# qinzheng93/GeoTransformer

Hardware: NVIDIA H100
Metric: point-cloud pairs/sec (3DMatch-shape synth) (higher is better)
Workload: dtype f32

## Files before the change

### geotransformer_b200/_lib.py

```python
import ctypes
import os
import threading

import torch

_HERE = os.path.dirname(os.path.abspath(__file__))
LIB_PATH = os.path.join(_HERE, 'libgeob200.so')
_lib = None

c_void_p, c_int64, c_int32, c_float, c_size_t, c_int = (
    ctypes.c_void_p, ctypes.c_int64, ctypes.c_int32, ctypes.c_float, ctypes.c_size_t, ctypes.c_int)

SIGNATURES = {}


def _sig(name, restype, *argtypes):
    SIGNATURES[name] = (restype, list(argtypes))


P, I64, I32, F, SZ = c_void_p, c_int64, c_int32, c_float, c_size_t
_sig('geob200_last_error', ctypes.c_char_p)
_sig('geob200_launch_count', ctypes.c_uint64)
_sig('geob200_grid_subsample_workspace_bytes', SZ, I64, I64)
_sig('geob200_grid_subsample', c_int, P, I64, P, I64, F, P, P, P, SZ, P)
_sig('geob200_radius_search_workspace_bytes', SZ, I64, I64, I64)
_sig('geob200_radius_search', c_int, P, I64, P, I64, P, P, I64, F, I64, P, P, P, P, SZ, P)

_sig('geob200_neighbor_histogram', c_int, P, I64, I64, I64, I64, P, P)
_sig('geob200_kpconv_workspace_bytes', SZ, I64)
_sig('geob200_kpconv', c_int, P, P, P, P, I64, I64, I64, P, I64, P, P, I64, I64, F, P, P, SZ, P)
_sig('geob200_kpconv_tc_workspace_bytes', SZ, I64, I64, I64)
_sig('geob200_kpconv_tc', c_int, P, P, P, P, I64, I64, I64, P, I64, P, P, I64, I64, F, P, P, SZ, P)
_sig('geob200_set_linear_mode', None, c_int)
_sig('geob200_linear', c_int, P, I64, P, P, P, I64, I64, I64, I64, c_int, P)
_sig('geob200_linear_batched', c_int, P, I64, I64, P, I64, I64, P, I64, P, I64, I64, I64, I64, I64, I64, c_int, P)
_sig('geob200_group_norm_workspace_bytes', SZ, I64)
_sig('geob200_group_norm', c_int, P, I64, I64, I64, P, P, F, P, c_int, F, P, P, SZ, P)
_sig('geob200_fused_group_norm_workspace_bytes', SZ, I64, I64, I64)
_sig('geob200_linear_group_norm', c_int, P, I64, P, P, I64, I64, I64, I64, P, P, F, P, c_int, F, P, P, P, SZ, P)
_sig('geob200_kpconv_group_norm_workspace_bytes', SZ, I64, I64, I64, I64, I64)
_sig('geob200_kpconv_group_norm', c_int, P, P, P, P, I64, I64, I64, P, I64, P, P, I64, I64, F, I64, P, P, F, c_int, F, P, P, P, SZ,
     P, SZ, P)
_sig('geob200_group_norm_batched_workspace_bytes', SZ, I64, I64, I64, I64)
_sig('geob200_group_norm_batched', c_int, P, I64, I64, I64, P, P, F, P, c_int, F, P, P, SZ, P, I64, P)
_sig('geob200_linear_group_norm_batched', c_int, P, I64, P, P, I64, I64, I64, I64, P, P, F, P, c_int, F, P, P, P, SZ, P, I64, P)
_sig('geob200_maxpool', c_int, P, P, I64, I64, I64, I64, P, P)
_sig('geob200_upsample_concat', c_int, P, P, I64, I64, P, I64, I64, I64, P, P)
_sig('geob200_point_to_node_partition', c_int, P, I64, P, I64, I64, P, P, P, P, P, P, P)
_sig('geob200_point_to_node_partition_batched', c_int, P, P, I64, P, P, I64, P, P, P, P, P, P)
_sig('geob200_gather_rows', c_int, P, I64, I64, P, I64, P, P)
_sig('geob200_knn_partition', c_int, P, I64, P, I64, I64, P, P, P)
_sig('geob200_pairwise_distance', c_int, P, I64, P, I64, I64, c_int, P, P)
_sig('geob200_point_to_node_indices', c_int, P, I64, P, I64, P, P, P)
_sig('geob200_apply_transform', c_int, P, I64, P, P, P)
_sig('geob200_gse_indices', c_int, P, I64, F, F, I64, P, P, P)
_sig('geob200_gse_indices_batched', c_int, P, I64, P, F, F, I64, P, P, P)
_sig('geob200_gse_embed_workspace_bytes', SZ, I64, I64)
_sig('geob200_gse_table_bytes', SZ, I64, I64, F, F)
_sig('geob200_gse_table_build', c_int, P, P, P, P, P, I64, I64, F, F, P, SZ, P)
_sig('geob200_gse_embed_table', c_int, P, P, I64, I64, P, SZ, I64, F, F, P, P, P, P, P, P, P)
_sig('geob200_gse_embed', c_int, P, P, I64, I64, P, P, P, P, P, P, P, P, c_int, P, SZ, P)
_sig('geob200_gse_embed_pairs', c_int, P, P, I64, I64, P, P, P, P, P, P, P, P, c_int, P, SZ, P)
_sig('geob200_attention_workspace_bytes', SZ, I64, I64, I64)
_sig('geob200_attention', c_int, P, I64, P, I64, P, I64, P, P, P, I64, I64, I64, I64, P, I64, P, SZ, P)
_sig('geob200_set_attention_tma', c_int, c_int)
_sig('geob200_head_bias', c_int, P, I64, P, I64, I64, I64, P, P)
_sig('geob200_add_layernorm', c_int, P, P, P, P, I64, I64, F, P, P)
_sig('geob200_l2_normalize', c_int, P, I64, I64, P, P)
_sig('geob200_superpoint_matching_workspace_bytes', SZ, I64, I64)
_sig('geob200_superpoint_matching', c_int, P, P, I64, I64, I64, P, P, I64, c_int, P, P, P, P, P, SZ, P)
_sig('geob200_gather_patches', c_int, P, I64, P, P, I64, P, I64, P, P, P, P)
_sig('geob200_patch_scores', c_int, P, I64, P, I64, I64, P, P, I64, I64, P, P)
_sig('geob200_sinkhorn', c_int, P, P, P, P, I64, I64, I64, F, P, P)
_sig('geob200_lgr_workspace_bytes', SZ, I64, I64, I64)
_sig('geob200_local_global_registration', c_int, P, P, P, P, P, I64, I64, I64, I64, F, c_int, F, I64, I64, P, P, P, P, P,
     P, P, P, P, P, SZ, P)
_sig('geob200_superpoint_matching_batched_workspace_bytes', SZ, I64, I64, I64)
_sig('geob200_superpoint_matching_batched', c_int, P, I64, P, I64, P, I64, c_int, P, P, P, P, SZ, P)
_sig('geob200_gather_patches_batched', c_int, P, I64, I64, P, P, P, P, I64, P, P, P, P, P)
_sig('geob200_patch_scores_batched', c_int, P, I64, I64, P, P, P, I64, I64, P, P)
_sig('geob200_lgr_batched_workspace_bytes', SZ, I64, I64, I64, I64)
_sig('geob200_local_global_registration_batched', c_int, P, P, P, P, P, I64, I64, I64, I64, I64, F, c_int, F, I64, I64, P, P, P, P,
     P, P, I64, P, P, P, P, SZ, P)
_sig('geob200_weighted_procrustes', c_int, P, P, P, I64, I64, F, F, P, P)

_sig('geob200_node_correspondences_workspace_bytes', SZ, I64, I64, I64)
_sig('geob200_node_correspondences', c_int, P, P, P, P, P, P, P, P, I64, I64, I64, P, F, P, P, P, P, SZ, P)
_sig('geob200_node_correspondences_batched_workspace_bytes', SZ, I64, I64, I64)
_sig('geob200_node_correspondences_batched', c_int, P, P, P, P, I64, P, I64, P, F, P, P, P, P, SZ, P)
_sig('geob200_evaluate', c_int, P, P, I64, F, P, P, I64, P, P, I64, F, P, P, P, I64, c_int, F, F, F, P, P)
_sig('geob200_evaluate_counts', c_int, P, P, I64, P, F, P, P, I64, P, P, P, I64, P, F, P, P, P, I64, c_int, F, F, F, P, P)
_sig('geob200_evaluate_batched', c_int, P, P, P, F, P, P, I64, P, P, P, I64, P, F, P, P, I64, P, I64, P, P, c_int, F, F, F, P, I64,
     P)

_sig('geob200_linear_profile_enable', c_int, c_int)
_sig('geob200_set_split_k', c_int, c_int)
_sig('geob200_set_linear_persistent', c_int, c_int)
_sig('geob200_linear_profile_read', I64, I64, P, P)
_sig('geob200_backbone_workspace_bytes', SZ, P, P)
_sig('geob200_backbone_forward', c_int, P, P, P, P, P, P, P, P, P, P, P, P, SZ, P, SZ, P)
_sig('geob200_transformer_workspace_bytes', SZ, I64, I64, I64, I64, I64)
_sig('geob200_transformer_forward', c_int, P, I64, I64, I64, P, I64, I64, P, P, P, P, SZ, P)
_sig('geob200_backbone_gn_workspace_bytes', SZ, P, P, I64)
_sig('geob200_backbone_forward_batched', c_int, P, P, P, P, P, P, P, P, P, P, P, P, SZ, P, SZ, P, I64, P, P)
_sig('geob200_cloud_max_count', c_int, P, I64, I64, I64, I64, P, P, P)
_sig('geob200_maxpool_batched', c_int, P, P, I64, I64, I64, I64, P, I64, P, P, P)
_sig('geob200_transformer_batched_workspace_bytes', SZ, I64, P, I64, I64, I64)
_sig('geob200_transformer_forward_batched', c_int, P, I64, I64, I64, P, I64, P, P, P, P, SZ, P)
_sig('geob200_attention_batched_workspace_bytes', SZ, P, I64, I64)
_sig('geob200_attention_batched', c_int, P, I64, I64, I64, I64, I64, I64, I64, P, SZ, P)


def lib():
    global _lib
    if _lib is None:
        if not os.path.exists(LIB_PATH):
            raise RuntimeError(
                f'{LIB_PATH} not found: build it with `python -c "import __graft_entry__ as g; g.build()"` '
                '(there is no CPU fallback for the geotransformer_b200 ops)')
        handle = ctypes.CDLL(LIB_PATH)
        for name, (restype, argtypes) in SIGNATURES.items():
            fn = getattr(handle, name)
            fn.restype = restype
            fn.argtypes = argtypes
        _lib = handle
    return _lib


def check(rc, what):
    if rc != 0:
        msg = lib().geob200_last_error().decode(errors='replace')
        raise RuntimeError(f'{what} failed ({rc}): {msg}')


_tls = threading.local()


def stream_ptr():
    p = getattr(_tls, 'stream', None)
    if p is not None:
        return p
    return torch.cuda.current_stream().cuda_stream


class stream_scope:

    def __init__(self, ptr):
        self.ptr = ptr

    def __enter__(self):
        self.prev = getattr(_tls, 'stream', None)
        _tls.stream = self.ptr
        return self

    def __exit__(self, *a):
        _tls.stream = self.prev
        return False


def require_cuda(t, name, dtype=None):
    if not t.is_cuda:
        raise RuntimeError(f'{name} must be a CUDA tensor (geotransformer_b200 has no CPU path)')
    if dtype is not None and t.dtype != dtype:
        raise RuntimeError(f'{name} must be {dtype}, got {t.dtype}')
    if not t.is_contiguous():
        raise RuntimeError(f'{name} must be contiguous')


_WS = {}


def workspace(nbytes, device, tag='default'):
    key = (device.index if device.index is not None else torch.cuda.current_device(), stream_ptr(), tag)
    buf = _WS.get(key)
    if buf is None or buf.numel() < nbytes:
        buf = torch.empty(max(int(nbytes * 1.3), 1 << 20), dtype=torch.uint8, device=device)
        _WS[key] = buf
    return buf


def ptr(t):
    return None if t is None else t.data_ptr()
```

### geotransformer_b200/csrc/common.cuh

```cuda
#pragma once
#include <cuda_runtime.h>
#include <stdint.h>
#include <stdio.h>

namespace geob200 {

void set_error(const char* fmt, ...);
void count_launches(int n);
int ensure_max_smem(const void* kernel);

#define GEOB_CHECK_CUDA(expr)                                                                   \
    do {                                                                                        \
        cudaError_t _e = (expr);                                                                \
        if (_e != cudaSuccess) {                                                                \
            geob200::set_error("%s:%d CUDA error %s: %s", __FILE__, __LINE__, #expr,            \
                               cudaGetErrorString(_e));                                         \
            return -1;                                                                          \
        }                                                                                       \
    } while (0)

#define GEOB_CHECK_LAUNCH()                                                                     \
    do {                                                                                        \
        cudaError_t _e = cudaGetLastError();                                                    \
        if (_e != cudaSuccess) {                                                                \
            geob200::set_error("%s:%d kernel launch failed: %s", __FILE__, __LINE__,            \
                               cudaGetErrorString(_e));                                         \
            return -1;                                                                          \
        }                                                                                       \
    } while (0)

#define GEOB_REQUIRE(cond, ...)                                                                 \
    do {                                                                                        \
        if (!(cond)) {                                                                          \
            geob200::set_error(__VA_ARGS__);                                                    \
            return -2;                                                                          \
        }                                                                                       \
    } while (0)

static inline size_t align_up(size_t x, size_t a) { return (x + a - 1) / a * a; }

template <int CNT, int MASK>
struct Butterfly {
    template <int NV>
    static __device__ __forceinline__ void run(float (&v)[NV], int lane) {
        if constexpr (CNT > 1) {
            constexpr int HALF = CNT / 2;
            const bool upper = (lane & MASK) != 0;
#pragma unroll
            for (int i = 0; i < HALF; ++i) {
                const float send = upper ? v[i] : v[i + HALF];
                const float keep = upper ? v[i + HALF] : v[i];
                v[i] = keep + __shfl_xor_sync(0xffffffffu, send, MASK);
            }
            if constexpr (MASK > 1) Butterfly<HALF, MASK / 2>::run(v, lane);
        } else {
            v[0] += __shfl_xor_sync(0xffffffffu, v[0], MASK);
            if constexpr (MASK > 1) Butterfly<1, MASK / 2>::run(v, lane);
        }
    }
};
template <int NV>
__device__ __forceinline__ float warp_butterfly(float (&v)[NV], int lane) {
    Butterfly<NV, 16>::run(v, lane);
    return v[0];
}

struct GnFuse {
    int groups;
    int slot_width;
    double* partial;
};

constexpr int GEOB_MAX_CLOUDS = 64;
struct GnSeg {
    int n_clouds;
    int n_pairs;
    int start[GEOB_MAX_CLOUDS + 1];
};
size_t fused_group_norm_workspace_bytes_batched(int64_t n_rows, int64_t channels, int64_t groups, int64_t n_pairs);
int group_norm_impl(const float* x, int64_t n_rows, int64_t channels, int64_t groups, const float* gamma, const float* beta, float eps,
                    const float* residual, int leaky, float slope, float* y, void* workspace, size_t workspace_bytes, void* stream,
                    const GnSeg* seg);
int linear_group_norm_impl(const float* x, int64_t ldx, const float* weight, const float* bias, int64_t m, int64_t n, int64_t k,
                           int64_t groups, const float* gamma, const float* beta, float eps, const float* residual, int leaky,
                           float slope, float* pre_norm, float* y, void* workspace, size_t workspace_bytes, void* stream,
                           const GnSeg* seg);
int kpconv_group_norm_impl(const float* s_feats, const float* q_points, const float* s_points, const int64_t* neighbors,
                           int64_t n_query, int64_t n_support, int64_t n_neighbors, const float* kernel_points, int64_t n_kernel,
                           const float* weights_t, const float* bias, int64_t c_in, int64_t c_out, float sigma, int64_t groups,
                           const float* gamma, const float* beta, float eps, int leaky, float slope, float* pre_norm, float* y,
                           void* gn_workspace, size_t gn_workspace_bytes, void* workspace, size_t workspace_bytes, void* stream,
                           const GnSeg* seg);

int maxpool_seg(const float* x, const int64_t* neighbors, int64_t n_query, int64_t n_support, int64_t n_neighbors, int64_t channels,
                float* y, const GnSeg* seg, const int* cloud_max, void* stream);

struct Segs {
    int n;
    int max;
    int start[GEOB_MAX_CLOUDS];
    int count[GEOB_MAX_CLOUDS];
};
int segs_from_counts(Segs* s, int64_t n, const int64_t* counts);
Segs segs_one(int64_t count);
Segs segs_range(const Segs& s, int first, int n);
int segs_products(Segs* s, const Segs& ref, const Segs& src);

struct Arena {
    char* base;
    size_t off;
    size_t cap;
    __host__ Arena(void* p, size_t bytes) : base(static_cast<char*>(p)), off(0), cap(bytes) {}
    template <typename T>
    __host__ T* take(size_t n) {
        off = align_up(off, 256);
        T* r = reinterpret_cast<T*>(base + off);
        off += n * sizeof(T);
        return r;
    }
    __host__ bool ok() const { return off <= cap; }
};

__device__ __forceinline__ float warp_sum(float v) {
#pragma unroll
    for (int o = 16; o > 0; o >>= 1) v += __shfl_xor_sync(0xffffffffu, v, o);
    return v;
}
__device__ __forceinline__ float warp_max(float v) {
#pragma unroll
    for (int o = 16; o > 0; o >>= 1) v = fmaxf(v, __shfl_xor_sync(0xffffffffu, v, o));
    return v;
}
__device__ __forceinline__ double warp_sum_d(double v) {
#pragma unroll
    for (int o = 16; o > 0; o >>= 1) v += __shfl_xor_sync(0xffffffffu, v, o);
    return v;
}

__device__ __forceinline__ float tf32_rn(float x) {
    uint32_t r;
    asm("cvt.rna.tf32.f32 %0, %1;" : "=r"(r) : "f"(x));
    return __uint_as_float(r);
}

static inline int num_sms() {
    static int n = 0;
    if (n == 0) {
        int dev = 0;
        cudaGetDevice(&dev);
        cudaDeviceGetAttribute(&n, cudaDevAttrMultiProcessorCount, dev);
        if (n <= 0) n = 132;
    }
    return n;
}

}
```

### geotransformer_b200/csrc/hopper.cuh

```cuda
#pragma once
#include <cuda.h>
#include <stdint.h>

namespace geob200 {
namespace hop {

__device__ __forceinline__ uint32_t smem_u32(const void* p) { return (uint32_t)__cvta_generic_to_shared(p); }
__device__ __forceinline__ void mbar_init(uint64_t* bar, uint32_t count) {
    asm volatile("mbarrier.init.shared::cta.b64 [%0], %1;" ::"r"(smem_u32(bar)), "r"(count));
}
__device__ __forceinline__ void mbar_arrive(uint64_t* bar) {
    asm volatile("{\n\t.reg .b64 st;\n\tmbarrier.arrive.shared::cta.b64 st, [%0];\n\t}" ::"r"(smem_u32(bar)) : "memory");
}
__device__ __forceinline__ void mbar_arrive_expect_tx(uint64_t* bar, uint32_t bytes) {
    asm volatile("{\n\t.reg .b64 st;\n\tmbarrier.arrive.expect_tx.shared::cta.b64 st, [%0], %1;\n\t}" ::"r"(smem_u32(bar)), "r"(bytes)
                 : "memory");
}
__device__ __forceinline__ void mbar_wait(uint64_t* bar, uint32_t parity) {
    const uint32_t addr = smem_u32(bar);
    uint32_t done;
    do {
        asm volatile("{\n\t.reg .pred p;\n\tmbarrier.try_wait.parity.shared::cta.b64 p, [%1], %2;\n\tselp.u32 %0, 1, 0, p;\n\t}"
                     : "=r"(done)
                     : "r"(addr), "r"(parity)
                     : "memory");
    } while (!done);
}
__device__ __forceinline__ void mbar_wait_cluster(uint64_t* bar, uint32_t parity) {
    const uint32_t addr = smem_u32(bar);
    uint32_t done;
    do {
        asm volatile("{\n\t.reg .pred p;\n\tmbarrier.try_wait.parity.acquire.cluster.shared::cta.b64 p, [%1], %2;\n\tselp.u32 %0, 1, 0, p;\n\t}"
                     : "=r"(done)
                     : "r"(addr), "r"(parity)
                     : "memory");
    } while (!done);
}
__device__ __forceinline__ void fence_proxy_async() { asm volatile("fence.proxy.async.shared::cta;" ::: "memory"); }

__device__ __forceinline__ void tma_load_2d(void* dst, const CUtensorMap* map, int c0, int c1, uint64_t* bar) {
    asm volatile("cp.async.bulk.tensor.2d.shared::cluster.global.mbarrier::complete_tx::bytes [%0], [%1, {%2, %3}], [%4];" ::"r"(
                     smem_u32(dst)),
                 "l"(map), "r"(c0), "r"(c1), "r"(smem_u32(bar))
                 : "memory");
}
__device__ __forceinline__ void bulk_g2s(void* dst, const void* src, uint32_t bytes, uint64_t* bar) {
    asm volatile("cp.async.bulk.shared::cluster.global.mbarrier::complete_tx::bytes [%0], [%1], %2, [%3];" ::"r"(smem_u32(dst)),
                 "l"(src), "r"(bytes), "r"(smem_u32(bar))
                 : "memory");
}

__device__ __forceinline__ uint64_t make_desc(uint32_t smem_addr) {
    uint64_t d = 0;
    d |= (uint64_t)((smem_addr & 0x3FFFFu) >> 4);
    d |= (uint64_t)1 << 16;
    d |= (uint64_t)(1024 >> 4) << 32;
    d |= (uint64_t)1 << 62;
    return d;
}

__device__ __forceinline__ void wgmma_fence() { asm volatile("wgmma.fence.sync.aligned;" ::: "memory"); }
__device__ __forceinline__ void wgmma_commit() { asm volatile("wgmma.commit_group.sync.aligned;" ::: "memory"); }
template <int N>
__device__ __forceinline__ void wgmma_wait() { asm volatile("wgmma.wait_group.sync.aligned %0;" ::"n"(N) : "memory"); }
template <int R>
__device__ __forceinline__ void reg_fence(float (&d)[R]) {
#pragma unroll
    for (int i = 0; i < R; ++i) asm volatile("" : "+f"(d[i])::"memory");
}

template <int N> __device__ void wgmma_tf32(float (&d)[N / 2], uint64_t da, uint64_t db, uint32_t acc);

template <> __device__ __forceinline__ void wgmma_tf32<32>(float (&d)[16], uint64_t da, uint64_t db, uint32_t acc) {
    asm volatile(
        "{\n\t.reg .pred p;\n\tsetp.ne.b32 p, %18, 0;\n\t"
        "wgmma.mma_async.sync.aligned.m64n32k8.f32.tf32.tf32 {%0, %1, %2, %3, %4, %5, %6, %7, %8, %9, %10, %11, %12, %13, %14, %15}, %16, %17, p, 1, 1;\n\t}"
        : "+f"(d[0]), "+f"(d[1]), "+f"(d[2]), "+f"(d[3]), "+f"(d[4]), "+f"(d[5]), "+f"(d[6]), "+f"(d[7]), "+f"(d[8]), "+f"(d[9]), "+f"(d[10]), "+f"(d[11]), "+f"(d[12]), "+f"(d[13]), "+f"(d[14]), "+f"(d[15])
        : "l"(da), "l"(db), "r"(acc));
}

template <> __device__ __forceinline__ void wgmma_tf32<64>(float (&d)[32], uint64_t da, uint64_t db, uint32_t acc) {
    asm volatile(
        "{\n\t.reg .pred p;\n\tsetp.ne.b32 p, %34, 0;\n\t"
        "wgmma.mma_async.sync.aligned.m64n64k8.f32.tf32.tf32 {%0, %1, %2, %3, %4, %5, %6, %7, %8, %9, %10, %11, %12, %13, %14, %15, %16, %17, %18, %19, %20, %21, %22, %23, %24, %25, %26, %27, %28, %29, %30, %31}, %32, %33, p, 1, 1;\n\t}"
        : "+f"(d[0]), "+f"(d[1]), "+f"(d[2]), "+f"(d[3]), "+f"(d[4]), "+f"(d[5]), "+f"(d[6]), "+f"(d[7]), "+f"(d[8]), "+f"(d[9]), "+f"(d[10]), "+f"(d[11]), "+f"(d[12]), "+f"(d[13]), "+f"(d[14]), "+f"(d[15]), "+f"(d[16]), "+f"(d[17]), "+f"(d[18]), "+f"(d[19]), "+f"(d[20]), "+f"(d[21]), "+f"(d[22]), "+f"(d[23]), "+f"(d[24]), "+f"(d[25]), "+f"(d[26]), "+f"(d[27]), "+f"(d[28]), "+f"(d[29]), "+f"(d[30]), "+f"(d[31])
        : "l"(da), "l"(db), "r"(acc));
}

template <> __device__ __forceinline__ void wgmma_tf32<128>(float (&d)[64], uint64_t da, uint64_t db, uint32_t acc) {
    asm volatile(
        "{\n\t.reg .pred p;\n\tsetp.ne.b32 p, %66, 0;\n\t"
        "wgmma.mma_async.sync.aligned.m64n128k8.f32.tf32.tf32 {%0, %1, %2, %3, %4, %5, %6, %7, %8, %9, %10, %11, %12, %13, %14, %15, %16, %17, %18, %19, %20, %21, %22, %23, %24, %25, %26, %27, %28, %29, %30, %31, %32, %33, %34, %35, %36, %37, %38, %39, %40, %41, %42, %43, %44, %45, %46, %47, %48, %49, %50, %51, %52, %53, %54, %55, %56, %57, %58, %59, %60, %61, %62, %63}, %64, %65, p, 1, 1;\n\t}"
        : "+f"(d[0]), "+f"(d[1]), "+f"(d[2]), "+f"(d[3]), "+f"(d[4]), "+f"(d[5]), "+f"(d[6]), "+f"(d[7]), "+f"(d[8]), "+f"(d[9]), "+f"(d[10]), "+f"(d[11]), "+f"(d[12]), "+f"(d[13]), "+f"(d[14]), "+f"(d[15]), "+f"(d[16]), "+f"(d[17]), "+f"(d[18]), "+f"(d[19]), "+f"(d[20]), "+f"(d[21]), "+f"(d[22]), "+f"(d[23]), "+f"(d[24]), "+f"(d[25]), "+f"(d[26]), "+f"(d[27]), "+f"(d[28]), "+f"(d[29]), "+f"(d[30]), "+f"(d[31]), "+f"(d[32]), "+f"(d[33]), "+f"(d[34]), "+f"(d[35]), "+f"(d[36]), "+f"(d[37]), "+f"(d[38]), "+f"(d[39]), "+f"(d[40]), "+f"(d[41]), "+f"(d[42]), "+f"(d[43]), "+f"(d[44]), "+f"(d[45]), "+f"(d[46]), "+f"(d[47]), "+f"(d[48]), "+f"(d[49]), "+f"(d[50]), "+f"(d[51]), "+f"(d[52]), "+f"(d[53]), "+f"(d[54]), "+f"(d[55]), "+f"(d[56]), "+f"(d[57]), "+f"(d[58]), "+f"(d[59]), "+f"(d[60]), "+f"(d[61]), "+f"(d[62]), "+f"(d[63])
        : "l"(da), "l"(db), "r"(acc));
}

template <> __device__ __forceinline__ void wgmma_tf32<256>(float (&d)[128], uint64_t da, uint64_t db, uint32_t acc) {
    asm volatile(
        "{\n\t.reg .pred p;\n\tsetp.ne.b32 p, %130, 0;\n\t"
        "wgmma.mma_async.sync.aligned.m64n256k8.f32.tf32.tf32 {%0, %1, %2, %3, %4, %5, %6, %7, %8, %9, %10, %11, %12, %13, %14, %15, %16, %17, %18, %19, %20, %21, %22, %23, %24, %25, %26, %27, %28, %29, %30, %31, %32, %33, %34, %35, %36, %37, %38, %39, %40, %41, %42, %43, %44, %45, %46, %47, %48, %49, %50, %51, %52, %53, %54, %55, %56, %57, %58, %59, %60, %61, %62, %63, %64, %65, %66, %67, %68, %69, %70, %71, %72, %73, %74, %75, %76, %77, %78, %79, %80, %81, %82, %83, %84, %85, %86, %87, %88, %89, %90, %91, %92, %93, %94, %95, %96, %97, %98, %99, %100, %101, %102, %103, %104, %105, %106, %107, %108, %109, %110, %111, %112, %113, %114, %115, %116, %117, %118, %119, %120, %121, %122, %123, %124, %125, %126, %127}, %128, %129, p, 1, 1;\n\t}"
        : "+f"(d[0]), "+f"(d[1]), "+f"(d[2]), "+f"(d[3]), "+f"(d[4]), "+f"(d[5]), "+f"(d[6]), "+f"(d[7]), "+f"(d[8]), "+f"(d[9]), "+f"(d[10]), "+f"(d[11]), "+f"(d[12]), "+f"(d[13]), "+f"(d[14]), "+f"(d[15]), "+f"(d[16]), "+f"(d[17]), "+f"(d[18]), "+f"(d[19]), "+f"(d[20]), "+f"(d[21]), "+f"(d[22]), "+f"(d[23]), "+f"(d[24]), "+f"(d[25]), "+f"(d[26]), "+f"(d[27]), "+f"(d[28]), "+f"(d[29]), "+f"(d[30]), "+f"(d[31]), "+f"(d[32]), "+f"(d[33]), "+f"(d[34]), "+f"(d[35]), "+f"(d[36]), "+f"(d[37]), "+f"(d[38]), "+f"(d[39]), "+f"(d[40]), "+f"(d[41]), "+f"(d[42]), "+f"(d[43]), "+f"(d[44]), "+f"(d[45]), "+f"(d[46]), "+f"(d[47]), "+f"(d[48]), "+f"(d[49]), "+f"(d[50]), "+f"(d[51]), "+f"(d[52]), "+f"(d[53]), "+f"(d[54]), "+f"(d[55]), "+f"(d[56]), "+f"(d[57]), "+f"(d[58]), "+f"(d[59]), "+f"(d[60]), "+f"(d[61]), "+f"(d[62]), "+f"(d[63]), "+f"(d[64]), "+f"(d[65]), "+f"(d[66]), "+f"(d[67]), "+f"(d[68]), "+f"(d[69]), "+f"(d[70]), "+f"(d[71]), "+f"(d[72]), "+f"(d[73]), "+f"(d[74]), "+f"(d[75]), "+f"(d[76]), "+f"(d[77]), "+f"(d[78]), "+f"(d[79]), "+f"(d[80]), "+f"(d[81]), "+f"(d[82]), "+f"(d[83]), "+f"(d[84]), "+f"(d[85]), "+f"(d[86]), "+f"(d[87]), "+f"(d[88]), "+f"(d[89]), "+f"(d[90]), "+f"(d[91]), "+f"(d[92]), "+f"(d[93]), "+f"(d[94]), "+f"(d[95]), "+f"(d[96]), "+f"(d[97]), "+f"(d[98]), "+f"(d[99]), "+f"(d[100]), "+f"(d[101]), "+f"(d[102]), "+f"(d[103]), "+f"(d[104]), "+f"(d[105]), "+f"(d[106]), "+f"(d[107]), "+f"(d[108]), "+f"(d[109]), "+f"(d[110]), "+f"(d[111]), "+f"(d[112]), "+f"(d[113]), "+f"(d[114]), "+f"(d[115]), "+f"(d[116]), "+f"(d[117]), "+f"(d[118]), "+f"(d[119]), "+f"(d[120]), "+f"(d[121]), "+f"(d[122]), "+f"(d[123]), "+f"(d[124]), "+f"(d[125]), "+f"(d[126]), "+f"(d[127])
        : "l"(da), "l"(db), "r"(acc));
}

template <int N> __device__ void wgmma_f16(float (&d)[N / 2], uint64_t da, uint64_t db, uint32_t acc);

template <> __device__ __forceinline__ void wgmma_f16<128>(float (&d)[64], uint64_t da, uint64_t db, uint32_t acc) {
    asm volatile(
        "{\n\t.reg .pred p;\n\tsetp.ne.b32 p, %66, 0;\n\t"
        "wgmma.mma_async.sync.aligned.m64n128k16.f32.f16.f16 {%0, %1, %2, %3, %4, %5, %6, %7, %8, %9, %10, %11, %12, %13, %14, %15, %16, %17, %18, %19, %20, %21, %22, %23, %24, %25, %26, %27, %28, %29, %30, %31, %32, %33, %34, %35, %36, %37, %38, %39, %40, %41, %42, %43, %44, %45, %46, %47, %48, %49, %50, %51, %52, %53, %54, %55, %56, %57, %58, %59, %60, %61, %62, %63}, %64, %65, p, 1, 1, 0, 0;\n\t}"
        : "+f"(d[0]), "+f"(d[1]), "+f"(d[2]), "+f"(d[3]), "+f"(d[4]), "+f"(d[5]), "+f"(d[6]), "+f"(d[7]), "+f"(d[8]), "+f"(d[9]), "+f"(d[10]), "+f"(d[11]), "+f"(d[12]), "+f"(d[13]), "+f"(d[14]), "+f"(d[15]), "+f"(d[16]), "+f"(d[17]), "+f"(d[18]), "+f"(d[19]), "+f"(d[20]), "+f"(d[21]), "+f"(d[22]), "+f"(d[23]), "+f"(d[24]), "+f"(d[25]), "+f"(d[26]), "+f"(d[27]), "+f"(d[28]), "+f"(d[29]), "+f"(d[30]), "+f"(d[31]), "+f"(d[32]), "+f"(d[33]), "+f"(d[34]), "+f"(d[35]), "+f"(d[36]), "+f"(d[37]), "+f"(d[38]), "+f"(d[39]), "+f"(d[40]), "+f"(d[41]), "+f"(d[42]), "+f"(d[43]), "+f"(d[44]), "+f"(d[45]), "+f"(d[46]), "+f"(d[47]), "+f"(d[48]), "+f"(d[49]), "+f"(d[50]), "+f"(d[51]), "+f"(d[52]), "+f"(d[53]), "+f"(d[54]), "+f"(d[55]), "+f"(d[56]), "+f"(d[57]), "+f"(d[58]), "+f"(d[59]), "+f"(d[60]), "+f"(d[61]), "+f"(d[62]), "+f"(d[63])
        : "l"(da), "l"(db), "r"(acc));
}

template <> __device__ __forceinline__ void wgmma_f16<256>(float (&d)[128], uint64_t da, uint64_t db, uint32_t acc) {
    asm volatile(
        "{\n\t.reg .pred p;\n\tsetp.ne.b32 p, %130, 0;\n\t"
        "wgmma.mma_async.sync.aligned.m64n256k16.f32.f16.f16 {%0, %1, %2, %3, %4, %5, %6, %7, %8, %9, %10, %11, %12, %13, %14, %15, %16, %17, %18, %19, %20, %21, %22, %23, %24, %25, %26, %27, %28, %29, %30, %31, %32, %33, %34, %35, %36, %37, %38, %39, %40, %41, %42, %43, %44, %45, %46, %47, %48, %49, %50, %51, %52, %53, %54, %55, %56, %57, %58, %59, %60, %61, %62, %63, %64, %65, %66, %67, %68, %69, %70, %71, %72, %73, %74, %75, %76, %77, %78, %79, %80, %81, %82, %83, %84, %85, %86, %87, %88, %89, %90, %91, %92, %93, %94, %95, %96, %97, %98, %99, %100, %101, %102, %103, %104, %105, %106, %107, %108, %109, %110, %111, %112, %113, %114, %115, %116, %117, %118, %119, %120, %121, %122, %123, %124, %125, %126, %127}, %128, %129, p, 1, 1, 0, 0;\n\t}"
        : "+f"(d[0]), "+f"(d[1]), "+f"(d[2]), "+f"(d[3]), "+f"(d[4]), "+f"(d[5]), "+f"(d[6]), "+f"(d[7]), "+f"(d[8]), "+f"(d[9]), "+f"(d[10]), "+f"(d[11]), "+f"(d[12]), "+f"(d[13]), "+f"(d[14]), "+f"(d[15]), "+f"(d[16]), "+f"(d[17]), "+f"(d[18]), "+f"(d[19]), "+f"(d[20]), "+f"(d[21]), "+f"(d[22]), "+f"(d[23]), "+f"(d[24]), "+f"(d[25]), "+f"(d[26]), "+f"(d[27]), "+f"(d[28]), "+f"(d[29]), "+f"(d[30]), "+f"(d[31]), "+f"(d[32]), "+f"(d[33]), "+f"(d[34]), "+f"(d[35]), "+f"(d[36]), "+f"(d[37]), "+f"(d[38]), "+f"(d[39]), "+f"(d[40]), "+f"(d[41]), "+f"(d[42]), "+f"(d[43]), "+f"(d[44]), "+f"(d[45]), "+f"(d[46]), "+f"(d[47]), "+f"(d[48]), "+f"(d[49]), "+f"(d[50]), "+f"(d[51]), "+f"(d[52]), "+f"(d[53]), "+f"(d[54]), "+f"(d[55]), "+f"(d[56]), "+f"(d[57]), "+f"(d[58]), "+f"(d[59]), "+f"(d[60]), "+f"(d[61]), "+f"(d[62]), "+f"(d[63]), "+f"(d[64]), "+f"(d[65]), "+f"(d[66]), "+f"(d[67]), "+f"(d[68]), "+f"(d[69]), "+f"(d[70]), "+f"(d[71]), "+f"(d[72]), "+f"(d[73]), "+f"(d[74]), "+f"(d[75]), "+f"(d[76]), "+f"(d[77]), "+f"(d[78]), "+f"(d[79]), "+f"(d[80]), "+f"(d[81]), "+f"(d[82]), "+f"(d[83]), "+f"(d[84]), "+f"(d[85]), "+f"(d[86]), "+f"(d[87]), "+f"(d[88]), "+f"(d[89]), "+f"(d[90]), "+f"(d[91]), "+f"(d[92]), "+f"(d[93]), "+f"(d[94]), "+f"(d[95]), "+f"(d[96]), "+f"(d[97]), "+f"(d[98]), "+f"(d[99]), "+f"(d[100]), "+f"(d[101]), "+f"(d[102]), "+f"(d[103]), "+f"(d[104]), "+f"(d[105]), "+f"(d[106]), "+f"(d[107]), "+f"(d[108]), "+f"(d[109]), "+f"(d[110]), "+f"(d[111]), "+f"(d[112]), "+f"(d[113]), "+f"(d[114]), "+f"(d[115]), "+f"(d[116]), "+f"(d[117]), "+f"(d[118]), "+f"(d[119]), "+f"(d[120]), "+f"(d[121]), "+f"(d[122]), "+f"(d[123]), "+f"(d[124]), "+f"(d[125]), "+f"(d[126]), "+f"(d[127])
        : "l"(da), "l"(db), "r"(acc));
}

}
}
```

### geotransformer_b200/csrc/kpconv.cu

```cuda
#include "common.cuh"
#include "geob200.h"

namespace geob200 {

constexpr int KP = 15;
constexpr int KP_PAD = 16;
constexpr int TQ = 32;
constexpr int CC = 32;

__device__ __forceinline__ void influence15(const float* __restrict__ kp_s, float rx, float ry, float rz, float inv_dummy,
                                            float sigma, float* w) {
#pragma unroll
    for (int k = 0; k < KP; ++k) {
        const float dx = rx - kp_s[3 * k], dy = ry - kp_s[3 * k + 1], dz = rz - kp_s[3 * k + 2];
        const float sq = __fadd_rn(__fadd_rn(__fmul_rn(dx, dx), __fmul_rn(dy, dy)), __fmul_rn(dz, dz));
        w[k] = fmaxf(1.0f - sqrtf(sq) / sigma, 0.0f);
    }
    (void)inv_dummy;
}

__global__ void __launch_bounds__(256) kpconv_c1_kernel(const float* __restrict__ feats, const float* __restrict__ q_pts,
                                                        const float* __restrict__ s_pts, const long long* __restrict__ nbr,
                                                        int H, const float* __restrict__ kp, const float* __restrict__ W,
                                                        const float* __restrict__ bias, float sigma, int Ns, int M, int Cout,
// ... 496 lines not shown
            if (var < 0.0) var = 0.0;
            mean_rstd[2 * g] = (float)mean;
            mean_rstd[2 * g + 1] = (float)(1.0 / sqrt(var + eps));
        }
    }
}

__global__ void __launch_bounds__(256) gn_tile_stats_kernel(const float* __restrict__ x, int N, int C, int slot_width,
                                                            double* __restrict__ partial) {
    extern __shared__ double sh[];
    const int slots = C / slot_width;
    for (int i = threadIdx.x; i < 2 * slots; i += blockDim.x) sh[i] = 0.0;
    __syncthreads();
    const int r0 = blockIdx.x * 128, r1 = min(N, r0 + 128);
    const int cw = C < 256 ? C : 256;
    const int rpb = 256 / cw;
    const int rr = threadIdx.x / cw;
    if (rr < rpb)
        for (int c = threadIdx.x % cw; c < C; c += cw) {
            double s = 0.0, s2 = 0.0;
            for (int r = r0 + rr; r < r1; r += rpb) {
                const double v = (double)x[(long long)r * C + c];
                s += v;
                s2 += v * v;
            }
            atomicAdd(&sh[2 * (c / slot_width)], s);
            atomicAdd(&sh[2 * (c / slot_width) + 1], s2);
        }
    __syncthreads();
    for (int i = threadIdx.x; i < 2 * slots; i += blockDim.x) partial[(long long)blockIdx.x * 2 * slots + i] = sh[i];
}

__global__ void __launch_bounds__(128) gn_seg_finalize_kernel(const double* __restrict__ partial, const float* __restrict__ x, int C,
                                                              int slots_total, int spg, int G, double eps, GnSeg seg,
                                                              float* __restrict__ mean_rstd) {
    __shared__ double red[8];
    const int lane = threadIdx.x & 31, warp = threadIdx.x >> 5;
    const int g = blockIdx.x, p = blockIdx.y;
    const int cpg = C / G;
    const double2* part = reinterpret_cast<const double2*>(partial);
    double sa = 0.0, sb = 0.0;
    long long rows = 0;
    for (int c = p; c < seg.n_clouds; c += seg.n_pairs) {
        const int r0 = seg.start[c], r1 = seg.start[c + 1];
        rows += r1 - r0;
        int t0 = (r0 + 127) / 128, t1 = r1 / 128;
        if (t1 < t0) t1 = t0;
        const int n_full = (t1 - t0) * spg;
        for (int i = threadIdx.x; i < n_full; i += 128) {
            const int t = t0 + i / spg, sl = i % spg;
            const double2 v = part[(long long)t * slots_total + (long long)g * spg + sl];
            sa += v.x;
            sb += v.y;
        }
        const int e0 = min(r1, t0 * 128);
        const int b1 = min(r1, max(e0, t1 * 128));
        const int n_edge = (e0 - r0) + (r1 - b1);
        for (int i = threadIdx.x; i < n_edge * cpg; i += 128) {
            const int ri = i / cpg, j = i % cpg;
            const int r = ri < e0 - r0 ? r0 + ri : b1 + (ri - (e0 - r0));
            const double v = (double)x[(long long)r * C + g * cpg + j];
            sa += v;
            sb += v * v;
        }
    }
#pragma unroll
    for (int o = 16; o > 0; o >>= 1) {
        sa += __shfl_xor_sync(0xffffffffu, sa, o);
        sb += __shfl_xor_sync(0xffffffffu, sb, o);
    }
    if (lane == 0) { red[2 * warp] = sa; red[2 * warp + 1] = sb; }
    __syncthreads();
    if (threadIdx.x == 0) {
        sa = (red[0] + red[2]) + (red[4] + red[6]);
        sb = (red[1] + red[3]) + (red[5] + red[7]);
        const double count = (double)cpg * (double)rows;
        const double mean = sa / count;
        double var = sb / count - mean * mean;
        if (var < 0.0) var = 0.0;
        mean_rstd[((long long)p * G + g) * 2] = (float)mean;
        mean_rstd[((long long)p * G + g) * 2 + 1] = (float)(1.0 / sqrt(var + eps));
    }
}

constexpr int GN_RPB = 32;
__global__ void __launch_bounds__(256) gn_seg_apply_kernel(const float* __restrict__ x, const float* __restrict__ mean_rstd,
                                                           const float* __restrict__ gamma, const float* __restrict__ beta,
                                                           const float* __restrict__ residual, float* __restrict__ y, int n_rows,
                                                           int C, int cpg, int G, int leaky, float slope, GnSeg seg) {
    extern __shared__ float gn_tab[];
    __shared__ int starts[GEOB_MAX_CLOUDS + 1];
    for (int i = threadIdx.x; i <= seg.n_clouds; i += blockDim.x) starts[i] = seg.start[i];
    __syncthreads();
    const int r0 = blockIdx.x * GN_RPB, r1 = min(n_rows, r0 + GN_RPB);
    int c0 = 0, hi = seg.n_clouds;
    while (hi - c0 > 1) {
        const int mid = (c0 + hi) >> 1;
        if (starts[mid] <= r0) c0 = mid; else hi = mid;
    }
    for (int i = threadIdx.x; i < 2 * C; i += blockDim.x) {
        const int t = i / C, c = i % C;
        const int cl = min(c0 + t, seg.n_clouds - 1);
        const float* mr = mean_rstd + (long long)(cl % seg.n_pairs) * 2 * G + 2 * (c / cpg);
        gn_tab[(2 * t) * C + c] = mr[0];
        gn_tab[(2 * t + 1) * C + c] = mr[1];
    }
    __syncthreads();
    const int b0 = starts[c0 + 1];
    const int b1 = (c0 + 2 <= seg.n_clouds) ? starts[c0 + 2] : n_rows;
    const int C4 = C >> 2;
    const long long base4 = (long long)r0 * C4;
    const int total4 = (r1 - r0) * C4;
    for (int i = threadIdx.x; i < total4; i += blockDim.x) {
        const int row = r0 + i / C4, c = (i % C4) * 4;
        const float4 v = reinterpret_cast<const float4*>(x)[base4 + i];
        float4 rv = make_float4(0.f, 0.f, 0.f, 0.f);
        if (residual != nullptr) rv = reinterpret_cast<const float4*>(residual)[base4 + i];
        float in[4] = {v.x, v.y, v.z, v.w}, o[4];
        const float rs[4] = {rv.x, rv.y, rv.z, rv.w};
        if (row < b1) {
            const float* ta = gn_tab + (row < b0 ? 0 : 2 * C) + c;
            const float4 gm = __ldg(reinterpret_cast<const float4*>(gamma + c)), bt = __ldg(reinterpret_cast<const float4*>(beta + c));
            const float ga[4] = {gm.x, gm.y, gm.z, gm.w}, ba[4] = {bt.x, bt.y, bt.z, bt.w};
#pragma unroll
            for (int u = 0; u < 4; ++u) o[u] = (in[u] - ta[u]) * ta[C + u] * ga[u] + ba[u] + rs[u];
        } else {
            int lo = c0, hh = seg.n_clouds;
            while (hh - lo > 1) {
                const int mid = (lo + hh) >> 1;
                if (starts[mid] <= row) lo = mid; else hh = mid;
            }
            const float* mr = mean_rstd + (long long)(lo % seg.n_pairs) * 2 * G;
#pragma unroll
            for (int u = 0; u < 4; ++u) {
                const int g = (c + u) / cpg;
                o[u] = (in[u] - mr[2 * g]) * mr[2 * g + 1] * gamma[c + u] + beta[c + u] + rs[u];
            }
        }
        if (leaky) {
#pragma unroll
            for (int u = 0; u < 4; ++u) o[u] = o[u] > 0.f ? o[u] : o[u] * slope;
        }
        reinterpret_cast<float4*>(y)[base4 + i] = make_float4(o[0], o[1], o[2], o[3]);
    }
}

__global__ void __launch_bounds__(256) gn_apply_kernel(const float* __restrict__ x, const float* __restrict__ mean_rstd,
                                                       const float* __restrict__ gamma, const float* __restrict__ beta,
                                                       const float* __restrict__ residual, float* __restrict__ y,
                                                       long long total4, int C, int cpg, int leaky, float slope) {
    const long long i = (long long)blockIdx.x * blockDim.x + threadIdx.x;
    if (i >= total4) return;
    const float4 v = reinterpret_cast<const float4*>(x)[i];
    const int c = (int)((i * 4) % C);
    float in[4] = {v.x, v.y, v.z, v.w}, o[4];
    float4 rv = make_float4(0.f, 0.f, 0.f, 0.f);
    if (residual != nullptr) rv = reinterpret_cast<const float4*>(residual)[i];
    const float rs[4] = {rv.x, rv.y, rv.z, rv.w};
#pragma unroll
    for (int u = 0; u < 4; ++u) {
        const int g = (c + u) / cpg;
        float t = (in[u] - mean_rstd[2 * g]) * mean_rstd[2 * g + 1] * gamma[c + u] + beta[c + u];
        t += rs[u];
        if (leaky) t = t > 0.f ? t : t * slope;
        o[u] = t;
    }
    reinterpret_cast<float4*>(y)[i] = make_float4(o[0], o[1], o[2], o[3]);
}

__device__ __forceinline__ void maxpool_row(const float* __restrict__ x, const long long* __restrict__ nb, int W, int Ns, int C,
                                            float* __restrict__ yrow, int lane) {
    constexpr int NI = 5;
    if ((C & 3) == 0 && W <= 32 * NI) {
        int idx_l[NI];
#pragma unroll
        for (int i = 0; i < NI; ++i) idx_l[i] = (lane + 32 * i < W) ? (int)min(nb[lane + 32 * i], (long long)Ns) : Ns;
        const int C4 = C >> 2;
        for (int c0 = 0; c0 < C4; c0 += 32) {
            const int c4 = c0 + lane;
            const bool active = c4 < C4;
            float4 best = make_float4(-INFINITY, -INFINITY, -INFINITY, -INFINITY);
            for (int h0 = 0; h0 < W; h0 += 4) {
                float4 v[4];
#pragma unroll
                for (int u = 0; u < 4; ++u) {
                    const int h = h0 + u;
                    int id = Ns;
#pragma unroll
                    for (int i = 0; i < NI; ++i) {
                        const int t = __shfl_sync(0xffffffffu, idx_l[i], h & 31);
                        if ((h >> 5) == i) id = t;
                    }
                    v[u] = (active && h < W && id < Ns) ? __ldg(reinterpret_cast<const float4*>(x + (long long)id * C) + c4)
                                                        : make_float4(0.f, 0.f, 0.f, 0.f);
                    if (h >= W) v[u] = best;
                }
#pragma unroll
                for (int u = 0; u < 4; ++u) {
                    best.x = fmaxf(best.x, v[u].x); best.y = fmaxf(best.y, v[u].y);
                    best.z = fmaxf(best.z, v[u].z); best.w = fmaxf(best.w, v[u].w);
                }
            }
            if (active) reinterpret_cast<float4*>(yrow)[c4] = best;
        }
        return;
    }
    for (int c = lane; c < C; c += 32) {
        float best = -INFINITY;
        for (int h = 0; h < W; ++h) {
            const long long idx = nb[h];
            const float v = (idx < Ns) ? x[idx * C + c] : 0.f;
            best = fmaxf(best, v);
        }
        yrow[c] = best;
    }
}

__global__ void __launch_bounds__(256) maxpool_seg_kernel(const float* __restrict__ x, const long long* __restrict__ nbr, int H,
                                                          int Ns, int M, int C, float* __restrict__ y, GnSeg seg,
                                                          const int* __restrict__ cloud_max) {
    __shared__ int starts[GEOB_MAX_CLOUDS + 1];
    __shared__ int width[GEOB_MAX_CLOUDS];
    for (int i = threadIdx.x; i <= seg.n_clouds; i += blockDim.x) starts[i] = seg.start[i];
    for (int i = threadIdx.x; i < seg.n_clouds; i += blockDim.x) {
        const int p = i % seg.n_pairs;
        int w = 0;
        for (int c = p; c < seg.n_clouds; c += seg.n_pairs) w = max(w, cloud_max[c]);
        width[i] = min(H, w);
    }
    __syncthreads();
    const int lane = threadIdx.x & 31;
    const int m = blockIdx.x * 8 + (threadIdx.x >> 5);
    if (m >= M) return;
    int lo = 0, hi = seg.n_clouds;
    while (hi - lo > 1) {
        const int mid = (lo + hi) >> 1;
        if (starts[mid] <= m) lo = mid; else hi = mid;
    }
    const int W = width[lo];
    maxpool_row(x, nbr + (long long)m * H, W, Ns, C, y + (long long)m * C, lane);
}

__global__ void __launch_bounds__(256) cloud_max_count_kernel(const long long* __restrict__ nbr, int H, int Ns, GnSeg seg,
                                                              int* __restrict__ cloud_max) {
    __shared__ int red[8];
    const int c = blockIdx.x;
    const int r0 = seg.start[c], r1 = seg.start[c + 1];
    int best = 0;
    for (int m = r0 + (int)threadIdx.x; m < r1; m += blockDim.x) {
        int lo = 0, hi = H;
        while (lo < hi) {
            const int mid = (lo + hi) >> 1;
            if (nbr[(long long)m * H + mid] < Ns) lo = mid + 1; else hi = mid;
        }
        best = max(best, lo);
    }
    for (int o = 16; o > 0; o >>= 1) best = max(best, __shfl_xor_sync(0xffffffffu, best, o));
    if ((threadIdx.x & 31) == 0) red[threadIdx.x >> 5] = best;
    __syncthreads();
    if (threadIdx.x == 0) {
        for (int w = 1; w < 8; ++w) best = max(best, red[w]);
        cloud_max[c] = best;
    }
}

__global__ void __launch_bounds__(256) maxpool_kernel(const float* __restrict__ x, const long long* __restrict__ nbr, int H,
                                                      int Ns, int M, int C, float* __restrict__ y) {
    const int lane = threadIdx.x & 31;
    const int m = blockIdx.x * 8 + (threadIdx.x >> 5);
    if (m >= M) return;
    if ((C & 3) == 0 && H <= 160) {
        maxpool_row(x, nbr + (long long)m * H, H, Ns, C, y + (long long)m * C, lane);
        return;
    }
    for (int c = lane; c < C; c += 32) {
        float best = -INFINITY;
        for (int h = 0; h < H; ++h) {
            const long long idx = nbr[(long long)m * H + h];
            const float v = (idx < Ns) ? x[idx * C + c] : 0.f;
            best = fmaxf(best, v);
        }
        y[(long long)m * C + c] = best;
    }
}

__global__ void __launch_bounds__(256) upsample_concat_kernel(const float* __restrict__ x, const long long* __restrict__ up,
                                                              int up_stride, int Ns, const float* __restrict__ skip, int M,
                                                              int C1, int C2, float* __restrict__ y) {
    const int lane = threadIdx.x & 31;
    const int m = blockIdx.x * 8 + (threadIdx.x >> 5);
    if (m >= M) return;
    const long long idx = up[(long long)m * up_stride];
    float* yr = y + (long long)m * (C1 + C2);
    for (int c = lane; c < C1; c += 32) yr[c] = (idx < Ns) ? x[idx * C1 + c] : 0.f;
    if (skip != nullptr)
        for (int c = lane; c < C2; c += 32) yr[C1 + c] = skip[(long long)m * C2 + c];
}

}

using namespace geob200;

namespace geob200 {
int linear_tc(const float* x, int64_t ldx, const float* w, int64_t ldw, const float* bias, const float* row_scale, float* y, int64_t ldy,
              int64_t m, int64_t n, int64_t k, int relu, cudaStream_t st, const GnFuse* gn = nullptr);
static int g_linear_mode = 1;
}

extern "C" {

void geob200_set_linear_mode(int mode) { g_linear_mode = mode; }

size_t geob200_kpconv_workspace_bytes(int64_t n_support) { return (size_t)n_support + 256; }

size_t geob200_kpconv_tc_workspace_bytes(int64_t n_query, int64_t n_support, int64_t c_in) {
    return align_up((size_t)n_support, 256) + align_up((size_t)n_query * 4, 256) + (size_t)n_query * KP * (size_t)c_in * 4 + 1024;
}

int geob200_kpconv_tc(const float* s_feats, const float* q_points, const float* s_points, const int64_t* neighbors, int64_t n_query,
                      int64_t n_support, int64_t n_neighbors, const float* kernel_points, int64_t n_kernel, const float* weights_t,
                      const float* bias, int64_t c_in, int64_t c_out, float sigma, float* out, void* workspace, size_t workspace_bytes,
                      void* stream) {
    cudaStream_t st = (cudaStream_t)stream;
    GEOB_REQUIRE(n_kernel == KP, "kpconv_tc: kernel_size %lld unsupported", (long long)n_kernel);
    GEOB_REQUIRE(n_query > 0 && n_support > 0 && n_neighbors > 0, "kpconv_tc: empty input");
    GEOB_REQUIRE(c_in % 32 == 0 && c_out % 16 == 0 && c_out >= 32 && (c_out <= 128 || c_out % 128 == 0) && n_query >= 64,
                 "kpconv_tc: unsupported shape (%lld -> %lld, %lld queries)", (long long)c_in, (long long)c_out, (long long)n_query);
    GEOB_REQUIRE(workspace_bytes >= geob200_kpconv_tc_workspace_bytes(n_query, n_support, c_in), "kpconv_tc: workspace too small");
    Arena ar(workspace, workspace_bytes);
    unsigned char* pos = ar.take<unsigned char>(n_support);
    float* inv_count = ar.take<float>(n_query);
    float* wf = ar.take<float>((size_t)n_query * KP * c_in);
    row_positive_kernel<<<(unsigned)((n_support + 7) / 8), 256, 0, st>>>(s_feats, (int)n_support, (int)c_in, pos);
    launch_kpconv_gather(s_feats, pos, q_points, s_points, (const long long*)neighbors, (int)n_neighbors, kernel_points, sigma,
                         (int)n_support, (int)n_query, (int)c_in, wf, inv_count, st);
    GEOB_CHECK_LAUNCH();
    count_launches(2);
    const int rc = linear_tc(wf, KP * c_in, weights_t, KP * c_in, bias, inv_count, out, c_out, n_query, c_out, KP * c_in, 0, st);
    GEOB_REQUIRE(rc == 0, "kpconv_tc: tensor-core GEMM rejected the shape");
    return 0;
}

int geob200_kpconv(const float* s_feats, const float* q_points, const float* s_points, const int64_t* neighbors,
                   int64_t n_query, int64_t n_support, int64_t n_neighbors, const float* kernel_points, int64_t n_kernel,
                   const float* weights, const float* bias, int64_t c_in, int64_t c_out, float sigma, float* out,
                   void* workspace, size_t workspace_bytes, void* stream) {
    cudaStream_t st = (cudaStream_t)stream;
    GEOB_REQUIRE(n_kernel == KP, "kpconv: kernel_size %lld unsupported (all shipped models use 15)", (long long)n_kernel);
    GEOB_REQUIRE(n_query > 0 && n_support > 0 && n_neighbors > 0, "kpconv: empty input");
    if (c_in == 1) {
        kpconv_c1_kernel<<<(unsigned)((n_query + 15) / 16), 256, 0, st>>>(s_feats, q_points, s_points, (const long long*)neighbors,
                                                                       (int)n_neighbors, kernel_points, weights, bias, sigma,
                                                                       (int)n_support, (int)n_query, (int)c_out, out);
        GEOB_CHECK_LAUNCH();
        count_launches(1);
        return 0;
    }
    GEOB_REQUIRE(c_in % 32 == 0 && c_out % 32 == 0 && c_out <= 512,
                 "kpconv: channel counts (%lld -> %lld) must be multiples of 32, c_out <= 512", (long long)c_in, (long long)c_out);
    GEOB_REQUIRE(workspace != nullptr && workspace_bytes >= geob200_kpconv_workspace_bytes(n_support), "kpconv: workspace too small");
    unsigned char* pos = (unsigned char*)workspace;
    row_positive_kernel<<<(unsigned)((n_support + 7) / 8), 256, 0, st>>>(s_feats, (int)n_support, (int)c_in, pos);
    const size_t smem = sizeof(float) * (TQ * KP * CC + 8 * 32 * KP_PAD + TQ + KP * 3 + 3) + sizeof(int) * 8 * 32;
    const unsigned qtiles = (unsigned)((n_query + TQ - 1) / TQ);
    int rc = (int)(c_out / 32);
    int split = 1;
    while (rc > 1 && split < 4 && (long long)qtiles * split < 2ll * num_sms()) { rc >>= 1; split <<= 1; }
    const dim3 grid(qtiles, (unsigned)split);
#define LAUNCH_KP(RCV)                                                                                              \
    {                                                                                                               \
        if (ensure_max_smem((const void*)kpconv_kernel<RCV>)) return -1;                                            \
        kpconv_kernel<RCV><<<grid, 256, smem, st>>>(s_feats, pos, q_points, s_points, (const long long*)neighbors,  \
                                                    (int)n_neighbors, kernel_points, weights, bias, sigma,         \
                                                    (int)n_support, (int)n_query, (int)c_in, (int)c_out, out);     \
    }
    switch (rc) {
        case 1: LAUNCH_KP(1) break;
        case 2: LAUNCH_KP(2) break;
        case 4: LAUNCH_KP(4) break;
        case 8: LAUNCH_KP(8) break;
        case 16: LAUNCH_KP(16) break;
        default: GEOB_REQUIRE(false, "kpconv: c_out %lld unsupported (32,64,128,256,512)", (long long)c_out);
    }
#undef LAUNCH_KP
    GEOB_CHECK_LAUNCH();
    count_launches(2);
    return 0;
}

int geob200_linear_batched(const float* x, int64_t ldx, int64_t stride_x, const float* weight, int64_t ldw, int64_t stride_w,
                           const float* bias, int64_t stride_b, float* y, int64_t ldy, int64_t stride_y, int64_t m, int64_t n,
                           int64_t k, int64_t batch, int relu, void* stream) {
    cudaStream_t st = (cudaStream_t)stream;
    GEOB_REQUIRE(m > 0 && n > 0 && k > 0 && batch > 0, "linear: empty problem");
    if (batch == 1 && g_linear_mode == 1) {
        const int rc = linear_tc(x, ldx, weight, ldw, bias, nullptr, y, ldy, m, n, k, relu, st);
        if (rc <= 0) return rc;
    }
    const unsigned z = (unsigned)batch;
    const long long c64 = ((n + 63) / 64) * ((m + 63) / 64) * batch, c6432 = ((n + 31) / 32) * ((m + 63) / 64) * batch;
    if (c64 >= num_sms()) {
        dim3 grid((unsigned)((n + 63) / 64), (unsigned)((m + 63) / 64), z);
        linear_kernel<64, 64><<<grid, 256, 0, st>>>(x, (int)ldx, weight, (int)ldw, bias, y, (int)ldy, (int)m, (int)n, (int)k, relu,
                                                    stride_x, stride_w, stride_b, stride_y);
    } else if (c6432 >= num_sms()) {
        dim3 grid((unsigned)((n + 31) / 32), (unsigned)((m + 63) / 64), z);
        linear_kernel<64, 32><<<grid, 256, 0, st>>>(x, (int)ldx, weight, (int)ldw, bias, y, (int)ldy, (int)m, (int)n, (int)k, relu,
                                                    stride_x, stride_w, stride_b, stride_y);
    } else {
        dim3 grid((unsigned)((n + 31) / 32), (unsigned)((m + 31) / 32), z);
        linear_kernel<32, 32><<<grid, 256, 0, st>>>(x, (int)ldx, weight, (int)ldw, bias, y, (int)ldy, (int)m, (int)n, (int)k, relu,
                                                    stride_x, stride_w, stride_b, stride_y);
    }
    GEOB_CHECK_LAUNCH();
    count_launches(1);
    return 0;
}

int geob200_linear(const float* x, int64_t ldx, const float* weight, const float* bias, float* y, int64_t ldy, int64_t m,
                   int64_t n, int64_t k, int relu, void* stream) {
    return geob200_linear_batched(x, ldx, 0, weight, k, 0, bias, 0, y, ldy, 0, m, n, k, 1, relu, stream);
}

size_t geob200_group_norm_workspace_bytes(int64_t groups) { return (size_t)(592 * 2 * groups * 8 + 2 * groups * 4 + 256 + 1024); }

size_t geob200_fused_group_norm_workspace_bytes(int64_t n_rows, int64_t channels, int64_t groups) {
    const size_t tiles = (size_t)((n_rows + 127) / 128);
    const size_t slots = (size_t)(channels / groups >= 32 ? channels / 32 : groups);
    const size_t fused = tiles * slots * 2 * 8;
    const size_t plain = (size_t)(592 * 2 * groups * 8);
    return (fused > plain ? fused : plain) + (size_t)(2 * groups * 4) + 256 + 1024;
}

}

namespace geob200 {
size_t fused_group_norm_workspace_bytes_batched(int64_t n_rows, int64_t channels, int64_t groups, int64_t n_pairs) {
    return geob200_fused_group_norm_workspace_bytes(n_rows, channels, groups) + (size_t)(2 * groups * 4) * (size_t)(n_pairs > 1 ? n_pairs : 1) + 512;
}
struct GnWs { unsigned* ticket; float* mean_rstd; double* partial; };
static GnWs gn_carve(void* workspace, size_t bytes, int64_t groups, int64_t n_pairs = 1) {
    Arena ar(workspace, bytes);
    GnWs w;
    w.ticket = ar.take<unsigned>(64);
    w.mean_rstd = ar.take<float>(2 * groups * n_pairs);
    w.partial = ar.take<double>(1);
    return w;
}
static void launch_gn_seg_apply(const float* x, const GnWs& w, const float* gamma, const float* beta, const float* residual, float* y,
                                int64_t n_rows, int64_t channels, int64_t groups, float eps, int leaky, float slope, const GnSeg& seg,
                                cudaStream_t st) {
    const int cpg = (int)(channels / groups);
    const int slot_width = cpg < 32 ? cpg : 32;
    gn_seg_finalize_kernel<<<dim3((unsigned)groups, (unsigned)seg.n_pairs), 128, 0, st>>>(
        w.partial, x, (int)channels, (int)(channels / slot_width), cpg / slot_width, (int)groups, (double)eps, seg, w.mean_rstd);
    gn_seg_apply_kernel<<<(unsigned)((n_rows + GN_RPB - 1) / GN_RPB), 256, sizeof(float) * 4 * channels, st>>>(
        x, w.mean_rstd, gamma, beta, residual, y, (int)n_rows, (int)channels, cpg, (int)groups, leaky, slope, seg);
    count_launches(2);
}
static void launch_gn_tile_stats(const float* x, const GnWs& w, int64_t n_rows, int64_t channels, int64_t groups, cudaStream_t st) {
    const int cpg = (int)(channels / groups);
    const int slot_width = cpg < 32 ? cpg : 32;
    gn_tile_stats_kernel<<<(unsigned)((n_rows + 127) / 128), 256, sizeof(double) * 2 * (channels / slot_width), st>>>(
        x, (int)n_rows, (int)channels, slot_width, w.partial);
    count_launches(1);
}
static void launch_gn_apply(const float* x, const GnWs& w, const float* gamma, const float* beta, const float* residual, float* y,
                            int64_t n_rows, int64_t channels, int64_t groups, float eps, int leaky, float slope, cudaStream_t st) {
    const int cpg = (int)(channels / groups);
    const int slot_width = cpg < 32 ? cpg : 32;
    gn_finalize_kernel<<<1, 1024, 0, st>>>(w.partial, (int)((n_rows + 127) / 128), (int)(channels / slot_width), cpg / slot_width,
                                           (int)groups, (double)cpg * (double)n_rows, (double)eps, w.mean_rstd);
    const long long total4 = n_rows * channels / 4;
    gn_apply_kernel<<<(unsigned)((total4 + 255) / 256), 256, 0, st>>>(x, w.mean_rstd, gamma, beta, residual, y, total4, (int)channels,
                                                                     (int)(channels / groups), leaky, slope);
}
}

extern "C" {

int geob200_group_norm(const float* x, int64_t n_rows, int64_t channels, int64_t groups, const float* gamma,
                       const float* beta, float eps, const float* residual, int leaky, float slope, float* y,
                       void* workspace, size_t workspace_bytes, void* stream) {
    return geob200::group_norm_impl(x, n_rows, channels, groups, gamma, beta, eps, residual, leaky, slope, y, workspace, workspace_bytes,
                                    stream, nullptr);
}
}

namespace geob200 {
int group_norm_impl(const float* x, int64_t n_rows, int64_t channels, int64_t groups, const float* gamma, const float* beta, float eps,
                    const float* residual, int leaky, float slope, float* y, void* workspace, size_t workspace_bytes, void* stream,
                    const GnSeg* seg) {
    cudaStream_t st = (cudaStream_t)stream;
    GEOB_REQUIRE(n_rows > 0 && channels > 0 && groups > 0 && channels % groups == 0, "group_norm: bad shape");
    GEOB_REQUIRE(channels % 4 == 0, "group_norm: channels must be a multiple of 4");
    if (seg != nullptr && seg->n_pairs > 1) {
        GEOB_REQUIRE(workspace_bytes >= fused_group_norm_workspace_bytes_batched(n_rows, channels, groups, seg->n_pairs),
                     "group_norm: workspace too small (batched)");
        const GnWs w = gn_carve(workspace, workspace_bytes, groups, seg->n_pairs);
        launch_gn_tile_stats(x, w, n_rows, channels, groups, st);
        launch_gn_seg_apply(x, w, gamma, beta, residual, y, n_rows, channels, groups, eps, leaky, slope, *seg, st);
        GEOB_CHECK_LAUNCH();
        return 0;
    }
    GEOB_REQUIRE(workspace_bytes >= geob200_group_norm_workspace_bytes(groups), "group_norm: workspace too small");
    Arena ar(workspace, workspace_bytes);
    unsigned* ticket = ar.take<unsigned>(64);
    float* mean_rstd = ar.take<float>(2 * groups);
    double* partial = ar.take<double>(592 * 2 * groups);
    int nblk = (int)((n_rows + 127) / 128);
    if (nblk > 296) nblk = 296;
    if (nblk < 1) nblk = 1;
    gn_stats_kernel<<<nblk, 256, sizeof(double) * 2 * groups, st>>>(x, (int)n_rows, (int)channels, (int)groups, (double)eps,
                                                                    partial, ticket, mean_rstd);
    const long long total4 = n_rows * channels / 4;
    gn_apply_kernel<<<(unsigned)((total4 + 255) / 256), 256, 0, st>>>(x, mean_rstd, gamma, beta, residual, y, total4,
                                                                     (int)channels, (int)(channels / groups), leaky, slope);
    GEOB_CHECK_LAUNCH();
    count_launches(2);
    return 0;
}
}

extern "C" {

int geob200_maxpool(const float* x, const int64_t* neighbors, int64_t n_query, int64_t n_support, int64_t n_neighbors,
                    int64_t channels, float* y, void* stream) {
    maxpool_kernel<<<(unsigned)((n_query + 7) / 8), 256, 0, (cudaStream_t)stream>>>(x, (const long long*)neighbors, (int)n_neighbors,
                                                                                  (int)n_support, (int)n_query, (int)channels, y);
    GEOB_CHECK_LAUNCH();
    count_launches(1);
    return 0;
}

int geob200_upsample_concat(const float* x, const int64_t* up_indices, int64_t up_stride, int64_t n_support,
                            const float* skip, int64_t n_query, int64_t c1, int64_t c2, float* y, void* stream) {
    upsample_concat_kernel<<<(unsigned)((n_query + 7) / 8), 256, 0, (cudaStream_t)stream>>>(
        x, (const long long*)up_indices, (int)up_stride, (int)n_support, skip, (int)n_query, (int)c1, (int)c2, y);
    GEOB_CHECK_LAUNCH();
    count_launches(1);
    return 0;
}

int geob200_linear_group_norm(const float* x, int64_t ldx, const float* weight, const float* bias, int64_t m, int64_t n, int64_t k,
                              int64_t groups, const float* gamma, const float* beta, float eps, const float* residual, int leaky,
                              float slope, float* pre_norm, float* y, void* workspace, size_t workspace_bytes, void* stream) {
    return geob200::linear_group_norm_impl(x, ldx, weight, bias, m, n, k, groups, gamma, beta, eps, residual, leaky, slope, pre_norm, y,
                                           workspace, workspace_bytes, stream, nullptr);
}
}

namespace geob200 {
int linear_group_norm_impl(const float* x, int64_t ldx, const float* weight, const float* bias, int64_t m, int64_t n, int64_t k,
                           int64_t groups, const float* gamma, const float* beta, float eps, const float* residual, int leaky,
                           float slope, float* pre_norm, float* y, void* workspace, size_t workspace_bytes, void* stream,
                           const GnSeg* seg) {
    cudaStream_t st = (cudaStream_t)stream;
    const int64_t np = (seg != nullptr && seg->n_pairs > 1) ? seg->n_pairs : 1;
    GEOB_REQUIRE(m > 0 && n > 0 && k > 0 && groups > 0 && n % groups == 0 && n % 4 == 0, "linear_group_norm: bad shape");
    GEOB_REQUIRE(workspace_bytes >= (np > 1 ? fused_group_norm_workspace_bytes_batched(m, n, groups, np)
                                            : geob200_fused_group_norm_workspace_bytes(m, n, groups)), "linear_group_norm: workspace too small");
    if (g_linear_mode == 1) {
        const GnWs w = gn_carve(workspace, workspace_bytes, groups, np);
        GnFuse gn{(int)groups, 0, w.partial};
        const int rc = linear_tc(x, ldx, weight, k, bias, nullptr, pre_norm, n, m, n, k, 0, st, &gn);
        if (rc < 0) return rc;
        if (rc == 0) {
            if (np > 1) {
                launch_gn_seg_apply(pre_norm, w, gamma, beta, residual, y, m, n, groups, eps, leaky, slope, *seg, st);
            } else {
                launch_gn_apply(pre_norm, w, gamma, beta, residual, y, m, n, groups, eps, leaky, slope, st);
                count_launches(2);
            }
            GEOB_CHECK_LAUNCH();
            return 0;
        }
    }
    int rc = geob200_linear(x, ldx, weight, bias, pre_norm, n, m, n, k, 0, stream);
    if (rc != 0) return rc;
    return group_norm_impl(pre_norm, m, n, groups, gamma, beta, eps, residual, leaky, slope, y, workspace, workspace_bytes, stream, seg);
}
}

extern "C" {

size_t geob200_kpconv_group_norm_workspace_bytes(int64_t n_query, int64_t n_support, int64_t c_in, int64_t c_out, int64_t groups) {
    return align_up(geob200_fused_group_norm_workspace_bytes(n_query, c_out, groups), 256) +
           geob200_kpconv_tc_workspace_bytes(n_query, n_support, c_in);
}

int geob200_kpconv_group_norm(const float* s_feats, const float* q_points, const float* s_points, const int64_t* neighbors,
                              int64_t n_query, int64_t n_support, int64_t n_neighbors, const float* kernel_points, int64_t n_kernel,
                              const float* weights_t, const float* bias, int64_t c_in, int64_t c_out, float sigma, int64_t groups,
                              const float* gamma, const float* beta, float eps, int leaky, float slope, float* pre_norm, float* y,
                              void* gn_workspace, size_t gn_workspace_bytes, void* workspace, size_t workspace_bytes, void* stream) {
    return geob200::kpconv_group_norm_impl(s_feats, q_points, s_points, neighbors, n_query, n_support, n_neighbors, kernel_points, n_kernel,
                                           weights_t, bias, c_in, c_out, sigma, groups, gamma, beta, eps, leaky, slope, pre_norm, y,
                                           gn_workspace, gn_workspace_bytes, workspace, workspace_bytes, stream, nullptr);
}
}

namespace geob200 {
int kpconv_group_norm_impl(const float* s_feats, const float* q_points, const float* s_points, const int64_t* neighbors,
                           int64_t n_query, int64_t n_support, int64_t n_neighbors, const float* kernel_points, int64_t n_kernel,
                           const float* weights_t, const float* bias, int64_t c_in, int64_t c_out, float sigma, int64_t groups,
                           const float* gamma, const float* beta, float eps, int leaky, float slope, float* pre_norm, float* y,
                           void* gn_workspace, size_t gn_workspace_bytes, void* workspace, size_t workspace_bytes, void* stream,
                           const GnSeg* seg) {
    cudaStream_t st = (cudaStream_t)stream;
    const int64_t np = (seg != nullptr && seg->n_pairs > 1) ? seg->n_pairs : 1;
    GEOB_REQUIRE(n_kernel == KP, "kpconv_group_norm: kernel_size %lld unsupported", (long long)n_kernel);
    GEOB_REQUIRE(n_query > 0 && n_support > 0 && n_neighbors > 0, "kpconv_group_norm: empty input");
    GEOB_REQUIRE(c_in % 32 == 0 && c_out % 16 == 0 && c_out >= 32 && (c_out <= 128 || c_out % 128 == 0) && n_query >= 64,
                 "kpconv_group_norm: unsupported shape (%lld -> %lld, %lld queries)", (long long)c_in, (long long)c_out,
                 (long long)n_query);
    GEOB_REQUIRE(groups > 0 && c_out % groups == 0, "kpconv_group_norm: bad group count");
    GEOB_REQUIRE(gn_workspace_bytes >= (np > 1 ? fused_group_norm_workspace_bytes_batched(n_query, c_out, groups, np)
                                               : geob200_fused_group_norm_workspace_bytes(n_query, c_out, groups)),
                 "kpconv_group_norm: GroupNorm workspace too small");
    GEOB_REQUIRE(workspace_bytes >= geob200_kpconv_tc_workspace_bytes(n_query, n_support, c_in), "kpconv_group_norm: workspace too small");
    Arena ar(workspace, workspace_bytes);
    unsigned char* pos = ar.take<unsigned char>(n_support);
    float* inv_count = ar.take<float>(n_query);
    float* wf = ar.take<float>((size_t)n_query * KP * c_in);
    row_positive_kernel<<<(unsigned)((n_support + 7) / 8), 256, 0, st>>>(s_feats, (int)n_support, (int)c_in, pos);
    launch_kpconv_gather(s_feats, pos, q_points, s_points, (const long long*)neighbors, (int)n_neighbors, kernel_points, sigma,
                         (int)n_support, (int)n_query, (int)c_in, wf, inv_count, st);
    GEOB_CHECK_LAUNCH();
    count_launches(2);
    const GnWs w = gn_carve(gn_workspace, gn_workspace_bytes, groups, np);
    GnFuse gn{(int)groups, 0, w.partial};
    int rc = linear_tc(wf, KP * c_in, weights_t, KP * c_in, bias, inv_count, pre_norm, c_out, n_query, c_out, KP * c_in, 0, st, &gn);
    if (rc < 0) return rc;
    if (rc == 0) {
        if (np > 1) {
            launch_gn_seg_apply(pre_norm, w, gamma, beta, nullptr, y, n_query, c_out, groups, eps, leaky, slope, *seg, st);
        } else {
            launch_gn_apply(pre_norm, w, gamma, beta, nullptr, y, n_query, c_out, groups, eps, leaky, slope, st);
            count_launches(2);
        }
        GEOB_CHECK_LAUNCH();
        return 0;
    }
    rc = linear_tc(wf, KP * c_in, weights_t, KP * c_in, bias, inv_count, pre_norm, c_out, n_query, c_out, KP * c_in, 0, st);
    GEOB_REQUIRE(rc == 0, "kpconv_group_norm: tensor-core GEMM rejected the shape");
    return group_norm_impl(pre_norm, n_query, c_out, groups, gamma, beta, eps, nullptr, leaky, slope, y, gn_workspace, gn_workspace_bytes,
                           stream, seg);
}
}

namespace geob200 {
static int make_seg(GnSeg* g, int64_t n_pairs, const int64_t* cloud_rows_h, int64_t n_rows) {
    GEOB_REQUIRE(n_pairs >= 1 && 2 * n_pairs <= GEOB_MAX_CLOUDS && cloud_rows_h != nullptr, "group_norm: 1 <= pairs per batch <= %d", GEOB_MAX_CLOUDS / 2);
    g->n_pairs = (int)n_pairs; g->n_clouds = (int)(2 * n_pairs); g->start[0] = 0;
    for (int c = 0; c < g->n_clouds; ++c) g->start[c + 1] = g->start[c] + (int)cloud_rows_h[c];
    GEOB_REQUIRE(g->start[g->n_clouds] == n_rows, "group_norm: cloud rows do not add up to n_rows");
    return 0;
}
}

extern "C" {

size_t geob200_group_norm_batched_workspace_bytes(int64_t n_rows, int64_t channels, int64_t groups, int64_t n_pairs) {
    return geob200::fused_group_norm_workspace_bytes_batched(n_rows, channels, groups, n_pairs);
}

int geob200_group_norm_batched(const float* x, int64_t n_rows, int64_t channels, int64_t groups, const float* gamma, const float* beta,
                               float eps, const float* residual, int leaky, float slope, float* y, void* workspace, size_t workspace_bytes,
                               void* stream, int64_t n_pairs, const int64_t* cloud_rows_h) {
    geob200::GnSeg seg;
    if (geob200::make_seg(&seg, n_pairs, cloud_rows_h, n_rows)) return -2;
    return geob200::group_norm_impl(x, n_rows, channels, groups, gamma, beta, eps, residual, leaky, slope, y, workspace, workspace_bytes,
                                    stream, &seg);
}

int geob200_linear_group_norm_batched(const float* x, int64_t ldx, const float* weight, const float* bias, int64_t m, int64_t n, int64_t k,
                                      int64_t groups, const float* gamma, const float* beta, float eps, const float* residual, int leaky,
                                      float slope, float* pre_norm, float* y, void* workspace, size_t workspace_bytes, void* stream,
                                      int64_t n_pairs, const int64_t* cloud_rows_h) {
    geob200::GnSeg seg;
    if (geob200::make_seg(&seg, n_pairs, cloud_rows_h, m)) return -2;
    return geob200::linear_group_norm_impl(x, ldx, weight, bias, m, n, k, groups, gamma, beta, eps, residual, leaky, slope, pre_norm, y,
                                           workspace, workspace_bytes, stream, &seg);
}

int geob200_cloud_max_count(const int64_t* neighbors, int64_t n_query, int64_t n_support, int64_t n_neighbors, int64_t n_pairs,
                            const int64_t* cloud_rows_h, int32_t* cloud_max, void* stream) {
    geob200::GnSeg seg;
    if (geob200::make_seg(&seg, n_pairs, cloud_rows_h, n_query)) return -2;
    geob200::cloud_max_count_kernel<<<seg.n_clouds, 256, 0, (cudaStream_t)stream>>>((const long long*)neighbors, (int)n_neighbors,
                                                                                   (int)n_support, seg, cloud_max);
    GEOB_CHECK_LAUNCH();
    geob200::count_launches(1);
    return 0;
}

int geob200_maxpool_batched(const float* x, const int64_t* neighbors, int64_t n_query, int64_t n_support, int64_t n_neighbors,
                            int64_t channels, float* y, int64_t n_pairs, const int64_t* cloud_rows_h, const int32_t* cloud_max,
                            void* stream) {
    geob200::GnSeg seg;
    if (geob200::make_seg(&seg, n_pairs, cloud_rows_h, n_query)) return -2;
    return geob200::maxpool_seg(x, neighbors, n_query, n_support, n_neighbors, channels, y, &seg, cloud_max, stream);
}

}

namespace geob200 {
int maxpool_seg(const float* x, const int64_t* neighbors, int64_t n_query, int64_t n_support, int64_t n_neighbors, int64_t channels,
                float* y, const GnSeg* seg, const int* cloud_max, void* stream) {
    maxpool_seg_kernel<<<(unsigned)((n_query + 7) / 8), 256, 0, (cudaStream_t)stream>>>(x, (const long long*)neighbors, (int)n_neighbors,
                                                                                      (int)n_support, (int)n_query, (int)channels, y, *seg,
                                                                                      cloud_max);
    GEOB_CHECK_LAUNCH();
    count_launches(1);
    return 0;
}
}
```

### geotransformer_b200/csrc/linear_tc.cu

```cuda
#include <cuda.h>

#include <cstdlib>
#include <mutex>
#include <vector>

#include "common.cuh"
#include "geob200.h"
#include "hopper.cuh"

namespace geob200 {
namespace ltc {

using namespace hop;

constexpr int BM = 128;
constexpr int KC = 32;
constexpr int TILE_A = BM * 128;
constexpr int TILE_B = 128 * 128;
constexpr int STAGE = 2 * TILE_A + 2 * TILE_B;
constexpr int NSTAGE = 3;
constexpr int PRODUCER_WARP = 8;
constexpr int NSPLIT_WARPS = 3;
constexpr int NTHREADS = (PRODUCER_WARP + 1 + NSPLIT_WARPS) * 32;
constexpr int SMEM = NSTAGE * STAGE + 1024 + 256 + 8 * 128 * 8 + 512;

__device__ __forceinline__ void split_stage(unsigned char* st, int BN, int t) {
    constexpr int NT = NSPLIT_WARPS * 32;
    const int nvec_a = TILE_A / 16, nvec_b = BN * 128 / 16;
    const int nvec = nvec_a + nvec_b;
    for (int v0 = t; v0 < nvec; v0 += 2 * NT) {
        const int v1 = v0 + NT;
        unsigned char* p0 = (v0 < nvec_a) ? (st + v0 * 16) : (st + 2 * TILE_A + (v0 - nvec_a) * 16);
        unsigned char* l0 = p0 + ((v0 < nvec_a) ? TILE_A : TILE_B);
        const bool two = v1 < nvec;
        unsigned char* p1 = !two ? p0 : (v1 < nvec_a) ? (st + v1 * 16) : (st + 2 * TILE_A + (v1 - nvec_a) * 16);
        unsigned char* l1 = p1 + ((v1 < nvec_a) ? TILE_A : TILE_B);
        const float4 x0 = *reinterpret_cast<float4*>(p0);
        const float4 x1 = *reinterpret_cast<float4*>(p1);
        float4 h0, q0, h1, q1;
        h0.x = tf32_rn(x0.x); q0.x = x0.x - h0.x;
        h0.y = tf32_rn(x0.y); q0.y = x0.y - h0.y;
        h0.z = tf32_rn(x0.z); q0.z = x0.z - h0.z;
        h0.w = tf32_rn(x0.w); q0.w = x0.w - h0.w;
        h1.x = tf32_rn(x1.x); q1.x = x1.x - h1.x;
        h1.y = tf32_rn(x1.y); q1.y = x1.y - h1.y;
        h1.z = tf32_rn(x1.z); q1.z = x1.z - h1.z;
        h1.w = tf32_rn(x1.w); q1.w = x1.w - h1.w;
        *reinterpret_cast<float4*>(p0) = h0;
        *reinterpret_cast<float4*>(l0) = q0;
        if (two) {
            *reinterpret_cast<float4*>(p1) = h1;
            *reinterpret_cast<float4*>(l1) = q1;
        }
    }
    fence_proxy_async();
}

template <int BNI>
__global__ void __launch_bounds__(NTHREADS, 1) linear_tc_kernel(const __grid_constant__ CUtensorMap map_x,
                                                                const __grid_constant__ CUtensorMap map_w,
                                                                const float* __restrict__ bias, const float* __restrict__ row_scale,
                                                                float* __restrict__ Y, int ldy, int M, int N, int K, int BN, int relu,
                                                                GnFuse gn, float* __restrict__ splitk_out, int chunks_per_split,
                                                                int col_tiles, int row_tiles, int num_tiles) {
    constexpr int R = BNI / 2;
    extern __shared__ unsigned char smem_raw[];
    unsigned char* smem = (unsigned char*)(((uintptr_t)smem_raw + 1023) & ~(uintptr_t)1023);
    uint64_t* bars = (uint64_t*)(smem + NSTAGE * STAGE);
    uint64_t* raw_full = bars;
    uint64_t* split_full = bars + NSTAGE;
    uint64_t* empty = bars + 2 * NSTAGE;
    float2* gn_sm = (float2*)(smem + NSTAGE * STAGE + 256);
    float* bias_s = (float*)(gn_sm + 8 * 128);
    const int warp = threadIdx.x >> 5, lane = threadIdx.x & 31;
    const int nk = (K + KC - 1) / KC;
    const int tiles_per_split = col_tiles * row_tiles;

    if (threadIdx.x == 0) {
        for (int s = 0; s < NSTAGE; ++s) { mbar_init(&raw_full[s], 1); mbar_init(&split_full[s], NSPLIT_WARPS); mbar_init(&empty[s], 8); }
        asm volatile("fence.mbarrier_init.release.cluster;" ::: "memory");
        asm volatile("prefetch.tensormap [%0];" ::"l"(&map_x) : "memory");
        asm volatile("prefetch.tensormap [%0];" ::"l"(&map_w) : "memory");
    }
    __syncthreads();

    if (warp == PRODUCER_WARP) {
        if (lane == 0) {
            int s = 0;
            uint32_t ph = 0;
            for (int t = blockIdx.x; t < num_tiles; t += gridDim.x) {
                const int z = t / tiles_per_split, rem = t % tiles_per_split;
                const int m0 = (rem / col_tiles) * BM, n0 = (rem % col_tiles) * BN;
                const int kc0 = z * chunks_per_split, kc1 = min(nk, kc0 + chunks_per_split);
                for (int kc = kc0; kc < kc1; ++kc) {
                    mbar_wait(&empty[s], ph ^ 1u);
                    unsigned char* st = smem + s * STAGE;
                    mbar_arrive_expect_tx(&raw_full[s], (uint32_t)(TILE_A + BN * 128));
                    tma_load_2d(st, &map_x, kc * KC, m0, &raw_full[s]);
                    tma_load_2d(st + 2 * TILE_A, &map_w, kc * KC, n0, &raw_full[s]);
                    if (++s == NSTAGE) { s = 0; ph ^= 1u; }
                }
            }
        }
        return;
    }
    if (warp > PRODUCER_WARP) {
        const int ts = threadIdx.x - (PRODUCER_WARP + 1) * 32;
        int s = 0;
        uint32_t ph = 0;
        for (int t = blockIdx.x; t < num_tiles; t += gridDim.x) {
            const int z = t / tiles_per_split;
            const int kc0 = z * chunks_per_split, kc1 = min(nk, kc0 + chunks_per_split);
            for (int kc = kc0; kc < kc1; ++kc) {
                mbar_wait(&raw_full[s], ph);
                split_stage(smem + s * STAGE, BN, ts);
                __syncwarp();
                if (lane == 0) mbar_arrive(&split_full[s]);
                if (++s == NSTAGE) { s = 0; ph ^= 1u; }
            }
        }
        return;
    }

    const int wg = warp >> 2, wq = warp & 3;
    int s = 0;
    uint32_t ph = 0;
    for (int t = blockIdx.x; t < num_tiles; t += gridDim.x) {
        const int z = t / tiles_per_split, rem = t % tiles_per_split;
        const int ty = rem / col_tiles;
        const int m0 = ty * BM, n0 = (rem % col_tiles) * BN;
        const int kc0 = z * chunks_per_split, kc1 = min(nk, kc0 + chunks_per_split);
        asm volatile("bar.sync 1, 256;" ::: "memory");
        if (threadIdx.x < 128) bias_s[threadIdx.x] = (bias != nullptr && (int)threadIdx.x < BN) ? __ldg(bias + n0 + threadIdx.x) : 0.f;
        asm volatile("bar.sync 1, 256;" ::: "memory");

        float acc[R], cor[R];
#pragma unroll
        for (int i = 0; i < R; ++i) { acc[i] = 0.f; cor[i] = 0.f; }
        int prev_s = -1;
        for (int kc = kc0; kc < kc1; ++kc) {
            mbar_wait(&split_full[s], ph);
            const uint32_t st = smem_u32(smem + s * STAGE);
            const uint64_t a_hi = make_desc(st + wg * (TILE_A / 2)), a_lo = make_desc(st + TILE_A + wg * (TILE_A / 2));
            const uint64_t b_hi = make_desc(st + 2 * TILE_A), b_lo = make_desc(st + 2 * TILE_A + TILE_B);
            wgmma_fence();
#pragma unroll
            for (int kk = 0; kk < KC / 8; ++kk) {
                const uint64_t adv = (uint64_t)(kk * 2);
                const uint32_t accum = (kc == kc0 && kk == 0) ? 0u : 1u;
                wgmma_tf32<BNI>(acc, a_hi + adv, b_hi + adv, accum);
                wgmma_tf32<BNI>(cor, a_hi + adv, b_lo + adv, accum);
                wgmma_tf32<BNI>(cor, a_lo + adv, b_hi + adv, 1u);
            }
            wgmma_commit();
            wgmma_wait<1>();
            if (prev_s >= 0) { __syncwarp(); if (lane == 0) mbar_arrive(&empty[prev_s]); }
            prev_s = s;
            if (++s == NSTAGE) { s = 0; ph ^= 1u; }
        }
        wgmma_wait<0>();
        reg_fence(acc);
        reg_fence(cor);
        if (prev_s >= 0) { __syncwarp(); if (lane == 0) mbar_arrive(&empty[prev_s]); }

        const int r0 = m0 + wg * 64 + wq * 16 + (lane >> 2);
        const int c0 = 2 * (lane & 3);
        float rs[2];
#pragma unroll
        for (int h = 0; h < 2; ++h) rs[h] = (row_scale != nullptr && r0 + 8 * h < M) ? row_scale[r0 + 8 * h] : 1.0f;
        if (splitk_out != nullptr) {
#pragma unroll
            for (int j = 0; j < BNI / 8; ++j)
#pragma unroll
                for (int h = 0; h < 2; ++h) {
                    const int m = r0 + 8 * h, col = 8 * j + c0;
                    if (m < M && col < BN)
                        *reinterpret_cast<float2*>(splitk_out + ((long long)z * M + m) * N + n0 + col) =
                            make_float2(acc[4 * j + 2 * h] + cor[4 * j + 2 * h], acc[4 * j + 2 * h + 1] + cor[4 * j + 2 * h + 1]);
                }
            continue;
        }
        const bool vec2 = ((ldy & 1) == 0) && ((reinterpret_cast<uintptr_t>(Y) & 7) == 0);
#pragma unroll
        for (int j = 0; j < BNI / 8; ++j) {
            const int col = 8 * j + c0;
            float o[4];
#pragma unroll
            for (int e = 0; e < 4; ++e) {
                float v = (acc[4 * j + e] + cor[4 * j + e]) * rs[e >> 1] + bias_s[col + (e & 1)];
                if (relu) v = fmaxf(v, 0.f);
                o[e] = v;
            }
#pragma unroll
            for (int h = 0; h < 2; ++h) {
                const int m = r0 + 8 * h;
                if (m < M && col < BN) {
                    float* yp = Y + (long long)m * ldy + n0 + col;
                    if (vec2) *reinterpret_cast<float2*>(yp) = make_float2(o[2 * h], o[2 * h + 1]);
                    else { yp[0] = o[2 * h]; yp[1] = o[2 * h + 1]; }
                }
            }
            if (gn.groups > 0) {
                const bool ok0 = r0 < M && col < BN, ok1 = r0 + 8 < M && col < BN;
                float a0 = (ok0 ? o[0] : 0.f) + (ok1 ? o[2] : 0.f), a1 = (ok0 ? o[1] : 0.f) + (ok1 ? o[3] : 0.f);
                float q0 = (ok0 ? o[0] * o[0] : 0.f) + (ok1 ? o[2] * o[2] : 0.f);
                float q1 = (ok0 ? o[1] * o[1] : 0.f) + (ok1 ? o[3] * o[3] : 0.f);
#pragma unroll
                for (int off = 4; off < 32; off <<= 1) {
                    a0 += __shfl_xor_sync(0xffffffffu, a0, off);
                    a1 += __shfl_xor_sync(0xffffffffu, a1, off);
                    q0 += __shfl_xor_sync(0xffffffffu, q0, off);
                    q1 += __shfl_xor_sync(0xffffffffu, q1, off);
                }
                if (lane < 4) {
                    gn_sm[warp * 128 + col] = make_float2(a0, q0);
                    gn_sm[warp * 128 + col + 1] = make_float2(a1, q1);
                }
            }
        }
        if (gn.groups > 0) {
            asm volatile("bar.sync 1, 256;" ::: "memory");
            const int sw = gn.slot_width, slots_tile = BN / sw, slots_total = N / sw;
            const int et = threadIdx.x;
            if (et < slots_tile) {
                double s1 = 0.0, s2 = 0.0;
                for (int w = 0; w < 8; ++w) {
                    float f1 = 0.f, f2 = 0.f;
                    for (int c = 0; c < sw; ++c) {
                        const float2 p = gn_sm[w * 128 + et * sw + c];
                        f1 += p.x;
                        f2 += p.y;
                    }
                    s1 += (double)f1;
                    s2 += (double)f2;
                }
                double* dst = gn.partial + ((long long)ty * slots_total + n0 / sw + et) * 2;
                dst[0] = s1;
                dst[1] = s2;
            }
        }
    }
}

__global__ void __launch_bounds__(256) splitk_reduce_kernel(const float* __restrict__ P, int splits, long long MN, int N,
                                                            const float* __restrict__ bias, const float* __restrict__ row_scale,
                                                            float* __restrict__ Y, int ldy, int relu) {
    const long long i4 = ((long long)blockIdx.x * blockDim.x + threadIdx.x) * 4;
    if (i4 >= MN) return;
    float4 a = *reinterpret_cast<const float4*>(P + i4);
    for (int z = 1; z < splits; ++z) {
        const float4 b = *reinterpret_cast<const float4*>(P + (long long)z * MN + i4);
        a.x += b.x; a.y += b.y; a.z += b.z; a.w += b.w;
    }
    const long long m = i4 / N;
    const int n = (int)(i4 % N);
    const float rs = row_scale != nullptr ? row_scale[m] : 1.0f;
    float o[4] = {a.x * rs, a.y * rs, a.z * rs, a.w * rs};
#pragma unroll
    for (int u = 0; u < 4; ++u) {
        if (bias != nullptr) o[u] += bias[n + u];
        if (relu) o[u] = fmaxf(o[u], 0.f);
    }
    float* y = Y + m * ldy + n;
    if ((reinterpret_cast<uintptr_t>(y) & 15) == 0) *reinterpret_cast<float4*>(y) = make_float4(o[0], o[1], o[2], o[3]);
    else { y[0] = o[0]; y[1] = o[1]; y[2] = o[2]; y[3] = o[3]; }
}

typedef CUresult (*EncodeTiledFn)(CUtensorMap*, CUtensorMapDataType, cuuint32_t, void*, const cuuint64_t*, const cuuint64_t*,
                                  const cuuint32_t*, const cuuint32_t*, CUtensorMapInterleave, CUtensorMapSwizzle,
                                  CUtensorMapL2promotion, CUtensorMapFloatOOBfill);
static EncodeTiledFn encode_fn() {
    static EncodeTiledFn fn = nullptr;
    if (fn == nullptr) {
        void* p = nullptr;
        cudaDriverEntryPointQueryResult q;
        if (cudaGetDriverEntryPoint("cuTensorMapEncodeTiled", &p, cudaEnableDefault, &q) == cudaSuccess && q == cudaDriverEntryPointSuccess)
            fn = (EncodeTiledFn)p;
    }
    return fn;
}

static int encode_map(CUtensorMap* map, const float* base, int64_t rows, int64_t cols, int64_t ld, int box_rows) {
    EncodeTiledFn fn = encode_fn();
    if (fn == nullptr) { set_error("cuTensorMapEncodeTiled entry point not available"); return -1; }
    cuuint64_t gdim[2] = {(cuuint64_t)cols, (cuuint64_t)rows};
    cuuint64_t gstride[1] = {(cuuint64_t)ld * sizeof(float)};
    cuuint32_t box[2] = {(cuuint32_t)KC, (cuuint32_t)box_rows};
    cuuint32_t estr[2] = {1, 1};
    CUresult r = fn(map, CU_TENSOR_MAP_DATA_TYPE_FLOAT32, 2, (void*)base, gdim, gstride, box, estr, CU_TENSOR_MAP_INTERLEAVE_NONE,
                    CU_TENSOR_MAP_SWIZZLE_128B, CU_TENSOR_MAP_L2_PROMOTION_L2_128B, CU_TENSOR_MAP_FLOAT_OOB_FILL_NONE);
    if (r != CUDA_SUCCESS) { set_error("cuTensorMapEncodeTiled failed with CUresult %d", (int)r); return -1; }
    return 0;
}

}

struct ProfRec { cudaEvent_t a, b; long long m, n, k; };
static std::vector<ProfRec> g_prof;
static std::mutex g_prof_mu;
static bool g_prof_on = false;
static bool g_splitk_on = true;
static bool g_persistent_on = true;

struct SplitWs { void* ptr; size_t bytes; };
static std::vector<std::pair<cudaStream_t, SplitWs>> g_split_ws;
static std::mutex g_split_mu;
static float* splitk_scratch(cudaStream_t st, size_t bytes) {
    std::lock_guard<std::mutex> lk(g_split_mu);
    for (auto& e : g_split_ws)
        if (e.first == st) {
            if (e.second.bytes >= bytes) return (float*)e.second.ptr;
            cudaFreeAsync(e.second.ptr, st);
            e.second = {nullptr, 0};
            if (cudaMallocAsync(&e.second.ptr, bytes * 2, st) != cudaSuccess) return nullptr;
            e.second.bytes = bytes * 2;
            return (float*)e.second.ptr;
        }
    SplitWs w{nullptr, 0};
    const size_t cap = bytes * 2 > (16u << 20) ? bytes * 2 : (16u << 20);
    if (cudaMallocAsync(&w.ptr, cap, st) != cudaSuccess) return nullptr;
    w.bytes = cap;
    g_split_ws.push_back({st, w});
    return (float*)w.ptr;
}

int linear_tc(const float* x, int64_t ldx, const float* w, int64_t ldw, const float* bias, const float* row_scale, float* y, int64_t ldy,
              int64_t m, int64_t n, int64_t k, int relu, cudaStream_t st, const GnFuse* gn) {
    if (m < 64 || n < 32 || (n % 16) != 0 || (k % 4) != 0 || (ldx % 4) != 0 || (ldw % 4) != 0) return 1;
    if ((reinterpret_cast<uintptr_t>(x) & 15) || (reinterpret_cast<uintptr_t>(w) & 15)) return 1;
    if (n > 128 && (n % 128) != 0) return 1;
    const int BN = (int)(n >= 128 ? 128 : n);
    CUtensorMap mx, mw;
    if (ltc::encode_map(&mx, x, m, k, ldx, ltc::BM)) return -1;
    if (ltc::encode_map(&mw, w, n, k, ldw, BN)) return -1;
    const int col_tiles = (int)(n / BN), row_tiles = (int)((m + ltc::BM - 1) / ltc::BM);
    GnFuse g{};
    if (gn != nullptr) {
        g = *gn;
        const int64_t cpg = n / g.groups;
        if (g.groups <= 0 || n % g.groups != 0 || (cpg < 32 ? (32 % cpg) != 0 : (cpg % 32) != 0 || (BN % cpg) != 0) || relu) return 1;
        g.slot_width = (int)(cpg < 32 ? cpg : 32);
    }
    const int nk = (int)((k + ltc::KC - 1) / ltc::KC);
    const int tiles = col_tiles * row_tiles;
    int splits = 1;
    if (g_splitk_on && tiles * 2 <= num_sms() && nk >= 16) {
        splits = nk / 8;
        if (splits > num_sms() / tiles) splits = num_sms() / tiles;
        if (splits > 16) splits = 16;
        if (splits < 2) splits = 1;
    }
    if (gn != nullptr && splits > 1) return 1;
    int cps = nk;
    float* part = nullptr;
    if (splits > 1) {
        cps = (nk + splits - 1) / splits;
        splits = (nk + cps - 1) / cps;
        part = splitk_scratch(st, (size_t)splits * (size_t)m * (size_t)n * sizeof(float));
        if (part == nullptr) { splits = 1; cps = nk; }
    }
    ProfRec rec{};
    const bool prof = g_prof_on;
    if (prof) {
        cudaEventCreate(&rec.a);
        cudaEventCreate(&rec.b);
        rec.m = m; rec.n = n; rec.k = k;
        cudaEventRecord(rec.a, st);
    }
    const int num_tiles = tiles * splits;
    const bool persistent = g_persistent_on && splits == 1 && tiles > num_sms();
    const unsigned grid = (unsigned)(persistent ? num_sms() : num_tiles);
    const void* kern = BN <= 32 ? (const void*)ltc::linear_tc_kernel<32> : BN <= 64 ? (const void*)ltc::linear_tc_kernel<64>
                                                                                      : (const void*)ltc::linear_tc_kernel<128>;
    if (ensure_max_smem(kern)) return -1;
#define GEOB_LTC_LAUNCH(BNI)                                                                                                  \
    ltc::linear_tc_kernel<BNI><<<grid, ltc::NTHREADS, ltc::SMEM, st>>>(mx, mw, bias, row_scale, y, (int)ldy, (int)m, (int)n, (int)k, \
                                                                       BN, relu, g, part, cps, col_tiles, row_tiles, num_tiles)
    if (BN <= 32) GEOB_LTC_LAUNCH(32);
    else if (BN <= 64) GEOB_LTC_LAUNCH(64);
    else GEOB_LTC_LAUNCH(128);
#undef GEOB_LTC_LAUNCH
    if (part != nullptr) {
        const long long mn = (long long)m * n;
        ltc::splitk_reduce_kernel<<<(unsigned)((mn / 4 + 255) / 256), 256, 0, st>>>(part, splits, mn, (int)n, bias, row_scale, y, (int)ldy, relu);
        count_launches(1);
    }
    if (prof) {
        cudaEventRecord(rec.b, st);
        std::lock_guard<std::mutex> lk(g_prof_mu);
        g_prof.push_back(rec);
    }
    GEOB_CHECK_LAUNCH();
    count_launches(1);
    return 0;
}

}

extern "C" {

int geob200_set_linear_persistent(int on) {
    geob200::g_persistent_on = on != 0;
    return 0;
}

int geob200_set_split_k(int on) {
    geob200::g_splitk_on = on != 0;
    return 0;
}

int geob200_linear_profile_enable(int on) {
    std::lock_guard<std::mutex> lk(geob200::g_prof_mu);
    for (auto& r : geob200::g_prof) { cudaEventDestroy(r.a); cudaEventDestroy(r.b); }
    geob200::g_prof.clear();
    geob200::g_prof_on = on != 0;
    return 0;
}

int64_t geob200_linear_profile_read(int64_t capacity, int64_t* shapes, float* ms) {
    std::lock_guard<std::mutex> lk(geob200::g_prof_mu);
    int64_t n = 0;
    for (auto& r : geob200::g_prof) {
        if (n >= capacity) break;
        if (cudaEventSynchronize(r.b) != cudaSuccess) break;
        float t = 0.f;
        cudaEventElapsedTime(&t, r.a, r.b);
        shapes[3 * n] = r.m; shapes[3 * n + 1] = r.n; shapes[3 * n + 2] = r.k;
        ms[n] = t;
        ++n;
    }
    return n;
}

}
```

### geotransformer_b200/csrc/native.cu

```cuda
#include "common.cuh"
#include "geob200.h"

namespace geob200 {

struct Ctx {
    Arena ar;
    void* gn_ws;
    size_t gn_ws_bytes;
    void* stream;
    int groups;
    Ctx(void* p, size_t n) : ar(p, n) {}
    float* fl(int64_t rows, int64_t ch) { return ar.take<float>((size_t)rows * (size_t)ch); }
};

#define TRY(expr)                  \
    do {                           \
        int _rc = (expr);          \
        if (_rc != 0) return _rc;  \
    } while (0)

static int run_kpconv(Ctx& c, const geob200_kpconv_t& k, const float* s_feats, const float* q_pts, const float* s_pts,
                      const int64_t* nbr, int64_t m, int64_t ns, int64_t h, float* out) {
    const bool tc = (k.c_in % 32 == 0) && (k.c_out % 16 == 0) && k.c_out >= 32 && (k.c_out <= 128 || k.c_out % 128 == 0) && m >= 64 &&
                    k.weights_t != nullptr;
    if (tc) {
        const size_t wb = geob200_kpconv_tc_workspace_bytes(m, ns, k.c_in);
        const size_t mark = c.ar.off;
        void* ws = c.ar.take<char>(wb);
        GEOB_REQUIRE(c.ar.ok(), "native: arena too small (kpconv)");
        TRY(geob200_kpconv_tc(s_feats, q_pts, s_pts, nbr, m, ns, h, k.kernel_points, 15, k.weights_t, k.bias, k.c_in, k.c_out, k.sigma,
                              out, ws, wb, c.stream));
        c.ar.off = mark;
        return 0;
    }
    const size_t wb = geob200_kpconv_workspace_bytes(ns);
    const size_t mark = c.ar.off;
    void* ws = c.ar.take<char>(wb);
    GEOB_REQUIRE(c.ar.ok(), "native: arena too small (kpconv)");
    TRY(geob200_kpconv(s_feats, q_pts, s_pts, nbr, m, ns, h, k.kernel_points, 15, k.weights, k.bias, k.c_in, k.c_out, k.sigma, out, ws,
                       wb, c.stream));
    c.ar.off = mark;
    return 0;
}

static int run_kpconv_norm(Ctx& c, const geob200_kpconv_t& k, const geob200_norm_t& n, const float* s_feats, const float* q_pts,
                           const float* s_pts, const int64_t* nbr, int64_t m, int64_t ns, int64_t h, float* out, const GnSeg* seg) {
    float* y = c.fl(m, k.c_out);
    GEOB_REQUIRE(c.ar.ok(), "native: arena too small (kpconv output)");
    const bool tc = (k.c_in % 32 == 0) && (k.c_out % 16 == 0) && k.c_out >= 32 && (k.c_out <= 128 || k.c_out % 128 == 0) && m >= 64 &&
                    k.weights_t != nullptr;
    if (tc) {
        const size_t wb = geob200_kpconv_tc_workspace_bytes(m, ns, k.c_in);
        const size_t mark = c.ar.off;
        void* ws = c.ar.take<char>(wb);
        GEOB_REQUIRE(c.ar.ok(), "native: arena too small (kpconv)");
        TRY(kpconv_group_norm_impl(s_feats, q_pts, s_pts, nbr, m, ns, h, k.kernel_points, 15, k.weights_t, k.bias, k.c_in, k.c_out,
                                   k.sigma, c.groups, n.gamma, n.beta, 1e-5f, 1, 0.1f, y, out, c.gn_ws, c.gn_ws_bytes, ws, wb, c.stream, seg));
        c.ar.off = mark;
        return 0;
    }
    TRY(run_kpconv(c, k, s_feats, q_pts, s_pts, nbr, m, ns, h, y));
    return group_norm_impl(y, m, k.c_out, c.groups, n.gamma, n.beta, 1e-5f, nullptr, 1, 0.1f, out, c.gn_ws, c.gn_ws_bytes, c.stream, seg);
}

static int run_unary(Ctx& c, const geob200_linear_t& l, const geob200_norm_t& n, const float* x, int64_t rows, const float* residual,
                     int leaky, float* out, const GnSeg* seg) {
    float* t = c.fl(rows, l.c_out);
    GEOB_REQUIRE(c.ar.ok(), "native: arena too small (unary)");
    TRY(linear_group_norm_impl(x, l.c_in, l.weight, l.bias, rows, l.c_out, l.c_in, c.groups, n.gamma, n.beta, 1e-5f, residual, leaky,
                               0.1f, t, out, c.gn_ws, c.gn_ws_bytes, c.stream, seg));
    return 0;
}

static int run_resblock(Ctx& c, const geob200_resblock_t& b, const float* feats, int64_t ns, const float* q_pts, const float* s_pts,
                        const int64_t* nbr, int64_t m, int64_t h, float* out, const GnSeg* seg_s, const GnSeg* seg_q,
                        const int* cloud_max = nullptr) {
    const float* x = feats;
    if (b.has_unary1) {
        float* u = c.fl(ns, b.unary1.c_out);
        TRY(run_unary(c, b.unary1, b.norm1, feats, ns, nullptr, 1, u, seg_s));
        x = u;
    }
    float* yn = c.fl(m, b.conv.c_out);
    GEOB_REQUIRE(c.ar.ok(), "native: arena too small (resblock)");
    TRY(run_kpconv_norm(c, b.conv, b.norm_conv, x, q_pts, s_pts, nbr, m, ns, h, yn, seg_q));
    const float* sc = feats;
    if (b.strided) {
        float* mp = c.fl(m, b.c_in);
        GEOB_REQUIRE(c.ar.ok(), "native: arena too small (maxpool)");
        if (seg_q != nullptr && cloud_max != nullptr) {
            TRY(maxpool_seg(feats, nbr, m, ns, h, b.c_in, mp, seg_q, cloud_max, c.stream));
        } else {
            TRY(geob200_maxpool(feats, nbr, m, ns, h, b.c_in, mp, c.stream));
        }
        sc = mp;
    }
    if (b.has_shortcut) {
        float* s2 = c.fl(m, b.shortcut.c_out);
        TRY(run_unary(c, b.shortcut, b.norm_sc, sc, m, nullptr, 0, s2, seg_q));
        sc = s2;
    }
    return run_unary(c, b.unary2, b.norm2, yn, m, sc, 1, out, seg_q);
}

}

using namespace geob200;

extern "C" {

size_t geob200_backbone_workspace_bytes(const geob200_backbone_t* net, const int64_t* level_rows) {
    size_t total = 1 << 20;
    for (int l = 0; l < net->num_stages; ++l) {
        const size_t rows = (size_t)level_rows[l];
        const size_t ch = (size_t)net->init_dim << (l + 1);
        total += rows * ch * 4 * 24;
        total += geob200_kpconv_tc_workspace_bytes(level_rows[l], l > 0 ? level_rows[l - 1] : level_rows[l], (int64_t)(ch / 2)) + 4096;
    }
    return total;
}

int geob200_backbone_forward(const geob200_backbone_t* net, const float* feats, const float* const* points, const int64_t* level_rows,
                             const int64_t* const* neighbors, const int64_t* neighbor_width, const int64_t* const* subsampling,
                             const int64_t* subsampling_width, const int64_t* const* upsampling, const int64_t* upsampling_width,
                             float* const* out_feats , void* gn_workspace,
                             size_t gn_workspace_bytes, void* workspace, size_t workspace_bytes, void* stream) {
    return geob200_backbone_forward_batched(net, feats, points, level_rows, neighbors, neighbor_width, subsampling, subsampling_width,
                                            upsampling, upsampling_width, out_feats, gn_workspace, gn_workspace_bytes, workspace,
                                            workspace_bytes, stream, 1, nullptr, nullptr);
}

size_t geob200_backbone_gn_workspace_bytes(const geob200_backbone_t* net, const int64_t* level_rows, int64_t n_pairs) {
    return fused_group_norm_workspace_bytes_batched(level_rows[0], (int64_t)net->init_dim << net->num_stages, net->groups, n_pairs);
}

int geob200_backbone_forward_batched(const geob200_backbone_t* net, const float* feats, const float* const* points,
                                     const int64_t* level_rows, const int64_t* const* neighbors, const int64_t* neighbor_width,
                                     const int64_t* const* subsampling, const int64_t* subsampling_width,
                                     const int64_t* const* upsampling, const int64_t* upsampling_width, float* const* out_feats,
                                     void* gn_workspace, size_t gn_workspace_bytes, void* workspace, size_t workspace_bytes, void* stream,
                                     int64_t n_pairs, const int64_t* const* cloud_rows_h, const int32_t* const* sub_cloud_max) {
    GEOB_REQUIRE(n_pairs == 1 || sub_cloud_max != nullptr, "backbone: batched execution needs the per-cloud subsampling widths");
    GEOB_REQUIRE(net->num_stages >= 2 && net->num_stages <= GEOB200_MAX_STAGES, "backbone: num_stages out of range");
    GEOB_REQUIRE(n_pairs >= 1 && 2 * n_pairs <= GEOB_MAX_CLOUDS, "backbone: 1 <= pairs per batch <= %d", GEOB_MAX_CLOUDS / 2);
    GEOB_REQUIRE(n_pairs == 1 || cloud_rows_h != nullptr, "backbone: batched execution needs the per-cloud row counts of every level");
    Ctx c(workspace, workspace_bytes);
    c.gn_ws = gn_workspace; c.gn_ws_bytes = gn_workspace_bytes; c.stream = stream; c.groups = net->groups;
    const int S = net->num_stages;
    GnSeg segs[GEOB200_MAX_STAGES];
    const GnSeg* sg[GEOB200_MAX_STAGES];
    for (int l = 0; l < S; ++l) {
        sg[l] = nullptr;
        if (n_pairs > 1) {
            GnSeg& g = segs[l];
            g.n_pairs = (int)n_pairs; g.n_clouds = (int)(2 * n_pairs); g.start[0] = 0;
            for (int cl = 0; cl < g.n_clouds; ++cl) g.start[cl + 1] = g.start[cl] + (int)cloud_rows_h[l][cl];
            GEOB_REQUIRE(g.start[g.n_clouds] == level_rows[l], "backbone: cloud rows of level %d do not add up", l);
            sg[l] = &g;
        }
    }
    const float* enc[GEOB200_MAX_STAGES];
    int64_t enc_ch[GEOB200_MAX_STAGES];
    {
        const int64_t n0 = level_rows[0];
        float* yn = c.fl(n0, net->conv1.c_out);
        GEOB_REQUIRE(c.ar.ok(), "native: arena too small (encoder1_1)");
        TRY(run_kpconv_norm(c, net->conv1, net->norm1, feats, points[0], points[0], neighbors[0], n0, n0, neighbor_width[0], yn, sg[0]));
        const geob200_resblock_t& b = net->blocks[0];
        float* o = c.fl(n0, b.unary2.c_out);
        TRY(run_resblock(c, b, yn, n0, points[0], points[0], neighbors[0], n0, neighbor_width[0], o, sg[0], sg[0]));
        enc[0] = o; enc_ch[0] = b.unary2.c_out;
    }
    int bi = 1;
    for (int lvl = 1; lvl < S; ++lvl) {
        const int64_t m = level_rows[lvl], ns = level_rows[lvl - 1];
        const geob200_resblock_t& b1 = net->blocks[bi++];
        float* o1 = c.fl(m, b1.unary2.c_out);
        TRY(run_resblock(c, b1, enc[lvl - 1], ns, points[lvl], points[lvl - 1], subsampling[lvl - 1], m, subsampling_width[lvl - 1], o1,
                         sg[lvl - 1], sg[lvl], sub_cloud_max != nullptr ? sub_cloud_max[lvl - 1] : nullptr));
        const geob200_resblock_t& b2 = net->blocks[bi++];
        float* o2 = c.fl(m, b2.unary2.c_out);
        TRY(run_resblock(c, b2, o1, m, points[lvl], points[lvl], neighbors[lvl], m, neighbor_width[lvl], o2, sg[lvl], sg[lvl]));
        const geob200_resblock_t& b3 = net->blocks[bi++];
        float* o3 = (lvl == S - 1) ? out_feats[0] : c.fl(m, b3.unary2.c_out);
        TRY(run_resblock(c, b3, o2, m, points[lvl], points[lvl], neighbors[lvl], m, neighbor_width[lvl], o3, sg[lvl], sg[lvl]));
        enc[lvl] = o3; enc_ch[lvl] = b3.unary2.c_out;
    }
    const float* latent = enc[S - 1];
    int64_t latent_ch = enc_ch[S - 1];
    int oi = 1;
    for (int lvl = S - 1; lvl >= net->finest_decoder; --lvl) {
        const int64_t m = level_rows[lvl - 1], ns = level_rows[lvl];
        const int64_t c2 = enc_ch[lvl - 1];
        float* cat = c.fl(m, latent_ch + c2);
        GEOB_REQUIRE(c.ar.ok(), "native: arena too small (decoder)");
        TRY(geob200_upsample_concat(latent, upsampling[lvl - 1], upsampling_width[lvl - 1], ns, enc[lvl - 1], m, latent_ch, c2, cat, stream));
        const geob200_linear_t& l = net->decoders[S - 1 - lvl];
        float* o = out_feats[oi++];
        if (lvl == net->finest_decoder) {
            TRY(geob200_linear(cat, l.c_in, l.weight, l.bias, o, l.c_out, m, l.c_out, l.c_in, 0, stream));
        } else {
            TRY(run_unary(c, l, net->decoder_norms[S - 1 - lvl], cat, m, nullptr, 1, o, sg[lvl - 1]));
        }
        latent = o; latent_ch = l.c_out;
    }
    GEOB_REQUIRE(c.ar.ok(), "native: arena too small");
    return 0;
}


size_t geob200_transformer_workspace_bytes(int64_t n0, int64_t n1, int64_t channels, int64_t heads, int64_t num_layers) {
    const int64_t rows[2] = {n0, n1};
    return geob200_transformer_batched_workspace_bytes(1, rows, channels, heads, num_layers);
}

static int run_tail(Ctx& c, const geob200_tlayer_t& L, const float* hidden, const float* inp, int64_t rows, int64_t ch, float* out) {
    float* h = c.fl(rows, ch);
    float* x = c.fl(rows, ch);
    float* y1 = c.fl(rows, 2 * ch);
    float* y2 = c.fl(rows, ch);
    GEOB_REQUIRE(c.ar.ok(), "native: arena too small (transformer tail)");
    TRY(geob200_linear(hidden, ch, L.att_linear.weight, L.att_linear.bias, h, ch, rows, ch, ch, 0, c.stream));
    TRY(geob200_add_layernorm(h, inp, L.att_norm.gamma, L.att_norm.beta, rows, ch, 1e-5f, x, c.stream));
    TRY(geob200_linear(x, ch, L.expand.weight, L.expand.bias, y1, 2 * ch, rows, 2 * ch, ch, 1, c.stream));
    TRY(geob200_linear(y1, 2 * ch, L.squeeze.weight, L.squeeze.bias, y2, ch, rows, ch, 2 * ch, 0, c.stream));
    TRY(geob200_add_layernorm(x, y2, L.out_norm.gamma, L.out_norm.beta, rows, ch, 1e-5f, out, c.stream));
    return 0;
}

int geob200_transformer_forward(const geob200_tlayer_t* layers, int64_t num_layers, int64_t channels, int64_t heads, const float* x_in,
                                int64_t n0, int64_t n1, const float* emb0, const float* emb1, float* out, void* workspace,
                                size_t workspace_bytes, void* stream) {
    const int64_t rows[2] = {n0, n1};
    const float* embs[2] = {emb0, emb1};
    return geob200_transformer_forward_batched(layers, num_layers, channels, heads, x_in, 1, rows, embs, out, workspace, workspace_bytes, stream);
}

size_t geob200_transformer_batched_workspace_bytes(int64_t n_pairs, const int64_t* cloud_rows_h, int64_t channels, int64_t heads,
                                                   int64_t num_layers) {
    size_t n = 0, att = 0;
    for (int64_t c = 0; c < 2 * n_pairs; ++c) {
        n += (size_t)cloud_rows_h[c];
        const size_t other = (size_t)cloud_rows_h[(c + n_pairs) % (2 * n_pairs)];
        const size_t m = (size_t)cloud_rows_h[c] > other ? (size_t)cloud_rows_h[c] : other;
        att += align_up((size_t)cloud_rows_h[c] * m * (size_t)heads * 4, 256);
    }
    return (n * (size_t)channels * 4 * (3 + 1 + (size_t)heads + 12)) * (size_t)(num_layers + 1) + att + (2 << 20);
}

int geob200_transformer_forward_batched(const geob200_tlayer_t* layers, int64_t num_layers, int64_t channels, int64_t heads,
                                        const float* x_in, int64_t n_pairs, const int64_t* cloud_rows_h, const float* const* embeddings,
                                        float* out, void* workspace, size_t workspace_bytes, void* stream) {
    GEOB_REQUIRE(n_pairs >= 1 && 2 * n_pairs <= GEOB_MAX_CLOUDS, "transformer: 1 <= pairs per batch <= %d", GEOB_MAX_CLOUDS / 2);
    Ctx c(workspace, workspace_bytes);
    c.stream = stream;
    const int64_t C = channels, H = heads, B = n_pairs, NC = 2 * n_pairs;
    int64_t off[GEOB_MAX_CLOUDS + 1];
    off[0] = 0;
    for (int64_t i = 0; i < NC; ++i) off[i + 1] = off[i] + cloud_rows_h[i];
    const int64_t n = off[NC], R = off[B];
    const float* x = x_in;
    geob200_att_item_t items[GEOB_MAX_CLOUDS];
    size_t att_ws_bytes = 0;
    {
        for (int64_t i = 0; i < NC; ++i) { items[i].n_query = cloud_rows_h[i]; items[i].n_key = cloud_rows_h[i]; }
        att_ws_bytes = geob200_attention_batched_workspace_bytes(items, NC, H);
        for (int64_t p = 0; p < B; ++p) { items[p].n_query = cloud_rows_h[p]; items[p].n_key = cloud_rows_h[B + p]; }
        const size_t cross = geob200_attention_batched_workspace_bytes(items, B, H);
        if (cross > att_ws_bytes) att_ws_bytes = cross;
    }
    void* att_ws = c.fl((int64_t)(att_ws_bytes / 4 + 1), 1);
    for (int64_t i = 0; i < num_layers; ++i) {
        const geob200_tlayer_t& L = layers[i];
        float* y = (i == num_layers - 1) ? out : c.fl(n, C);
        if (L.is_self) {
            float* qkv = c.fl(n, 3 * C);
            float* qp = c.fl(n, H * C);
            float* qb = c.fl(n, H);
            float* hidden = c.fl(n, C);
            GEOB_REQUIRE(c.ar.ok(), "native: arena too small (self layer)");
            TRY(geob200_linear(x, C, L.w_qkv, L.b_qkv, qkv, 3 * C, n, 3 * C, C, 0, stream));
            const int64_t d = C / H;
            TRY(geob200_linear_batched(qkv, 3 * C, d, L.wp_t, C, d, nullptr, 0, qp, H * C, C, n, C, d, H, 0, stream));
            TRY(geob200_head_bias(qkv, 3 * C, L.bp, n, C, H, qb, stream));
            for (int64_t cl = 0; cl < NC; ++cl) {
                const int64_t o = off[cl];
                items[cl] = geob200_att_item_t{qkv + o * 3 * C, qkv + o * 3 * C + C, qkv + o * 3 * C + 2 * C, qp + o * H * C, qb + o * H,
                                               embeddings[cl], hidden + o * C, cloud_rows_h[cl], cloud_rows_h[cl]};
            }
            TRY(geob200_attention_batched(items, NC, 3 * C, 3 * C, 3 * C, C, C, H, att_ws, att_ws_bytes, stream));
            TRY(run_tail(c, L, hidden, x, n, C, y));
        } else {
            const int64_t Sn = n - R;
            float* q0 = c.fl(R, C);
            float* kv1 = c.fl(Sn, 2 * C);
            float* hid0 = c.fl(R, C);
            float* q1 = c.fl(Sn, C);
            float* kv0 = c.fl(R, 2 * C);
            float* hid1 = c.fl(Sn, C);
            GEOB_REQUIRE(c.ar.ok(), "native: arena too small (cross layer)");
            TRY(geob200_linear(x, C, L.w_q, L.b_q, q0, C, R, C, C, 0, stream));
            TRY(geob200_linear(x + R * C, C, L.w_kv, L.b_kv, kv1, 2 * C, Sn, 2 * C, C, 0, stream));
            for (int64_t p = 0; p < B; ++p) {
                const int64_t ro = off[p], so = off[B + p] - R;
                items[p] = geob200_att_item_t{q0 + ro * C, kv1 + so * 2 * C, kv1 + so * 2 * C + C, nullptr, nullptr, nullptr, hid0 + ro * C,
                                              cloud_rows_h[p], cloud_rows_h[B + p]};
            }
            TRY(geob200_attention_batched(items, B, C, 2 * C, 2 * C, C, C, H, att_ws, att_ws_bytes, stream));
            TRY(run_tail(c, L, hid0, x, R, C, y));
            TRY(geob200_linear(x + R * C, C, L.w_q, L.b_q, q1, C, Sn, C, C, 0, stream));
            TRY(geob200_linear(y, C, L.w_kv, L.b_kv, kv0, 2 * C, R, 2 * C, C, 0, stream));
            for (int64_t p = 0; p < B; ++p) {
                const int64_t ro = off[p], so = off[B + p] - R;
                items[p] = geob200_att_item_t{q1 + so * C, kv0 + ro * 2 * C, kv0 + ro * 2 * C + C, nullptr, nullptr, nullptr, hid1 + so * C,
                                              cloud_rows_h[B + p], cloud_rows_h[p]};
            }
            TRY(geob200_attention_batched(items, B, C, 2 * C, 2 * C, C, C, H, att_ws, att_ws_bytes, stream));
            TRY(run_tail(c, L, hid1, x + R * C, Sn, C, y + R * C));
        }
        x = y;
    }
    return 0;
}

}
```

### geotransformer_b200/functional.py

```python
import ctypes
import math

import torch

from . import _lib as L

_f32, _i64, _u8, _i32 = torch.float32, torch.int64, torch.uint8, torch.int32

GSE_MODE = int(__import__('os').environ.get('GEOB200_GSE_MODE', '5'))
GSE_TABLE_INV_STEP = int(__import__('os').environ.get('GEOB200_GSE_TABLE_INV_STEP', '256'))
GSE_TABLE_D_MAX = float(__import__('os').environ.get('GEOB200_GSE_TABLE_D_MAX', '96'))

EVENTS = None


class _timed:
    def __init__(self, name):
        self.name = name

    def __enter__(self):
        if EVENTS is not None:
            self.s = torch.cuda.Event(enable_timing=True)
            self.e = torch.cuda.Event(enable_timing=True)
            self.s.record()
        return self

    def __exit__(self, *a):
        if EVENTS is not None:
            self.e.record()
            EVENTS.setdefault(self.name, []).append((self.s, self.e))
        return False


def _f(t, name):
    L.require_cuda(t, name, _f32)
    return t


def _detach(t):
    return t.detach() if t is not None and t.requires_grad else t


_GN_WS = {}


def _gn_workspace(device, groups, rows=0, channels=0, n_pairs=1):
    key = (device.index, L.stream_ptr(), groups)
    lib = L.lib()
    need = lib.geob200_fused_group_norm_workspace_bytes(rows, channels, groups) if rows else lib.geob200_group_norm_workspace_bytes(groups)
    need += 8 * groups * max(int(n_pairs), 1) + 1024
    ws = _GN_WS.get(key)
    if ws is None or ws.numel() < need:
        ws = torch.zeros(max(int(need * 1.5), 1 << 20), dtype=_u8, device=device)
        _GN_WS[key] = ws
    return ws



KPCONV_MODE = 'tc'


def kpconv(s_feats, q_points, s_points, neighbor_indices, kernel_points, weights, bias, sigma, weights_t=None):
    s_feats, weights, bias = _detach(s_feats), _detach(weights), _detach(bias)
    _f(s_feats, 's_feats'); _f(q_points, 'q_points'); _f(s_points, 's_points')
    L.require_cuda(neighbor_indices, 'neighbor_indices', _i64)
    m, h = neighbor_indices.shape
    ns = s_points.shape[0]
    k, cin, cout = weights.shape
    out = torch.empty((m, cout), dtype=_f32, device=s_feats.device)
    lib = L.lib()
    if (KPCONV_MODE == 'tc' and cin % 32 == 0 and cout % 16 == 0 and cout >= 32 and (cout <= 128 or cout % 128 == 0) and m >= 64):
        if weights_t is None:
            weights_t = weights.reshape(k * cin, cout).t().contiguous()
        ws = L.workspace(lib.geob200_kpconv_tc_workspace_bytes(m, ns, cin), s_feats.device, 'kpconv_tc')
        L.check(lib.geob200_kpconv_tc(s_feats.data_ptr(), q_points.data_ptr(), s_points.data_ptr(), neighbor_indices.data_ptr(), m, ns,
                                      h, kernel_points.data_ptr(), k, weights_t.data_ptr(), L.ptr(bias), cin, cout, float(sigma),
                                      out.data_ptr(), ws.data_ptr(), ws.numel(), L.stream_ptr()), 'kpconv_tc')
        return out
    ws = L.workspace(lib.geob200_kpconv_workspace_bytes(ns), s_feats.device, 'kpconv')
    L.check(lib.geob200_kpconv(s_feats.data_ptr(), q_points.data_ptr(), s_points.data_ptr(),
                               neighbor_indices.data_ptr(), m, ns, h, kernel_points.data_ptr(), k,
                               weights.data_ptr(), L.ptr(bias), cin, cout, float(sigma), out.data_ptr(),
                               ws.data_ptr(), ws.numel(), L.stream_ptr()), 'kpconv')
    return out


def linear(x, weight, bias=None, relu=False, out=None):
    x, weight, bias = _detach(x), _detach(weight), _detach(bias)
    if not x.is_cuda or x.dtype != _f32 or x.stride(1) != 1:
        raise RuntimeError('linear: x must be a float32 CUDA tensor with unit inner stride')
    L.require_cuda(weight, 'weight', _f32)
    m, k = x.shape
    n = weight.shape[0]
    if out is None:
        out = torch.empty((m, n), dtype=_f32, device=x.device)
    L.check(L.lib().geob200_linear(x.data_ptr(), x.stride(0), weight.data_ptr(), L.ptr(bias), out.data_ptr(),
                                   out.stride(0), m, n, k, int(relu), L.stream_ptr()), 'linear')
    return out


def group_norm(x, weight, bias, groups, eps=1e-5, negative_slope=None, residual=None):
    x, weight, bias = _detach(x), _detach(weight), _detach(bias)
    _f(x, 'x')
    n, c = x.shape
    ws = _gn_workspace(x.device, groups)
    y = torch.empty_like(x)
    L.check(L.lib().geob200_group_norm(x.data_ptr(), n, c, groups, weight.data_ptr(), bias.data_ptr(), float(eps),
                                       L.ptr(residual), int(negative_slope is not None),
                                       float(negative_slope or 0.0), y.data_ptr(), ws.data_ptr(), ws.numel(),
                                       L.stream_ptr()), 'group_norm')
    return y


def linear_group_norm(x, weight, bias, gn_weight, gn_bias, groups, eps=1e-5, negative_slope=None, residual=None):
    x, weight, bias, gn_weight, gn_bias = _detach(x), _detach(weight), _detach(bias), _detach(gn_weight), _detach(gn_bias)
    if not x.is_cuda or x.dtype != _f32 or x.stride(1) != 1:
        raise RuntimeError('linear_group_norm: x must be a float32 CUDA tensor with unit inner stride')
    L.require_cuda(weight, 'weight', _f32)
    m, k = x.shape
    n = weight.shape[0]
    pre = scratch((m, n), x.device, 'pre_norm')
    y = torch.empty((m, n), dtype=_f32, device=x.device)
    ws = _gn_workspace(x.device, groups, m, n)
    L.check(L.lib().geob200_linear_group_norm(x.data_ptr(), x.stride(0), weight.data_ptr(), L.ptr(bias), m, n, k, groups,
                                              gn_weight.data_ptr(), gn_bias.data_ptr(), float(eps), L.ptr(residual),
                                              int(negative_slope is not None), float(negative_slope or 0.0), pre.data_ptr(),
                                              y.data_ptr(), ws.data_ptr(), ws.numel(), L.stream_ptr()), 'linear_group_norm')
    return y


def kpconv_group_norm(s_feats, q_points, s_points, neighbor_indices, kernel_points, weights, bias, sigma, gn_weight, gn_bias, groups,
                      eps=1e-5, negative_slope=0.1, weights_t=None):
    m, h = neighbor_indices.shape
    k, cin, cout = weights.shape
    if not (KPCONV_MODE == 'tc' and cin % 32 == 0 and cout % 16 == 0 and cout >= 32 and (cout <= 128 or cout % 128 == 0) and m >= 64):
        x = kpconv(s_feats, q_points, s_points, neighbor_indices, kernel_points, weights, bias, sigma, weights_t=weights_t)
        return group_norm(x, gn_weight, gn_bias, groups, eps, negative_slope=negative_slope)
    s_feats, weights, bias, gn_weight, gn_bias = _detach(s_feats), _detach(weights), _detach(bias), _detach(gn_weight), _detach(gn_bias)
    _f(s_feats, 's_feats'); _f(q_points, 'q_points'); _f(s_points, 's_points')
    L.require_cuda(neighbor_indices, 'neighbor_indices', _i64)
    ns = s_points.shape[0]
    dev = s_feats.device
    if weights_t is None:
        weights_t = weights.reshape(k * cin, cout).t().contiguous()
    lib = L.lib()
    pre = scratch((m, cout), dev, 'pre_norm')
    y = torch.empty((m, cout), dtype=_f32, device=dev)
    gws = _gn_workspace(dev, groups, m, cout)
    ws = L.workspace(lib.geob200_kpconv_tc_workspace_bytes(m, ns, cin), dev, 'kpconv_tc')
    L.check(lib.geob200_kpconv_group_norm(s_feats.data_ptr(), q_points.data_ptr(), s_points.data_ptr(), neighbor_indices.data_ptr(),
                                          m, ns, h, kernel_points.data_ptr(), k, weights_t.data_ptr(), L.ptr(bias), cin, cout,
                                          float(sigma), groups, gn_weight.data_ptr(), gn_bias.data_ptr(), float(eps),
                                          int(negative_slope is not None), float(negative_slope or 0.0), pre.data_ptr(),
                                          y.data_ptr(), gws.data_ptr(), gws.numel(), ws.data_ptr(), ws.numel(), L.stream_ptr()),
            'kpconv_group_norm')
    return y


def _cloud_rows(cloud_rows):
    import ctypes
    return (ctypes.c_int64 * len(cloud_rows))(*[int(r) for r in cloud_rows])


def group_norm_batched(x, weight, bias, groups, cloud_rows, eps=1e-5, negative_slope=None, residual=None):
    x, weight, bias = _detach(x), _detach(weight), _detach(bias)
    _f(x, 'x')
    n, c = x.shape
    np_ = len(cloud_rows) // 2
    ws = _gn_workspace(x.device, groups, n, c, n_pairs=np_)
    y = torch.empty_like(x)
    L.check(L.lib().geob200_group_norm_batched(x.data_ptr(), n, c, groups, weight.data_ptr(), bias.data_ptr(), float(eps), L.ptr(residual),
                                               int(negative_slope is not None), float(negative_slope or 0.0), y.data_ptr(), ws.data_ptr(),
                                               ws.numel(), L.stream_ptr(), np_, _cloud_rows(cloud_rows)), 'group_norm_batched')
    return y


def linear_group_norm_batched(x, weight, bias, gn_weight, gn_bias, groups, cloud_rows, eps=1e-5, negative_slope=None, residual=None):
    x, weight, bias, gn_weight, gn_bias = _detach(x), _detach(weight), _detach(bias), _detach(gn_weight), _detach(gn_bias)
    m, k = x.shape
    n = weight.shape[0]
    np_ = len(cloud_rows) // 2
    pre = scratch((m, n), x.device, 'pre_norm')
    y = torch.empty((m, n), dtype=_f32, device=x.device)
    ws = _gn_workspace(x.device, groups, m, n, n_pairs=np_)
    L.check(L.lib().geob200_linear_group_norm_batched(x.data_ptr(), x.stride(0), weight.data_ptr(), L.ptr(bias), m, n, k, groups,
                                                      gn_weight.data_ptr(), gn_bias.data_ptr(), float(eps), L.ptr(residual),
                                                      int(negative_slope is not None), float(negative_slope or 0.0), pre.data_ptr(),
                                                      y.data_ptr(), ws.data_ptr(), ws.numel(), L.stream_ptr(), np_, _cloud_rows(cloud_rows)),
            'linear_group_norm_batched')
    return y


def maxpool(x, neighbor_indices):
    x = _detach(x)
    _f(x, 'x'); L.require_cuda(neighbor_indices, 'neighbor_indices', _i64)
    m, h = neighbor_indices.shape
    y = torch.empty((m, x.shape[1]), dtype=_f32, device=x.device)
    L.check(L.lib().geob200_maxpool(x.data_ptr(), neighbor_indices.data_ptr(), m, x.shape[0], h, x.shape[1],
                                    y.data_ptr(), L.stream_ptr()), 'maxpool')
    return y


def upsample_concat(x, upsample_indices, skip=None):
    x = _detach(x)
    _f(x, 'x')
    if not upsample_indices.is_cuda or upsample_indices.dtype != _i64:
        raise RuntimeError('upsample_indices must be an int64 CUDA tensor')
    m = upsample_indices.shape[0]
    stride = upsample_indices.stride(0) if upsample_indices.ndim == 2 else 1
    c1 = x.shape[1]
    c2 = 0 if skip is None else skip.shape[1]
    y = torch.empty((m, c1 + c2), dtype=_f32, device=x.device)
    L.check(L.lib().geob200_upsample_concat(x.data_ptr(), upsample_indices.data_ptr(), stride, x.shape[0],
                                            L.ptr(skip), m, c1, c2, y.data_ptr(), L.stream_ptr()), 'upsample_concat')
    return y


def nearest_upsample(x, upsample_indices):
    return upsample_concat(x, upsample_indices, None)



def point_to_node_partition(points, nodes, point_limit, return_count=False):
    _f(points, 'points'); _f(nodes, 'nodes')
    n, m = points.shape[0], nodes.shape[0]
    dev = points.device
    p2n = torch.empty((n,), dtype=_i64, device=dev)
    node_masks = torch.empty((m,), dtype=torch.bool, device=dev)
    node_sizes = torch.empty((m,), dtype=_i32, device=dev)
    knn = torch.empty((m, point_limit), dtype=_i64, device=dev)
    knn_masks = torch.empty((m, point_limit), dtype=torch.bool, device=dev)
    L.check(L.lib().geob200_point_to_node_partition(points.data_ptr(), n, nodes.data_ptr(), m, point_limit,
                                                    p2n.data_ptr(), node_masks.data_ptr(), node_sizes.data_ptr(),
                                                    knn.data_ptr(), knn_masks.data_ptr(), None,
                                                    L.stream_ptr()), 'point_to_node_partition')
    if return_count:
        return p2n, node_sizes.long(), node_masks, knn, knn_masks
    return p2n, node_masks, knn, knn_masks


def knn_partition(points, nodes, k, return_distance=False):
    _f(points, 'points'); _f(nodes, 'nodes')
    n, m = points.shape[0], nodes.shape[0]
    k = min(int(k), n)
    idx = torch.empty((m, k), dtype=_i64, device=points.device)
    d2 = torch.empty((m, k), dtype=_f32, device=points.device) if return_distance else None
    L.check(L.lib().geob200_knn_partition(points.data_ptr(), n, nodes.data_ptr(), m, k, idx.data_ptr(), L.ptr(d2), L.stream_ptr()),
            'knn_partition')
    if return_distance:
        return d2.sqrt_(), idx
    return idx


def pairwise_distance(x, y, normalized=False, channel_first=False):
    if channel_first:
        x, y = x.transpose(-1, -2), y.transpose(-1, -2)
    if x.ndim == 3:
        return torch.stack([pairwise_distance(a, b, normalized) for a, b in zip(x, y)])
    x, y = x.contiguous(), y.contiguous()
    _f(x, 'x'); _f(y, 'y')
    if x.ndim != 2 or y.ndim != 2 or x.shape[1] != y.shape[1]:
        raise RuntimeError('pairwise_distance: x (N, C) and y (M, C) expected')
    out = torch.empty((x.shape[0], y.shape[0]), dtype=_f32, device=x.device)
    L.check(L.lib().geob200_pairwise_distance(x.data_ptr(), x.shape[0], y.data_ptr(), y.shape[0], x.shape[1], int(normalized),
                                              out.data_ptr(), L.stream_ptr()), 'pairwise_distance')
    return out


def point_to_node_indices(points, nodes, return_counts=False):
    _f(points, 'points'); _f(nodes, 'nodes')
    idx = torch.empty((points.shape[0],), dtype=_i64, device=points.device)
    sizes = torch.empty((nodes.shape[0],), dtype=_i32, device=points.device) if return_counts else None
    L.check(L.lib().geob200_point_to_node_indices(points.data_ptr(), points.shape[0], nodes.data_ptr(), nodes.shape[0], idx.data_ptr(),
                                                  L.ptr(sizes), L.stream_ptr()), 'get_point_to_node_indices')
    return (idx, sizes.long()) if return_counts else idx


def apply_transform(points, transform):
    _f(transform, 'transform')
    p = points.reshape(-1, 3).contiguous()
    _f(p, 'points')
    out = torch.empty_like(p)
    L.check(L.lib().geob200_apply_transform(p.data_ptr(), p.shape[0], transform.data_ptr(), out.data_ptr(), L.stream_ptr()),
            'apply_transform')
    return out.reshape(points.shape)


def gather_rows(table, indices):
    table = _detach(table)
    _f(table, 'table'); L.require_cuda(indices, 'indices', _i64)
    c = table.shape[1]
    out = torch.empty((*indices.shape, c), dtype=_f32, device=table.device)
    L.check(L.lib().geob200_gather_rows(table.data_ptr(), table.shape[0], c, indices.data_ptr(), indices.numel(),
                                        out.data_ptr(), L.stream_ptr()), 'gather_rows')
    return out



def gse_indices(points, sigma_d, sigma_a, angle_k, out=None):
    _f(points, 'points')
    n = points.shape[0]
    if out is not None:
        d, a = out[0].view(n, n), out[1].view(n, n, angle_k)
    else:
        d = torch.empty((n, n), dtype=_f32, device=points.device)
        a = torch.empty((n, n, angle_k), dtype=_f32, device=points.device)
    factor_a = 180.0 / (sigma_a * math.pi)
    L.check(L.lib().geob200_gse_indices(points.data_ptr(), n, float(sigma_d), float(factor_a), angle_k, d.data_ptr(),
                                        a.data_ptr(), L.stream_ptr()), 'gse_indices')
    return d, a


def gse_indices_batched(points, cloud_rows, sigma_d, sigma_a, angle_k, d_out, a_out):
    _f(points, 'points')
    factor_a = 180.0 / (sigma_a * math.pi)
    L.check(L.lib().geob200_gse_indices_batched(points.data_ptr(), len(cloud_rows), _cloud_rows(cloud_rows), float(sigma_d), float(factor_a),
                                                angle_k, d_out.data_ptr(), a_out.data_ptr(), L.stream_ptr()), 'gse_indices_batched')
    return d_out, a_out


def scratch(shape, device, tag):
    numel = 1
    for s in shape:
        numel *= int(s)
    key = (device.index if device.index is not None else torch.cuda.current_device(), L.stream_ptr(), tag)
    buf = _SCRATCH.get(key)
    if buf is None or buf.numel() < numel:
        buf = torch.empty(int(numel * 1.3) + 1024, dtype=_f32, device=device)
        _SCRATCH[key] = buf
    return buf[:numel].view(*shape)


_SCRATCH = {}
_ARANGE = {}


def scratch_arange(n, device, tag='arange'):
    key = device.index if device.index is not None else torch.cuda.current_device()
    buf = _ARANGE.get(key)
    if buf is None or buf.numel() < n:
        buf = torch.arange(max(int(n) * 2, 4096), dtype=_i64, device=device)
        torch.cuda.current_stream(device).synchronize()
        _ARANGE[key] = buf
    return buf[:n]


class GseTable:
    __slots__ = ('blob', 'channels', 'inv_step', 'd_max', 'a_max')

    def __init__(self, blob, channels, inv_step, d_max, a_max):
        self.blob, self.channels, self.inv_step, self.d_max, self.a_max = blob, channels, inv_step, d_max, a_max


def gse_table(div_term, wd_t, wa_t, bd, ba, sigma_a, inv_step=None, d_max=None):
    for t, name in ((div_term, 'div_term'), (wd_t, 'wd_t'), (wa_t, 'wa_t'), (bd, 'bd'), (ba, 'ba')):
        L.require_cuda(t, name, _f32)
    c = int(wd_t.shape[0])
    inv_step = GSE_TABLE_INV_STEP if inv_step is None else int(inv_step)
    d_max = GSE_TABLE_D_MAX if d_max is None else float(d_max)
    a_max = 180.0 / float(sigma_a) + 0.25
    lib = L.lib()
    nbytes = lib.geob200_gse_table_bytes(c, inv_step, d_max, a_max)
    if nbytes == 0:
        raise RuntimeError(f'gse_table: bad grid (channels {c}, inv_step {inv_step}, d_max {d_max}, a_max {a_max})')
    blob = torch.empty(nbytes, dtype=_u8, device=wd_t.device)
    L.check(lib.geob200_gse_table_build(div_term.data_ptr(), wd_t.data_ptr(), wa_t.data_ptr(), bd.data_ptr(), ba.data_ptr(), c,
                                        inv_step, d_max, a_max, blob.data_ptr(), nbytes, L.stream_ptr()), 'gse_table_build')
    torch.cuda.current_stream(wd_t.device).synchronize()
    return GseTable(blob, c, inv_step, d_max, a_max)


def _gse_embed_table(d_indices, a_indices, n_rows, div_term, wd, wa, bd, ba, table, out):
    c = wd.shape[0]
    if table is None or table.channels != c:
        raise RuntimeError('gse_embed mode 5 (tabulated projections) needs the GseTable of these weights (functional.gse_table)')
    with _timed('gse_embed'):
        L.check(L.lib().geob200_gse_embed_table(d_indices.data_ptr(), a_indices.data_ptr(), int(n_rows), c, table.blob.data_ptr(),
                                                table.blob.numel(), table.inv_step, table.d_max, table.a_max, div_term.data_ptr(),
                                                wd.data_ptr(), wa.data_ptr(), bd.data_ptr(), ba.data_ptr(), out.data_ptr(),
                                                L.stream_ptr()), 'gse_embed_table')
    return out


def _gse_mode(mode, table):
    if mode is not None:
        return mode
    return 3 if (GSE_MODE == 5 and table is None) else GSE_MODE


def gse_embed_flat(d_indices, a_indices, n_rows, div_term, wd, wa, bd, ba, wd_t, wa_t, out, mode=None, table=None):
    c = wd.shape[0]
    mode = _gse_mode(mode, table)
    if mode == 5 and c in (128, 256):
        return _gse_embed_table(d_indices, a_indices, n_rows, div_term, wd, wa, bd, ba, table, out)
    if c == 128 and mode != 0:
        mode = 3
    elif c != 256:
        mode = 0
    lib = L.lib()
    ws = L.workspace(lib.geob200_gse_embed_workspace_bytes(1, c), d_indices.device, 'gse')
# ... 369 lines not shown
```

### geotransformer_b200/native.py

```python
import ctypes

import torch

from . import _lib as L
from . import functional as GF

MAX_STAGES = 6
P, I64, I32, F32 = ctypes.c_void_p, ctypes.c_int64, ctypes.c_int32, ctypes.c_float


class LinearT(ctypes.Structure):
    _fields_ = [('weight', P), ('bias', P), ('c_in', I64), ('c_out', I64)]


class NormT(ctypes.Structure):
    _fields_ = [('gamma', P), ('beta', P)]


class KPConvT(ctypes.Structure):
    _fields_ = [('weights', P), ('weights_t', P), ('bias', P), ('kernel_points', P), ('c_in', I64), ('c_out', I64), ('sigma', F32)]


class ResBlockT(ctypes.Structure):
    _fields_ = [('has_unary1', I32), ('has_shortcut', I32), ('strided', I32), ('reserved', I32), ('c_in', I64),
                ('unary1', LinearT), ('norm1', NormT), ('conv', KPConvT), ('norm_conv', NormT), ('unary2', LinearT), ('norm2', NormT),
                ('shortcut', LinearT), ('norm_sc', NormT)]


class BackboneT(ctypes.Structure):
    _fields_ = [('num_stages', I32), ('finest_decoder', I32), ('groups', I32), ('init_dim', I32), ('conv1', KPConvT), ('norm1', NormT),
                ('blocks', ResBlockT * (1 + 3 * (MAX_STAGES - 1))), ('decoders', LinearT * MAX_STAGES), ('decoder_norms', NormT * MAX_STAGES)]


class TLayerT(ctypes.Structure):
    _fields_ = [('is_self', I32), ('reserved', I32), ('w_qkv', P), ('b_qkv', P), ('w_q', P), ('b_q', P), ('w_kv', P), ('b_kv', P),
                ('wp_t', P), ('bp', P), ('att_linear', LinearT), ('att_norm', NormT), ('expand', LinearT), ('squeeze', LinearT),
                ('out_norm', NormT)]


def _ptr(t):
    return None if t is None else t.data_ptr()


class NativeModel:

    def __init__(self, model):
        self.model = model
        self._keep = []
        self.device = next(model.parameters()).device
        self.backbone = self._build_backbone(model.backbone)
        self.layers, self.num_layers = self._build_transformer(model.transformer.transformer)
        self.hidden = model.transformer.in_proj.out_features
        self.heads = model.transformer.transformer.layers[0].attention.attention.num_heads

    def _lin(self, mlp):
        return LinearT(_ptr(mlp.weight), _ptr(mlp.bias), mlp.in_features, mlp.out_features)

    def _norm(self, gn):
        return NormT(_ptr(gn.norm.weight), _ptr(gn.norm.bias))

    def _kp(self, kp):
        w = kp.weights.detach()
        wt = w.reshape(-1, w.shape[2]).t().contiguous() if w.shape[1] % 32 == 0 else None
        if wt is not None:
            self._keep.append(wt)
        return KPConvT(_ptr(w), _ptr(wt), _ptr(kp.bias), _ptr(kp.kernel_points), w.shape[1], w.shape[2], float(kp.sigma))

    def _res(self, blk):
        r = ResBlockT()
        r.c_in, r.strided = blk.in_channels, int(blk.strided)
        r.has_unary1 = int(not isinstance(blk.unary1, torch.nn.Identity))
        if r.has_unary1:
            r.unary1, r.norm1 = self._lin(blk.unary1.mlp), self._norm(blk.unary1.norm)
        r.conv, r.norm_conv = self._kp(blk.KPConv), self._norm(blk.norm_conv)
        r.unary2, r.norm2 = self._lin(blk.unary2.mlp), self._norm(blk.unary2.norm)
        r.has_shortcut = int(not isinstance(blk.unary_shortcut, torch.nn.Identity))
        if r.has_shortcut:
            r.shortcut, r.norm_sc = self._lin(blk.unary_shortcut.mlp), self._norm(blk.unary_shortcut.norm)
        return r

    def _build_backbone(self, bb):
        b = BackboneT()
        b.num_stages, b.finest_decoder = bb.num_stages, bb.finest_decoder
        b.groups = bb.encoder1_1.norm.num_groups
        b.init_dim = bb.encoder1_1.out_channels
        b.conv1, b.norm1 = self._kp(bb.encoder1_1.KPConv), self._norm(bb.encoder1_1.norm)
        b.blocks[0] = self._res(bb.encoder1_2)
        i = 1
        for lvl in range(2, bb.num_stages + 1):
            for j in (1, 2, 3):
                b.blocks[i] = self._res(getattr(bb, f'encoder{lvl}_{j}'))
                i += 1
        for d, lvl in enumerate(range(bb.num_stages - 1, bb.finest_decoder - 1, -1)):
            dec = getattr(bb, f'decoder{lvl}')
            b.decoders[d] = self._lin(dec.mlp)
            if lvl != bb.finest_decoder:
                b.decoder_norms[d] = self._norm(dec.norm)
        self._dec_channels = [getattr(bb, f'decoder{lvl}').mlp.out_features
                              for lvl in range(bb.num_stages - 1, bb.finest_decoder - 1, -1)]
        self._coarse_channels = getattr(bb, f'encoder{bb.num_stages}_3').out_channels
        return b

    def _build_transformer(self, tr):
        arr = (TLayerT * len(tr.layers))()
        for i, (blk, layer) in enumerate(zip(tr.blocks, tr.layers)):
            mha = layer.attention.attention
            t = TLayerT()
            t.is_self = int(blk == 'self')
            cat = lambda names, attr: torch.cat([getattr(getattr(mha, n), attr).detach() for n in names], dim=0).contiguous()
            if t.is_self:
                wqkv, bqkv = cat(('proj_q', 'proj_k', 'proj_v'), 'weight'), cat(('proj_q', 'proj_k', 'proj_v'), 'bias')
                wpt = mha.proj_p.weight.detach().t().contiguous()
                self._keep += [wqkv, bqkv, wpt]
                t.w_qkv, t.b_qkv, t.wp_t, t.bp = _ptr(wqkv), _ptr(bqkv), _ptr(wpt), _ptr(mha.proj_p.bias)
            else:
                wkv, bkv = cat(('proj_k', 'proj_v'), 'weight'), cat(('proj_k', 'proj_v'), 'bias')
                self._keep += [wkv, bkv]
                t.w_q, t.b_q, t.w_kv, t.b_kv = _ptr(mha.proj_q.weight), _ptr(mha.proj_q.bias), _ptr(wkv), _ptr(bkv)
            att, ffn = layer.attention, layer.output
            t.att_linear = LinearT(_ptr(att.linear.weight), _ptr(att.linear.bias), att.linear.in_features, att.linear.out_features)
            t.att_norm = NormT(_ptr(att.norm.weight), _ptr(att.norm.bias))
            t.expand = LinearT(_ptr(ffn.expand.weight), _ptr(ffn.expand.bias), ffn.expand.in_features, ffn.expand.out_features)
            t.squeeze = LinearT(_ptr(ffn.squeeze.weight), _ptr(ffn.squeeze.bias), ffn.squeeze.in_features, ffn.squeeze.out_features)
            t.out_norm = NormT(_ptr(ffn.norm.weight), _ptr(ffn.norm.bias))
            arr[i] = t
        return arr, len(tr.layers)

    def backbone_forward(self, feats, data_dict):
        lib = L.lib()
        S = self.backbone.num_stages
        pts, nb, sub, up = data_dict['points'], data_dict['neighbors'], data_dict['subsampling'], data_dict['upsampling']
        dev = feats.device
        rows = (I64 * S)(*[p.shape[0] for p in pts])
        parr = (P * S)(*[p.data_ptr() for p in pts])
        narr, nw = (P * S)(*[t.data_ptr() for t in nb]), (I64 * S)(*[t.shape[1] for t in nb])
        sarr, sw = (P * S)(*[t.data_ptr() for t in sub]), (I64 * S)(*[t.shape[1] for t in sub])
        uarr, uw = (P * S)(*[t.data_ptr() for t in up]), (I64 * S)(*[t.shape[1] for t in up])
        outs = [torch.empty((pts[-1].shape[0], self._coarse_channels), dtype=torch.float32, device=dev)]
        for d, lvl in enumerate(range(S - 1, self.backbone.finest_decoder - 1, -1)):
            outs.append(torch.empty((pts[lvl - 1].shape[0], self._dec_channels[d]), dtype=torch.float32, device=dev))
        oarr = (P * len(outs))(*[o.data_ptr() for o in outs])
        ws_bytes = lib.geob200_backbone_workspace_bytes(ctypes.byref(self.backbone), rows)
        ws = L.workspace(ws_bytes, dev, 'native_backbone')
        n_pairs = int(data_dict.get('batch_size', 1))
        gn = GF._gn_workspace(dev, self.backbone.groups, pts[0].shape[0], self.backbone.init_dim << S, n_pairs=n_pairs)
        if n_pairs > 1:
            lens = data_dict['lengths_host']
            keep = [(I64 * (2 * n_pairs))(*[int(v) for v in lens[l]]) for l in range(S)]
            carr = (P * S)(*[ctypes.cast(k, P).value for k in keep])
            cmax = torch.empty((S - 1, 2 * n_pairs), dtype=torch.int32, device=dev)
            for l in range(S - 1):
                L.check(lib.geob200_cloud_max_count(sub[l].data_ptr(), sub[l].shape[0], pts[l].shape[0], sub[l].shape[1], n_pairs, keep[l + 1],
                                                    cmax[l].data_ptr(), L.stream_ptr()), 'cloud_max_count')
            marr = (P * S)(*([cmax[l].data_ptr() for l in range(S - 1)] + [None]))
            L.check(lib.geob200_backbone_forward_batched(ctypes.byref(self.backbone), feats.data_ptr(), parr, rows, narr, nw, sarr, sw,
                                                         uarr, uw, oarr, gn.data_ptr(), gn.numel(), ws.data_ptr(), ws.numel(),
                                                         L.stream_ptr(), n_pairs, carr, marr), 'backbone_forward_batched')
        else:
            L.check(lib.geob200_backbone_forward(ctypes.byref(self.backbone), feats.data_ptr(), parr, rows, narr, nw, sarr, sw, uarr, uw,
                                                 oarr, gn.data_ptr(), gn.numel(), ws.data_ptr(), ws.numel(), L.stream_ptr()),
                    'backbone_forward')
        outs.reverse()
        return outs

    def transformer_forward_batched(self, x, cloud_rows, embeddings):
        lib = L.lib()
        nc = len(cloud_rows)
        rows = (I64 * nc)(*[int(r) for r in cloud_rows])
        earr = (P * nc)(*[e.data_ptr() for e in embeddings])
        out = torch.empty_like(x)
        ws_bytes = lib.geob200_transformer_batched_workspace_bytes(nc // 2, rows, self.hidden, self.heads, self.num_layers)
        ws = L.workspace(ws_bytes, x.device, 'native_transformer')
        L.check(lib.geob200_transformer_forward_batched(self.layers, self.num_layers, self.hidden, self.heads, x.data_ptr(), nc // 2, rows,
                                                        earr, out.data_ptr(), ws.data_ptr(), ws.numel(), L.stream_ptr()),
                'transformer_forward_batched')
        return out

    def transformer_forward(self, x, n0, emb0, emb1):
        lib = L.lib()
        n1 = x.shape[0] - n0
        out = torch.empty_like(x)
        ws_bytes = lib.geob200_transformer_workspace_bytes(n0, n1, self.hidden, self.heads, self.num_layers)
        ws = L.workspace(ws_bytes, x.device, 'native_transformer')
        L.check(lib.geob200_transformer_forward(self.layers, self.num_layers, self.hidden, self.heads, x.data_ptr(), n0, n1, emb0.data_ptr(),
                                                emb1.data_ptr(), out.data_ptr(), ws.data_ptr(), ws.numel(), L.stream_ptr()),
                'transformer_forward')
        return out
```

### include/geob200.h

```cpp
#ifndef GEOB200_H
#define GEOB200_H

#include <stddef.h>
#include <stdint.h>

#ifdef __cplusplus
extern "C" {
#endif

const char* geob200_last_error(void);
uint64_t geob200_launch_count(void);


size_t geob200_grid_subsample_workspace_bytes(int64_t n_points, int64_t batch);
int geob200_grid_subsample(const float* points, int64_t n_points, const int64_t* lengths_h, int64_t batch, float voxel,
                           float* s_points, int64_t* s_lengths, void* workspace, size_t workspace_bytes, void* stream);

size_t geob200_radius_search_workspace_bytes(int64_t n_query, int64_t n_support, int64_t batch);
int geob200_radius_search(const float* q_points, int64_t n_query, const float* s_points, int64_t n_support,
                          const int64_t* q_lengths_h, const int64_t* s_lengths_h, int64_t batch, float radius,
                          int64_t width, int64_t* out, int32_t* counts, int32_t* max_count, void* workspace,
                          size_t workspace_bytes, void* stream);

int geob200_neighbor_histogram(const int64_t* neighbors, int64_t n_rows, int64_t width, int64_t n_support, int64_t hist_n,
                               int32_t* hist, void* stream);


size_t geob200_kpconv_workspace_bytes(int64_t n_support);
int geob200_kpconv(const float* s_feats, const float* q_points, const float* s_points, const int64_t* neighbors,
                   int64_t n_query, int64_t n_support, int64_t n_neighbors, const float* kernel_points, int64_t n_kernel,
                   const float* weights, const float* bias, int64_t c_in, int64_t c_out, float sigma, float* out,
                   void* workspace, size_t workspace_bytes, void* stream);

size_t geob200_kpconv_tc_workspace_bytes(int64_t n_query, int64_t n_support, int64_t c_in);
int geob200_kpconv_tc(const float* s_feats, const float* q_points, const float* s_points, const int64_t* neighbors, int64_t n_query,
                      int64_t n_support, int64_t n_neighbors, const float* kernel_points, int64_t n_kernel, const float* weights_t,
                      const float* bias, int64_t c_in, int64_t c_out, float sigma, float* out, void* workspace, size_t workspace_bytes,
                      void* stream);

void geob200_set_linear_mode(int mode);
int geob200_linear(const float* x, int64_t ldx, const float* weight, const float* bias, float* y, int64_t ldy, int64_t m,
                   int64_t n, int64_t k, int relu, void* stream);
int geob200_linear_batched(const float* x, int64_t ldx, int64_t stride_x, const float* weight, int64_t ldw, int64_t stride_w,
                           const float* bias, int64_t stride_b, float* y, int64_t ldy, int64_t stride_y, int64_t m, int64_t n,
                           int64_t k, int64_t batch, int relu, void* stream);

size_t geob200_group_norm_workspace_bytes(int64_t groups);
int geob200_group_norm(const float* x, int64_t n_rows, int64_t channels, int64_t groups, const float* gamma,
                       const float* beta, float eps, const float* residual, int leaky, float slope, float* y,
                       void* workspace, size_t workspace_bytes, void* stream);

size_t geob200_fused_group_norm_workspace_bytes(int64_t n_rows, int64_t channels, int64_t groups);
int geob200_linear_group_norm(const float* x, int64_t ldx, const float* weight, const float* bias, int64_t m, int64_t n, int64_t k,
                              int64_t groups, const float* gamma, const float* beta, float eps, const float* residual, int leaky,
                              float slope, float* pre_norm, float* y, void* workspace, size_t workspace_bytes, void* stream);
size_t geob200_kpconv_group_norm_workspace_bytes(int64_t n_query, int64_t n_support, int64_t c_in, int64_t c_out, int64_t groups);
int geob200_kpconv_group_norm(const float* s_feats, const float* q_points, const float* s_points, const int64_t* neighbors,
                              int64_t n_query, int64_t n_support, int64_t n_neighbors, const float* kernel_points, int64_t n_kernel,
                              const float* weights_t, const float* bias, int64_t c_in, int64_t c_out, float sigma, int64_t groups,
                              const float* gamma, const float* beta, float eps, int leaky, float slope, float* pre_norm, float* y,
                              void* gn_workspace, size_t gn_workspace_bytes, void* workspace, size_t workspace_bytes, void* stream);

size_t geob200_group_norm_batched_workspace_bytes(int64_t n_rows, int64_t channels, int64_t groups, int64_t n_pairs);
int geob200_group_norm_batched(const float* x, int64_t n_rows, int64_t channels, int64_t groups, const float* gamma, const float* beta,
                               float eps, const float* residual, int leaky, float slope, float* y, void* workspace, size_t workspace_bytes,
                               void* stream, int64_t n_pairs, const int64_t* cloud_rows_h);
int geob200_linear_group_norm_batched(const float* x, int64_t ldx, const float* weight, const float* bias, int64_t m, int64_t n, int64_t k,
                                      int64_t groups, const float* gamma, const float* beta, float eps, const float* residual, int leaky,
                                      float slope, float* pre_norm, float* y, void* workspace, size_t workspace_bytes, void* stream,
                                      int64_t n_pairs, const int64_t* cloud_rows_h);

int geob200_maxpool(const float* x, const int64_t* neighbors, int64_t n_query, int64_t n_support, int64_t n_neighbors,
                    int64_t channels, float* y, void* stream);

int geob200_cloud_max_count(const int64_t* neighbors, int64_t n_query, int64_t n_support, int64_t n_neighbors, int64_t n_pairs,
                            const int64_t* cloud_rows_h, int32_t* cloud_max, void* stream);
int geob200_maxpool_batched(const float* x, const int64_t* neighbors, int64_t n_query, int64_t n_support, int64_t n_neighbors,
                            int64_t channels, float* y, int64_t n_pairs, const int64_t* cloud_rows_h, const int32_t* cloud_max,
                            void* stream);

int geob200_upsample_concat(const float* x, const int64_t* up_indices, int64_t up_stride, int64_t n_support,
                            const float* skip, int64_t n_query, int64_t c1, int64_t c2, float* y, void* stream);


int geob200_point_to_node_partition(const float* points, int64_t n_points, const float* nodes, int64_t n_nodes,
                                    int64_t point_limit, int64_t* point_to_node, uint8_t* node_masks, int32_t* node_sizes,
                                    int64_t* node_knn_indices, uint8_t* node_knn_masks, int32_t* status, void* stream);

int geob200_point_to_node_partition_batched(const float* points, const float* nodes, int64_t n_clouds, const int64_t* cloud_points,
                                            const int64_t* cloud_nodes, int64_t point_limit, int64_t* point_to_node, uint8_t* node_masks,
                                            int32_t* node_sizes, int64_t* node_knn_indices, uint8_t* node_knn_masks, void* stream);

int geob200_knn_partition(const float* points, int64_t n_points, const float* nodes, int64_t n_nodes, int64_t k,
                          int64_t* knn_indices, float* knn_sq_distances, void* stream);
int geob200_pairwise_distance(const float* x, int64_t n, const float* y, int64_t m, int64_t channels, int normalized, float* out,
                              void* stream);
int geob200_point_to_node_indices(const float* points, int64_t n_points, const float* nodes, int64_t n_nodes, int64_t* indices,
                                  int32_t* node_sizes, void* stream);
int geob200_apply_transform(const float* points, int64_t n_points, const float* transform, float* out, void* stream);

int geob200_gather_rows(const float* table, int64_t n_rows, int64_t channels, const int64_t* indices, int64_t n_indices,
                        float* out, void* stream);


int geob200_gse_indices(const float* points, int64_t n, float sigma_d, float factor_a, int64_t angle_k, float* d_indices,
                        float* a_indices, void* stream);

int geob200_gse_indices_batched(const float* points, int64_t n_clouds, const int64_t* cloud_rows_h, float sigma_d, float factor_a,
                                int64_t angle_k, float* d_indices, float* a_indices, void* stream);

size_t geob200_gse_embed_workspace_bytes(int64_t n, int64_t channels);
int geob200_gse_embed(const float* d_indices, const float* a_indices, int64_t n, int64_t channels, const float* div_term,
                      const float* wd_t, const float* wa_t, const float* wd, const float* wa, const float* bd, const float* ba,
                      float* embeddings, int mode, void* workspace, size_t workspace_bytes, void* stream);

int geob200_gse_embed_pairs(const float* d_indices, const float* a_indices, int64_t n_rows, int64_t channels, const float* div_term,
                            const float* wd_t, const float* wa_t, const float* wd, const float* wa, const float* bd, const float* ba,
                            float* embeddings, int mode, void* workspace, size_t workspace_bytes, void* stream);

size_t geob200_gse_table_bytes(int64_t channels, int64_t inv_step, float d_max, float a_max);
int geob200_gse_table_build(const float* div_term, const float* wd_t, const float* wa_t, const float* bd, const float* ba,
                            int64_t channels, int64_t inv_step, float d_max, float a_max, void* table, size_t table_bytes,
                            void* stream);
int geob200_gse_embed_table(const float* d_indices, const float* a_indices, int64_t n_rows, int64_t channels, const void* table,
                            size_t table_bytes, int64_t inv_step, float d_max, float a_max, const float* div_term, const float* wd,
                            const float* wa, const float* bd, const float* ba, float* embeddings, void* stream);

size_t geob200_attention_workspace_bytes(int64_t n_query, int64_t n_key, int64_t heads);
int geob200_attention(const float* q, int64_t ldq, const float* k, int64_t ldk, const float* v, int64_t ldv, const float* qp,
                      const float* qb, const float* embed, int64_t n_query, int64_t n_key, int64_t channels, int64_t heads,
                      float* out, int64_t ldo, void* workspace, size_t workspace_bytes, void* stream);
typedef struct { const float* q; const float* k; const float* v; const float* qp; const float* qb; const float* embed; float* out;
                 int64_t n_query, n_key; } geob200_att_item_t;
size_t geob200_attention_batched_workspace_bytes(const geob200_att_item_t* items_h, int64_t n_items, int64_t heads);
int geob200_attention_batched(const geob200_att_item_t* items_h, int64_t n_items, int64_t ldq, int64_t ldk, int64_t ldv, int64_t ldo,
                              int64_t channels, int64_t heads, void* workspace, size_t workspace_bytes, void* stream);
int geob200_set_attention_tma(int on);
int geob200_head_bias(const float* q, int64_t ldq, const float* bias_p, int64_t n, int64_t channels, int64_t heads, float* qb,
                      void* stream);
int geob200_add_layernorm(const float* a, const float* b, const float* gamma, const float* beta, int64_t n, int64_t channels,
                          float eps, float* y, void* stream);
int geob200_l2_normalize(const float* x, int64_t n, int64_t channels, float* y, void* stream);


size_t geob200_superpoint_matching_workspace_bytes(int64_t n_ref, int64_t n_src);
int geob200_superpoint_matching(const float* ref_feats, const float* src_feats, int64_t n_ref, int64_t n_src, int64_t channels,
                                const uint8_t* ref_masks, const uint8_t* src_masks, int64_t num_correspondences, int dual,
                                int64_t* ref_corr_indices, int64_t* src_corr_indices, float* corr_scores, int32_t* num_out,
                                void* workspace, size_t workspace_bytes, void* stream);
size_t geob200_superpoint_matching_batched_workspace_bytes(int64_t n_rows, int64_t n_products, int64_t n_pairs);
int geob200_superpoint_matching_batched(const float* feats, int64_t channels, const uint8_t* masks, int64_t n_pairs,
                                        const int64_t* cloud_nodes, int64_t num_correspondences, int dual, int64_t* corr_indices,
                                        float* corr_scores, int32_t* num_out, void* workspace, size_t workspace_bytes, void* stream);

int geob200_gather_patches(const int64_t* corr_indices, int64_t n_corr, const int64_t* node_knn_indices,
                           const uint8_t* node_knn_masks, int64_t k, const float* points, int64_t n_points,
                           int64_t* out_indices, uint8_t* out_masks, float* out_points, void* stream);
int geob200_gather_patches_batched(const int64_t* corr_indices, int64_t n_corr, int64_t n_clouds, const int64_t* cloud_nodes,
                                   const int64_t* cloud_points, const int64_t* node_knn_indices, const uint8_t* node_knn_masks, int64_t k,
                                   const float* points, int64_t* out_indices, uint8_t* out_masks, float* out_points, void* stream);

int geob200_patch_scores(const float* ref_feats, int64_t n_ref, const float* src_feats, int64_t n_src, int64_t channels,
                         const int64_t* ref_knn_indices, const int64_t* src_knn_indices, int64_t n_patches, int64_t k,
                         float* scores, void* stream);
int geob200_patch_scores_batched(const float* feats, int64_t channels, int64_t n_pairs, const int64_t* cloud_points,
                                 const int64_t* ref_knn_indices, const int64_t* src_knn_indices, int64_t n_patches, int64_t k,
                                 float* scores, void* stream);

int geob200_sinkhorn(const float* scores, const uint8_t* row_masks, const uint8_t* col_masks, const float* alpha,
                     int64_t n_patches, int64_t k, int64_t num_iterations, float inf, float* out, void* stream);


size_t geob200_lgr_workspace_bytes(int64_t n_patches, int64_t k, int64_t topk);
int geob200_local_global_registration(const float* ref_knn_points, const float* src_knn_points, const uint8_t* ref_knn_masks,
                                      const uint8_t* src_knn_masks, const float* log_scores, int64_t n_patches, int64_t k,
                                      int64_t score_ld, int64_t topk, float acceptance_radius, int mutual,
                                      float confidence_threshold, int64_t correspondence_threshold, int64_t num_refinement_steps,
                                      float* ref_corr_points, float* src_corr_points, float* corr_scores, int32_t* corr_patch,
                                      int32_t* num_corr, float* estimated_transform, float* patch_transforms, int32_t* patch_inliers,
                                      int32_t* best_patch, void* workspace, size_t workspace_bytes, void* stream);
size_t geob200_lgr_batched_workspace_bytes(int64_t n_pairs, int64_t n_patches, int64_t k, int64_t topk);
int geob200_local_global_registration_batched(const float* ref_knn_points, const float* src_knn_points, const uint8_t* ref_knn_masks,
                                              const uint8_t* src_knn_masks, const float* log_scores, int64_t n_pairs, int64_t n_patches,
                                              int64_t k, int64_t score_ld, int64_t topk, float acceptance_radius, int mutual,
                                              float confidence_threshold, int64_t correspondence_threshold, int64_t num_refinement_steps,
                                              float* ref_corr_points, float* src_corr_points, float* corr_scores, int32_t* corr_patch,
                                              int32_t* num_corr, float* estimated_transform, int64_t transform_ld, float* patch_transforms,
                                              int32_t* patch_inliers, int32_t* best_patch, void* workspace, size_t workspace_bytes,
                                              void* stream);

int geob200_weighted_procrustes(const float* src_points, const float* ref_points, const float* weights, int64_t batch,
                                int64_t n, float weight_thresh, float eps, float* transforms, void* stream);

size_t geob200_node_correspondences_workspace_bytes(int64_t n_ref, int64_t n_src, int64_t k);
int geob200_node_correspondences(const float* ref_nodes, const float* src_nodes, const float* ref_knn_points,
                                 const float* src_knn_points, const uint8_t* ref_masks, const uint8_t* src_masks,
                                 const uint8_t* ref_knn_masks, const uint8_t* src_knn_masks, int64_t n_ref, int64_t n_src,
                                 int64_t k, const float* transform, float pos_radius, int64_t* corr_indices,
                                 float* corr_overlaps, int32_t* count, void* workspace, size_t workspace_bytes, void* stream);
size_t geob200_node_correspondences_batched_workspace_bytes(int64_t n_rows, int64_t n_products, int64_t k);
int geob200_node_correspondences_batched(const float* nodes, const float* knn_points, const uint8_t* node_masks, const uint8_t* knn_masks,
                                         int64_t n_pairs, const int64_t* cloud_nodes, int64_t k, const float* transforms, float pos_radius,
                                         int64_t* corr_indices, float* corr_overlaps, int32_t* count, void* workspace, size_t workspace_bytes,
                                         void* stream);

int geob200_evaluate(const int64_t* gt_node_corr_indices, const float* gt_node_corr_overlaps, int64_t n_gt,
                     float acceptance_overlap, const int64_t* ref_node_corr_indices, const int64_t* src_node_corr_indices,
                     int64_t n_node_corr, const float* ref_corr_points, const float* src_corr_points, int64_t n_corr,
                     float acceptance_radius, const float* gt_transform, const float* est_transform, const float* src_points,
                     int64_t n_src_points, int mode, float rmse_threshold, float rre_threshold, float rte_threshold,
                     float* metrics, void* stream);

int geob200_evaluate_counts(const int64_t* gt_node_corr_indices, const float* gt_node_corr_overlaps, int64_t n_gt, const int32_t* n_gt_dev,
                            float acceptance_overlap, const int64_t* ref_node_corr_indices, const int64_t* src_node_corr_indices,
                            int64_t n_node_corr, const int32_t* n_node_corr_dev, const float* ref_corr_points, const float* src_corr_points,
                            int64_t n_corr, const int32_t* n_corr_dev, float acceptance_radius, const float* gt_transform,
                            const float* est_transform, const float* src_points, int64_t n_src_points, int mode, float rmse_threshold,
                            float rre_threshold, float rte_threshold, float* metrics, void* stream);
int geob200_evaluate_batched(const int64_t* gt_node_corr_indices, const float* gt_node_corr_overlaps, const int32_t* n_gt_dev,
                             float acceptance_overlap, const int64_t* ref_node_corr_indices, const int64_t* src_node_corr_indices,
                             int64_t n_node_corr, const int32_t* n_node_corr_dev, const float* ref_corr_points, const float* src_corr_points,
                             int64_t n_corr, const int32_t* n_corr_dev, float acceptance_radius, const float* gt_transforms,
                             const float* est_transforms, int64_t transform_ld, const float* points, int64_t n_pairs, const int64_t* cloud_nodes,
                             const int64_t* cloud_points, int mode, float rmse_threshold, float rre_threshold, float rte_threshold,
                             float* metrics, int64_t metrics_ld, void* stream);

int geob200_linear_profile_enable(int on);
int geob200_set_split_k(int on);
int geob200_set_linear_persistent(int on);
int64_t geob200_linear_profile_read(int64_t capacity, int64_t* shapes, float* ms);

#define GEOB200_MAX_STAGES 6
typedef struct { const float* weight; const float* bias; int64_t c_in, c_out; } geob200_linear_t;
typedef struct { const float* gamma; const float* beta; } geob200_norm_t;
typedef struct { const float* weights; const float* weights_t; const float* bias; const float* kernel_points;
                 int64_t c_in, c_out; float sigma; } geob200_kpconv_t;
typedef struct {
    int32_t has_unary1, has_shortcut, strided, reserved;
    int64_t c_in;
    geob200_linear_t unary1; geob200_norm_t norm1;
    geob200_kpconv_t conv;   geob200_norm_t norm_conv;
    geob200_linear_t unary2; geob200_norm_t norm2;
    geob200_linear_t shortcut; geob200_norm_t norm_sc;
} geob200_resblock_t;
typedef struct {
    int32_t num_stages, finest_decoder, groups, init_dim;
    geob200_kpconv_t conv1; geob200_norm_t norm1;
    geob200_resblock_t blocks[1 + 3 * (GEOB200_MAX_STAGES - 1)];
    geob200_linear_t decoders[GEOB200_MAX_STAGES];
    geob200_norm_t decoder_norms[GEOB200_MAX_STAGES];
} geob200_backbone_t;
size_t geob200_backbone_workspace_bytes(const geob200_backbone_t* net, const int64_t* level_rows);
int geob200_backbone_forward(const geob200_backbone_t* net, const float* feats, const float* const* points, const int64_t* level_rows,
                             const int64_t* const* neighbors, const int64_t* neighbor_width, const int64_t* const* subsampling,
                             const int64_t* subsampling_width, const int64_t* const* upsampling, const int64_t* upsampling_width,
                             float* const* out_feats, void* gn_workspace, size_t gn_workspace_bytes, void* workspace,
                             size_t workspace_bytes, void* stream);

size_t geob200_backbone_gn_workspace_bytes(const geob200_backbone_t* net, const int64_t* level_rows, int64_t n_pairs);
int geob200_backbone_forward_batched(const geob200_backbone_t* net, const float* feats, const float* const* points,
                                     const int64_t* level_rows, const int64_t* const* neighbors, const int64_t* neighbor_width,
                                     const int64_t* const* subsampling, const int64_t* subsampling_width,
                                     const int64_t* const* upsampling, const int64_t* upsampling_width, float* const* out_feats,
                                     void* gn_workspace, size_t gn_workspace_bytes, void* workspace, size_t workspace_bytes, void* stream,
                                     int64_t n_pairs, const int64_t* const* cloud_rows_h, const int32_t* const* sub_cloud_max);

typedef struct {
    int32_t is_self, reserved;
    const float* w_qkv; const float* b_qkv; const float* w_q; const float* b_q; const float* w_kv; const float* b_kv;
    const float* wp_t; const float* bp;
    geob200_linear_t att_linear; geob200_norm_t att_norm;
    geob200_linear_t expand; geob200_linear_t squeeze; geob200_norm_t out_norm;
} geob200_tlayer_t;
size_t geob200_transformer_workspace_bytes(int64_t n0, int64_t n1, int64_t channels, int64_t heads, int64_t num_layers);
int geob200_transformer_forward(const geob200_tlayer_t* layers, int64_t num_layers, int64_t channels, int64_t heads, const float* x,
                                int64_t n0, int64_t n1, const float* emb0, const float* emb1, float* out, void* workspace,
                                size_t workspace_bytes, void* stream);

size_t geob200_transformer_batched_workspace_bytes(int64_t n_pairs, const int64_t* cloud_rows_h, int64_t channels, int64_t heads,
                                                   int64_t num_layers);
int geob200_transformer_forward_batched(const geob200_tlayer_t* layers, int64_t num_layers, int64_t channels, int64_t heads,
                                        const float* x, int64_t n_pairs, const int64_t* cloud_rows_h, const float* const* embeddings_h,
                                        float* out, void* workspace, size_t workspace_bytes, void* stream);

#ifdef __cplusplus
}
#endif
#endif
```

Baseline: 328.6.

## Presplit weights into TF32 hi/lo images once and use register-A wgmma

Weights are now split into TF32 high and low parts once at model setup by a new split kernel, and the pre-split image is passed through every linear, kpconv and transformer projection to the tensor-core GEMM. This removes the in-kernel split warps and the per-stage split pass over shared memory for weights. The activation split appears to move into registers via new register-operand wgmma variants, so each stage holds one A tile. Freeing that shared memory allows one more pipeline stage. The cost is extra device memory for the weight images plus wider parameter structs, and it relies on the images staying in sync with the weights.

```diff
diff --git a/geotransformer_b200/_lib.py b/geotransformer_b200/_lib.py
--- a/geotransformer_b200/_lib.py
+++ b/geotransformer_b200/_lib.py
@@ -33,6 +33,7 @@
 _sig('geob200_kpconv_tc', c_int, P, P, P, P, I64, I64, I64, P, I64, P, P, I64, I64, F, P, P, SZ, P)
 _sig('geob200_set_linear_mode', None, c_int)
 _sig('geob200_linear', c_int, P, I64, P, P, P, I64, I64, I64, I64, c_int, P)
+_sig('geob200_split_tf32', c_int, P, I64, I64, I64, P, P)
 _sig('geob200_linear_batched', c_int, P, I64, I64, P, I64, I64, P, I64, P, I64, I64, I64, I64, I64, I64, c_int, P)
 _sig('geob200_group_norm_workspace_bytes', SZ, I64)
 _sig('geob200_group_norm', c_int, P, I64, I64, I64, P, P, F, P, c_int, F, P, P, SZ, P)
diff --git a/geotransformer_b200/csrc/common.cuh b/geotransformer_b200/csrc/common.cuh
--- a/geotransformer_b200/csrc/common.cuh
+++ b/geotransformer_b200/csrc/common.cuh
@@ -84,13 +84,19 @@
 int linear_group_norm_impl(const float* x, int64_t ldx, const float* weight, const float* bias, int64_t m, int64_t n, int64_t k,
                            int64_t groups, const float* gamma, const float* beta, float eps, const float* residual, int leaky,
                            float slope, float* pre_norm, float* y, void* workspace, size_t workspace_bytes, void* stream,
-                           const GnSeg* seg);
+                           const GnSeg* seg, const float* w_img = nullptr);
 int kpconv_group_norm_impl(const float* s_feats, const float* q_points, const float* s_points, const int64_t* neighbors,
                            int64_t n_query, int64_t n_support, int64_t n_neighbors, const float* kernel_points, int64_t n_kernel,
                            const float* weights_t, const float* bias, int64_t c_in, int64_t c_out, float sigma, int64_t groups,
                            const float* gamma, const float* beta, float eps, int leaky, float slope, float* pre_norm, float* y,
                            void* gn_workspace, size_t gn_workspace_bytes, void* workspace, size_t workspace_bytes, void* stream,
-                           const GnSeg* seg);
+                           const GnSeg* seg, const float* w_img = nullptr);
+int linear_img(const float* x, int64_t ldx, const float* weight, const float* w_img, const float* bias, float* y, int64_t ldy,
+               int64_t m, int64_t n, int64_t k, int relu, void* stream);
+int kpconv_tc_impl(const float* s_feats, const float* q_points, const float* s_points, const int64_t* neighbors, int64_t n_query,
+                   int64_t n_support, int64_t n_neighbors, const float* kernel_points, int64_t n_kernel, const float* weights_t,
+                   const float* w_img, const float* bias, int64_t c_in, int64_t c_out, float sigma, float* out, void* workspace,
+                   size_t workspace_bytes, void* stream);
 
 int maxpool_seg(const float* x, const int64_t* neighbors, int64_t n_query, int64_t n_support, int64_t n_neighbors, int64_t channels,
                 float* y, const GnSeg* seg, const int* cloud_max, void* stream);
diff --git a/geotransformer_b200/csrc/hopper.cuh b/geotransformer_b200/csrc/hopper.cuh
--- a/geotransformer_b200/csrc/hopper.cuh
+++ b/geotransformer_b200/csrc/hopper.cuh
@@ -103,6 +103,32 @@
         : "l"(da), "l"(db), "r"(acc));
 }
 
+template <int N> __device__ void wgmma_tf32_rs(float (&d)[N / 2], const uint32_t (&a)[4], uint64_t db, uint32_t acc);
+
+template <> __device__ __forceinline__ void wgmma_tf32_rs<32>(float (&d)[16], const uint32_t (&a)[4], uint64_t db, uint32_t acc) {
+    asm volatile(
+        "{\n\t.reg .pred p;\n\tsetp.ne.b32 p, %21, 0;\n\t"
+        "wgmma.mma_async.sync.aligned.m64n32k8.f32.tf32.tf32 {%0, %1, %2, %3, %4, %5, %6, %7, %8, %9, %10, %11, %12, %13, %14, %15}, {%16, %17, %18, %19}, %20, p, 1, 1;\n\t}"
+        : "+f"(d[0]), "+f"(d[1]), "+f"(d[2]), "+f"(d[3]), "+f"(d[4]), "+f"(d[5]), "+f"(d[6]), "+f"(d[7]), "+f"(d[8]), "+f"(d[9]), "+f"(d[10]), "+f"(d[11]), "+f"(d[12]), "+f"(d[13]), "+f"(d[14]), "+f"(d[15])
+        : "r"(a[0]), "r"(a[1]), "r"(a[2]), "r"(a[3]), "l"(db), "r"(acc));
+}
+
+template <> __device__ __forceinline__ void wgmma_tf32_rs<64>(float (&d)[32], const uint32_t (&a)[4], uint64_t db, uint32_t acc) {
+    asm volatile(
+        "{\n\t.reg .pred p;\n\tsetp.ne.b32 p, %37, 0;\n\t"
+        "wgmma.mma_async.sync.aligned.m64n64k8.f32.tf32.tf32 {%0, %1, %2, %3, %4, %5, %6, %7, %8, %9, %10, %11, %12, %13, %14, %15, %16, %17, %18, %19, %20, %21, %22, %23, %24, %25, %26, %27, %28, %29, %30, %31}, {%32, %33, %34, %35}, %36, p, 1, 1;\n\t}"
+        : "+f"(d[0]), "+f"(d[1]), "+f"(d[2]), "+f"(d[3]), "+f"(d[4]), "+f"(d[5]), "+f"(d[6]), "+f"(d[7]), "+f"(d[8]), "+f"(d[9]), "+f"(d[10]), "+f"(d[11]), "+f"(d[12]), "+f"(d[13]), "+f"(d[14]), "+f"(d[15]), "+f"(d[16]), "+f"(d[17]), "+f"(d[18]), "+f"(d[19]), "+f"(d[20]), "+f"(d[21]), "+f"(d[22]), "+f"(d[23]), "+f"(d[24]), "+f"(d[25]), "+f"(d[26]), "+f"(d[27]), "+f"(d[28]), "+f"(d[29]), "+f"(d[30]), "+f"(d[31])
+        : "r"(a[0]), "r"(a[1]), "r"(a[2]), "r"(a[3]), "l"(db), "r"(acc));
+}
+
+template <> __device__ __forceinline__ void wgmma_tf32_rs<128>(float (&d)[64], const uint32_t (&a)[4], uint64_t db, uint32_t acc) {
+    asm volatile(
+        "{\n\t.reg .pred p;\n\tsetp.ne.b32 p, %69, 0;\n\t"
+        "wgmma.mma_async.sync.aligned.m64n128k8.f32.tf32.tf32 {%0, %1, %2, %3, %4, %5, %6, %7, %8, %9, %10, %11, %12, %13, %14, %15, %16, %17, %18, %19, %20, %21, %22, %23, %24, %25, %26, %27, %28, %29, %30, %31, %32, %33, %34, %35, %36, %37, %38, %39, %40, %41, %42, %43, %44, %45, %46, %47, %48, %49, %50, %51, %52, %53, %54, %55, %56, %57, %58, %59, %60, %61, %62, %63}, {%64, %65, %66, %67}, %68, p, 1, 1;\n\t}"
+        : "+f"(d[0]), "+f"(d[1]), "+f"(d[2]), "+f"(d[3]), "+f"(d[4]), "+f"(d[5]), "+f"(d[6]), "+f"(d[7]), "+f"(d[8]), "+f"(d[9]), "+f"(d[10]), "+f"(d[11]), "+f"(d[12]), "+f"(d[13]), "+f"(d[14]), "+f"(d[15]), "+f"(d[16]), "+f"(d[17]), "+f"(d[18]), "+f"(d[19]), "+f"(d[20]), "+f"(d[21]), "+f"(d[22]), "+f"(d[23]), "+f"(d[24]), "+f"(d[25]), "+f"(d[26]), "+f"(d[27]), "+f"(d[28]), "+f"(d[29]), "+f"(d[30]), "+f"(d[31]), "+f"(d[32]), "+f"(d[33]), "+f"(d[34]), "+f"(d[35]), "+f"(d[36]), "+f"(d[37]), "+f"(d[38]), "+f"(d[39]), "+f"(d[40]), "+f"(d[41]), "+f"(d[42]), "+f"(d[43]), "+f"(d[44]), "+f"(d[45]), "+f"(d[46]), "+f"(d[47]), "+f"(d[48]), "+f"(d[49]), "+f"(d[50]), "+f"(d[51]), "+f"(d[52]), "+f"(d[53]), "+f"(d[54]), "+f"(d[55]), "+f"(d[56]), "+f"(d[57]), "+f"(d[58]), "+f"(d[59]), "+f"(d[60]), "+f"(d[61]), "+f"(d[62]), "+f"(d[63])
+        : "r"(a[0]), "r"(a[1]), "r"(a[2]), "r"(a[3]), "l"(db), "r"(acc));
+}
+
 template <int N> __device__ void wgmma_f16(float (&d)[N / 2], uint64_t da, uint64_t db, uint32_t acc);
 
 template <> __device__ __forceinline__ void wgmma_f16<128>(float (&d)[64], uint64_t da, uint64_t db, uint32_t acc) {
diff --git a/geotransformer_b200/csrc/kpconv.cu b/geotransformer_b200/csrc/kpconv.cu
--- a/geotransformer_b200/csrc/kpconv.cu
+++ b/geotransformer_b200/csrc/kpconv.cu
@@ -822,7 +822,7 @@
 using namespace geob200;
 
 namespace geob200 {
-int linear_tc(const float* x, int64_t ldx, const float* w, int64_t ldw, const float* bias, const float* row_scale, float* y, int64_t ldy,
+int linear_tc(const float* x, int64_t ldx, const float* w, int64_t ldw, const float* w_img, const float* bias, const float* row_scale, float* y, int64_t ldy,
               int64_t m, int64_t n, int64_t k, int relu, cudaStream_t st, const GnFuse* gn = nullptr);
 static int g_linear_mode = 1;
 }
@@ -841,6 +841,16 @@
                       int64_t n_support, int64_t n_neighbors, const float* kernel_points, int64_t n_kernel, const float* weights_t,
                       const float* bias, int64_t c_in, int64_t c_out, float sigma, float* out, void* workspace, size_t workspace_bytes,
                       void* stream) {
+    return geob200::kpconv_tc_impl(s_feats, q_points, s_points, neighbors, n_query, n_support, n_neighbors, kernel_points, n_kernel,
+                                   weights_t, nullptr, bias, c_in, c_out, sigma, out, workspace, workspace_bytes, stream);
+}
+}
+
+namespace geob200 {
+int kpconv_tc_impl(const float* s_feats, const float* q_points, const float* s_points, const int64_t* neighbors, int64_t n_query,
+                   int64_t n_support, int64_t n_neighbors, const float* kernel_points, int64_t n_kernel, const float* weights_t,
+                   const float* w_img, const float* bias, int64_t c_in, int64_t c_out, float sigma, float* out, void* workspace,
+                   size_t workspace_bytes, void* stream) {
     cudaStream_t st = (cudaStream_t)stream;
     GEOB_REQUIRE(n_kernel == KP, "kpconv_tc: kernel_size %lld unsupported", (long long)n_kernel);
     GEOB_REQUIRE(n_query > 0 && n_support > 0 && n_neighbors > 0, "kpconv_tc: empty input");
@@ -856,10 +866,22 @@
                          (int)n_support, (int)n_query, (int)c_in, wf, inv_count, st);
     GEOB_CHECK_LAUNCH();
     count_launches(2);
-    const int rc = linear_tc(wf, KP * c_in, weights_t, KP * c_in, bias, inv_count, out, c_out, n_query, c_out, KP * c_in, 0, st);
+    const int rc = linear_tc(wf, KP * c_in, weights_t, KP * c_in, w_img, bias, inv_count, out, c_out, n_query, c_out, KP * c_in, 0, st);
     GEOB_REQUIRE(rc == 0, "kpconv_tc: tensor-core GEMM rejected the shape");
     return 0;
 }
+
+int linear_img(const float* x, int64_t ldx, const float* weight, const float* w_img, const float* bias, float* y, int64_t ldy,
+               int64_t m, int64_t n, int64_t k, int relu, void* stream) {
+    if (g_linear_mode == 1 && m > 0 && n > 0 && k > 0) {
+        const int rc = linear_tc(x, ldx, weight, k, w_img, bias, nullptr, y, ldy, m, n, k, relu, (cudaStream_t)stream);
+        if (rc <= 0) return rc;
+    }
+    return geob200_linear(x, ldx, weight, bias, y, ldy, m, n, k, relu, stream);
+}
+}
+
+extern "C" {
 
 int geob200_kpconv(const float* s_feats, const float* q_points, const float* s_points, const int64_t* neighbors,
                    int64_t n_query, int64_t n_support, int64_t n_neighbors, const float* kernel_points, int64_t n_kernel,
@@ -914,7 +936,7 @@
     cudaStream_t st = (cudaStream_t)stream;
     GEOB_REQUIRE(m > 0 && n > 0 && k > 0 && batch > 0, "linear: empty problem");
     if (batch == 1 && g_linear_mode == 1) {
-        const int rc = linear_tc(x, ldx, weight, ldw, bias, nullptr, y, ldy, m, n, k, relu, st);
+        const int rc = linear_tc(x, ldx, weight, ldw, nullptr, bias, nullptr, y, ldy, m, n, k, relu, st);
         if (rc <= 0) return rc;
     }
     const unsigned z = (unsigned)batch;
@@ -1074,7 +1096,7 @@
 int linear_group_norm_impl(const float* x, int64_t ldx, const float* weight, const float* bias, int64_t m, int64_t n, int64_t k,
                            int64_t groups, const float* gamma, const float* beta, float eps, const float* residual, int leaky,
                            float slope, float* pre_norm, float* y, void* workspace, size_t workspace_bytes, void* stream,
-                           const GnSeg* seg) {
+                           const GnSeg* seg, const float* w_img) {
     cudaStream_t st = (cudaStream_t)stream;
     const int64_t np = (seg != nullptr && seg->n_pairs > 1) ? seg->n_pairs : 1;
     GEOB_REQUIRE(m > 0 && n > 0 && k > 0 && groups > 0 && n % groups == 0 && n % 4 == 0, "linear_group_norm: bad shape");
@@ -1083,7 +1105,7 @@
     if (g_linear_mode == 1) {
         const GnWs w = gn_carve(workspace, workspace_bytes, groups, np);
         GnFuse gn{(int)groups, 0, w.partial};
-        const int rc = linear_tc(x, ldx, weight, k, bias, nullptr, pre_norm, n, m, n, k, 0, st, &gn);
+        const int rc = linear_tc(x, ldx, weight, k, w_img, bias, nullptr, pre_norm, n, m, n, k, 0, st, &gn);
         if (rc < 0) return rc;
         if (rc == 0) {
             if (np > 1) {
@@ -1096,7 +1118,7 @@
             return 0;
         }
     }
-    int rc = geob200_linear(x, ldx, weight, bias, pre_norm, n, m, n, k, 0, stream);
+    int rc = linear_img(x, ldx, weight, w_img, bias, pre_norm, n, m, n, k, 0, stream);
     if (rc != 0) return rc;
     return group_norm_impl(pre_norm, m, n, groups, gamma, beta, eps, residual, leaky, slope, y, workspace, workspace_bytes, stream, seg);
 }
@@ -1126,7 +1148,7 @@
                            const float* weights_t, const float* bias, int64_t c_in, int64_t c_out, float sigma, int64_t groups,
                            const float* gamma, const float* beta, float eps, int leaky, float slope, float* pre_norm, float* y,
                            void* gn_workspace, size_t gn_workspace_bytes, void* workspace, size_t workspace_bytes, void* stream,
-                           const GnSeg* seg) {
+                           const GnSeg* seg, const float* w_img) {
     cudaStream_t st = (cudaStream_t)stream;
     const int64_t np = (seg != nullptr && seg->n_pairs > 1) ? seg->n_pairs : 1;
     GEOB_REQUIRE(n_kernel == KP, "kpconv_group_norm: kernel_size %lld unsupported", (long long)n_kernel);
@@ -1150,7 +1172,7 @@
     count_launches(2);
     const GnWs w = gn_carve(gn_workspace, gn_workspace_bytes, groups, np);
     GnFuse gn{(int)groups, 0, w.partial};
-    int rc = linear_tc(wf, KP * c_in, weights_t, KP * c_in, bias, inv_count, pre_norm, c_out, n_query, c_out, KP * c_in, 0, st, &gn);
+    int rc = linear_tc(wf, KP * c_in, weights_t, KP * c_in, w_img, bias, inv_count, pre_norm, c_out, n_query, c_out, KP * c_in, 0, st, &gn);
     if (rc < 0) return rc;
     if (rc == 0) {
         if (np > 1) {
@@ -1162,7 +1184,7 @@
         GEOB_CHECK_LAUNCH();
         return 0;
     }
-    rc = linear_tc(wf, KP * c_in, weights_t, KP * c_in, bias, inv_count, pre_norm, c_out, n_query, c_out, KP * c_in, 0, st);
+    rc = linear_tc(wf, KP * c_in, weights_t, KP * c_in, w_img, bias, inv_count, pre_norm, c_out, n_query, c_out, KP * c_in, 0, st);
     GEOB_REQUIRE(rc == 0, "kpconv_group_norm: tensor-core GEMM rejected the shape");
     return group_norm_impl(pre_norm, n_query, c_out, groups, gamma, beta, eps, nullptr, leaky, slope, y, gn_workspace, gn_workspace_bytes,
                            stream, seg);
diff --git a/geotransformer_b200/csrc/linear_tc.cu b/geotransformer_b200/csrc/linear_tc.cu
--- a/geotransformer_b200/csrc/linear_tc.cu
+++ b/geotransformer_b200/csrc/linear_tc.cu
@@ -17,43 +17,22 @@
 constexpr int KC = 32;
 constexpr int TILE_A = BM * 128;
 constexpr int TILE_B = 128 * 128;
-constexpr int STAGE = 2 * TILE_A + 2 * TILE_B;
-constexpr int NSTAGE = 3;
+constexpr int STAGE = TILE_A + 2 * TILE_B;
+constexpr int NSTAGE = 4;
 constexpr int PRODUCER_WARP = 8;
-constexpr int NSPLIT_WARPS = 3;
-constexpr int NTHREADS = (PRODUCER_WARP + 1 + NSPLIT_WARPS) * 32;
+constexpr int NTHREADS = (PRODUCER_WARP + 4) * 32;
 constexpr int SMEM = NSTAGE * STAGE + 1024 + 256 + 8 * 128 * 8 + 512;
 
-__device__ __forceinline__ void split_stage(unsigned char* st, int BN, int t) {
-    constexpr int NT = NSPLIT_WARPS * 32;
-    const int nvec_a = TILE_A / 16, nvec_b = BN * 128 / 16;
-    const int nvec = nvec_a + nvec_b;
-    for (int v0 = t; v0 < nvec; v0 += 2 * NT) {
-        const int v1 = v0 + NT;
-        unsigned char* p0 = (v0 < nvec_a) ? (st + v0 * 16) : (st + 2 * TILE_A + (v0 - nvec_a) * 16);
-        unsigned char* l0 = p0 + ((v0 < nvec_a) ? TILE_A : TILE_B);
-        const bool two = v1 < nvec;
-        unsigned char* p1 = !two ? p0 : (v1 < nvec_a) ? (st + v1 * 16) : (st + 2 * TILE_A + (v1 - nvec_a) * 16);
-        unsigned char* l1 = p1 + ((v1 < nvec_a) ? TILE_A : TILE_B);
-        const float4 x0 = *reinterpret_cast<float4*>(p0);
-        const float4 x1 = *reinterpret_cast<float4*>(p1);
-        float4 h0, q0, h1, q1;
-        h0.x = tf32_rn(x0.x); q0.x = x0.x - h0.x;
-        h0.y = tf32_rn(x0.y); q0.y = x0.y - h0.y;
-        h0.z = tf32_rn(x0.z); q0.z = x0.z - h0.z;
-        h0.w = tf32_rn(x0.w); q0.w = x0.w - h0.w;
-        h1.x = tf32_rn(x1.x); q1.x = x1.x - h1.x;
-        h1.y = tf32_rn(x1.y); q1.y = x1.y - h1.y;
-        h1.z = tf32_rn(x1.z); q1.z = x1.z - h1.z;
-        h1.w = tf32_rn(x1.w); q1.w = x1.w - h1.w;
-        *reinterpret_cast<float4*>(p0) = h0;
-        *reinterpret_cast<float4*>(l0) = q0;
-        if (two) {
-            *reinterpret_cast<float4*>(p1) = h1;
-            *reinterpret_cast<float4*>(l1) = q1;
-        }
-    }
-    fence_proxy_async();
+__global__ void __launch_bounds__(256) split_tf32_kernel(const float* __restrict__ w, long long ld, long long n, long long k,
+                                                         float* __restrict__ out) {
+    const long long nk = n * k;
+    for (long long i = (long long)blockIdx.x * blockDim.x + threadIdx.x; i < nk; i += (long long)gridDim.x * blockDim.x) {
+        const long long r = i / k, c = i % k;
+        const float x = w[r * ld + c];
+        const float hi = tf32_rn(x);
+        out[i] = hi;
+        out[nk + i] = x - hi;
+    }
 }
 
 template <int BNI>
@@ -67,9 +46,8 @@
     extern __shared__ unsigned char smem_raw[];
     unsigned char* smem = (unsigned char*)(((uintptr_t)smem_raw + 1023) & ~(uintptr_t)1023);
     uint64_t* bars = (uint64_t*)(smem + NSTAGE * STAGE);
-    uint64_t* raw_full = bars;
-    uint64_t* split_full = bars + NSTAGE;
-    uint64_t* empty = bars + 2 * NSTAGE;
+    uint64_t* full = bars;
+    uint64_t* empty = bars + NSTAGE;
     float2* gn_sm = (float2*)(smem + NSTAGE * STAGE + 256);
     float* bias_s = (float*)(gn_sm + 8 * 128);
     const int warp = threadIdx.x >> 5, lane = threadIdx.x & 31;
@@ -77,15 +55,16 @@
     const int tiles_per_split = col_tiles * row_tiles;
 
     if (threadIdx.x == 0) {
-        for (int s = 0; s < NSTAGE; ++s) { mbar_init(&raw_full[s], 1); mbar_init(&split_full[s], NSPLIT_WARPS); mbar_init(&empty[s], 8); }
+        for (int s = 0; s < NSTAGE; ++s) { mbar_init(&full[s], 1); mbar_init(&empty[s], 8); }
         asm volatile("fence.mbarrier_init.release.cluster;" ::: "memory");
         asm volatile("prefetch.tensormap [%0];" ::"l"(&map_x) : "memory");
         asm volatile("prefetch.tensormap [%0];" ::"l"(&map_w) : "memory");
     }
     __syncthreads();
 
-    if (warp == PRODUCER_WARP) {
-        if (lane == 0) {
+    if (warp >= PRODUCER_WARP) {
+        asm volatile("setmaxnreg.dec.sync.aligned.u32 40;" ::: "memory");
+        if (warp == PRODUCER_WARP && lane == 0) {
             int s = 0;
             uint32_t ph = 0;
             for (int t = blockIdx.x; t < num_tiles; t += gridDim.x) {
@@ -95,33 +74,18 @@
                 for (int kc = kc0; kc < kc1; ++kc) {
                     mbar_wait(&empty[s], ph ^ 1u);
                     unsigned char* st = smem + s * STAGE;
-                    mbar_arrive_expect_tx(&raw_full[s], (uint32_t)(TILE_A + BN * 128));
-                    tma_load_2d(st, &map_x, kc * KC, m0, &raw_full[s]);
-                    tma_load_2d(st + 2 * TILE_A, &map_w, kc * KC, n0, &raw_full[s]);
+                    mbar_arrive_expect_tx(&full[s], (uint32_t)(TILE_A + 2 * BN * 128));
+                    tma_load_2d(st, &map_x, kc * KC, m0, &full[s]);
+                    tma_load_2d(st + TILE_A, &map_w, kc * KC, n0, &full[s]);
+                    tma_load_2d(st + TILE_A + TILE_B, &map_w, kc * KC, N + n0, &full[s]);
                     if (++s == NSTAGE) { s = 0; ph ^= 1u; }
                 }
             }
         }
         return;
     }
-    if (warp > PRODUCER_WARP) {
-        const int ts = threadIdx.x - (PRODUCER_WARP + 1) * 32;
-        int s = 0;
-        uint32_t ph = 0;
-        for (int t = blockIdx.x; t < num_tiles; t += gridDim.x) {
-            const int z = t / tiles_per_split;
-            const int kc0 = z * chunks_per_split, kc1 = min(nk, kc0 + chunks_per_split);
-            for (int kc = kc0; kc < kc1; ++kc) {
-                mbar_wait(&raw_full[s], ph);
-                split_stage(smem + s * STAGE, BN, ts);
-                __syncwarp();
-                if (lane == 0) mbar_arrive(&split_full[s]);
-                if (++s == NSTAGE) { s = 0; ph ^= 1u; }
-            }
-        }
-        return;
-    }
-
+
+    asm volatile("setmaxnreg.inc.sync.aligned.u32 232;" ::: "memory");
     const int wg = warp >> 2, wq = warp & 3;
     int s = 0;
     uint32_t ph = 0;
@@ -137,31 +101,41 @@
         float acc[R], cor[R];
 #pragma unroll
         for (int i = 0; i < R; ++i) { acc[i] = 0.f; cor[i] = 0.f; }
-        int prev_s = -1;
+        const int g = lane >> 2, tq = lane & 3;
+        const int a_off = (wg * 64 + wq * 16 + g) * 128 + tq * 4;
         for (int kc = kc0; kc < kc1; ++kc) {
-            mbar_wait(&split_full[s], ph);
-            const uint32_t st = smem_u32(smem + s * STAGE);
-            const uint64_t a_hi = make_desc(st + wg * (TILE_A / 2)), a_lo = make_desc(st + TILE_A + wg * (TILE_A / 2));
-            const uint64_t b_hi = make_desc(st + 2 * TILE_A), b_lo = make_desc(st + 2 * TILE_A + TILE_B);
+            mbar_wait(&full[s], ph);
+            unsigned char* st = smem + s * STAGE;
+            uint32_t f[2][KC / 8][4];
+#pragma unroll
+            for (int kk = 0; kk < KC / 8; ++kk)
+#pragma unroll
+                for (int e = 0; e < 4; ++e) {
+                    const int j = 2 * kk + (e >> 1);
+                    const float x = *reinterpret_cast<const float*>(st + a_off + (e & 1) * 8 * 128 + ((j ^ g) << 4));
+                    const float hi = tf32_rn(x);
+                    f[0][kk][e] = __float_as_uint(hi);
+                    f[1][kk][e] = __float_as_uint(x - hi);
+                }
+            const uint32_t sb = smem_u32(st + TILE_A);
+            const uint64_t b_hi = make_desc(sb), b_lo = make_desc(sb + TILE_B);
             wgmma_fence();
 #pragma unroll
             for (int kk = 0; kk < KC / 8; ++kk) {
                 const uint64_t adv = (uint64_t)(kk * 2);
                 const uint32_t accum = (kc == kc0 && kk == 0) ? 0u : 1u;
-                wgmma_tf32<BNI>(acc, a_hi + adv, b_hi + adv, accum);
-                wgmma_tf32<BNI>(cor, a_hi + adv, b_lo + adv, accum);
-                wgmma_tf32<BNI>(cor, a_lo + adv, b_hi + adv, 1u);
+                wgmma_tf32_rs<BNI>(acc, f[0][kk], b_hi + adv, accum);
+                wgmma_tf32_rs<BNI>(cor, f[0][kk], b_lo + adv, accum);
+                wgmma_tf32_rs<BNI>(cor, f[1][kk], b_hi + adv, 1u);
             }
             wgmma_commit();
-            wgmma_wait<1>();
-            if (prev_s >= 0) { __syncwarp(); if (lane == 0) mbar_arrive(&empty[prev_s]); }
-            prev_s = s;
+            wgmma_wait<0>();
+            __syncwarp();
+            if (lane == 0) mbar_arrive(&empty[s]);
             if (++s == NSTAGE) { s = 0; ph ^= 1u; }
         }
-        wgmma_wait<0>();
         reg_fence(acc);
         reg_fence(cor);
-        if (prev_s >= 0) { __syncwarp(); if (lane == 0) mbar_arrive(&empty[prev_s]); }
 
         const int r0 = m0 + wg * 64 + wq * 16 + (lane >> 2);
         const int c0 = 2 * (lane & 3);
@@ -302,12 +276,12 @@
 static bool g_splitk_on = true;
 static bool g_persistent_on = true;
 
-struct SplitWs { void* ptr; size_t bytes; };
-static std::vector<std::pair<cudaStream_t, SplitWs>> g_split_ws;
+struct StreamWs { void* ptr; size_t bytes; };
+static std::vector<std::pair<cudaStream_t, StreamWs>> g_split_ws, g_wimg_ws;
 static std::mutex g_split_mu;
-static float* splitk_scratch(cudaStream_t st, size_t bytes) {
+static float* stream_scratch(std::vector<std::pair<cudaStream_t, StreamWs>>& pool, cudaStream_t st, size_t bytes) {
     std::lock_guard<std::mutex> lk(g_split_mu);
-    for (auto& e : g_split_ws)
+    for (auto& e : pool)
         if (e.first == st) {
             if (e.second.bytes >= bytes) return (float*)e.second.ptr;
             cudaFreeAsync(e.second.ptr, st);
@@ -316,23 +290,29 @@
             e.second.bytes = bytes * 2;
             return (float*)e.second.ptr;
         }
-    SplitWs w{nullptr, 0};
+    StreamWs w{nullptr, 0};
     const size_t cap = bytes * 2 > (16u << 20) ? bytes * 2 : (16u << 20);
     if (cudaMallocAsync(&w.ptr, cap, st) != cudaSuccess) return nullptr;
     w.bytes = cap;
-    g_split_ws.push_back({st, w});
+    pool.push_back({st, w});
     return (float*)w.ptr;
 }
 
-int linear_tc(const float* x, int64_t ldx, const float* w, int64_t ldw, const float* bias, const float* row_scale, float* y, int64_t ldy,
-              int64_t m, int64_t n, int64_t k, int relu, cudaStream_t st, const GnFuse* gn) {
-    if (m < 64 || n < 32 || (n % 16) != 0 || (k % 4) != 0 || (ldx % 4) != 0 || (ldw % 4) != 0) return 1;
-    if ((reinterpret_cast<uintptr_t>(x) & 15) || (reinterpret_cast<uintptr_t>(w) & 15)) return 1;
+static void launch_split_tf32(const float* w, int64_t ld, int64_t n, int64_t k, float* out, cudaStream_t st) {
+    const long long nk = (long long)n * k;
+    long long blocks = (nk + 255) / 256;
+    if (blocks > 4LL * num_sms()) blocks = 4LL * num_sms();
+    ltc::split_tf32_kernel<<<(unsigned)(blocks > 0 ? blocks : 1), 256, 0, st>>>(w, ld, n, k, out);
+    count_launches(1);
+}
+
+int linear_tc(const float* x, int64_t ldx, const float* w, int64_t ldw, const float* w_img, const float* bias, const float* row_scale,
+              float* y, int64_t ldy, int64_t m, int64_t n, int64_t k, int relu, cudaStream_t st, const GnFuse* gn) {
+    if (m < 64 || n < 32 || (n % 16) != 0 || (k % 4) != 0 || (ldx % 4) != 0) return 1;
+    if ((reinterpret_cast<uintptr_t>(x) & 15) || (reinterpret_cast<uintptr_t>(w_img) & 15)) return 1;
+    if (w_img == nullptr && ((ldw % 4) != 0 || (reinterpret_cast<uintptr_t>(w) & 15))) return 1;
     if (n > 128 && (n % 128) != 0) return 1;
     const int BN = (int)(n >= 128 ? 128 : n);
-    CUtensorMap mx, mw;
-    if (ltc::encode_map(&mx, x, m, k, ldx, ltc::BM)) return -1;
-    if (ltc::encode_map(&mw, w, n, k, ldw, BN)) return -1;
     const int col_tiles = (int)(n / BN), row_tiles = (int)((m + ltc::BM - 1) / ltc::BM);
     GnFuse g{};
     if (gn != nullptr) {
@@ -356,9 +336,18 @@
     if (splits > 1) {
         cps = (nk + splits - 1) / splits;
         splits = (nk + cps - 1) / cps;
-        part = splitk_scratch(st, (size_t)splits * (size_t)m * (size_t)n * sizeof(float));
+        part = stream_scratch(g_split_ws, st, (size_t)splits * (size_t)m * (size_t)n * sizeof(float));
         if (part == nullptr) { splits = 1; cps = nk; }
     }
+    float* img = nullptr;
+    if (w_img == nullptr) {
+        img = stream_scratch(g_wimg_ws, st, (size_t)2 * (size_t)n * (size_t)k * sizeof(float));
+        if (img == nullptr) { set_error("linear_tc: weight image scratch allocation failed"); return -1; }
+        w_img = img;
+    }
+    CUtensorMap mx, mw;
+    if (ltc::encode_map(&mx, x, m, k, ldx, ltc::BM)) return -1;
+    if (ltc::encode_map(&mw, w_img, 2 * n, k, k, BN)) return -1;
     ProfRec rec{};
     const bool prof = g_prof_on;
     if (prof) {
@@ -367,6 +356,7 @@
         rec.m = m; rec.n = n; rec.k = k;
         cudaEventRecord(rec.a, st);
     }
+    if (img != nullptr) launch_split_tf32(w, ldw, n, k, img, st);
     const int num_tiles = tiles * splits;
     const bool persistent = g_persistent_on && splits == 1 && tiles > num_sms();
     const unsigned grid = (unsigned)(persistent ? num_sms() : num_tiles);
@@ -404,6 +394,13 @@
     return 0;
 }
 
+int geob200_split_tf32(const float* w, int64_t ld, int64_t n, int64_t k, float* out, void* stream) {
+    GEOB_REQUIRE(n > 0 && k > 0 && ld >= k, "split_tf32: bad shape (%lld x %lld, ld %lld)", (long long)n, (long long)k, (long long)ld);
+    geob200::launch_split_tf32(w, ld, n, k, out, (cudaStream_t)stream);
+    GEOB_CHECK_LAUNCH();
+    return 0;
+}
+
 int geob200_set_split_k(int on) {
     geob200::g_splitk_on = on != 0;
     return 0;
diff --git a/geotransformer_b200/csrc/native.cu b/geotransformer_b200/csrc/native.cu
--- a/geotransformer_b200/csrc/native.cu
+++ b/geotransformer_b200/csrc/native.cu
@@ -28,8 +28,8 @@
         const size_t mark = c.ar.off;
         void* ws = c.ar.take<char>(wb);
         GEOB_REQUIRE(c.ar.ok(), "native: arena too small (kpconv)");
-        TRY(geob200_kpconv_tc(s_feats, q_pts, s_pts, nbr, m, ns, h, k.kernel_points, 15, k.weights_t, k.bias, k.c_in, k.c_out, k.sigma,
-                              out, ws, wb, c.stream));
+        TRY(kpconv_tc_impl(s_feats, q_pts, s_pts, nbr, m, ns, h, k.kernel_points, 15, k.weights_t, k.weights_img, k.bias, k.c_in, k.c_out,
+                           k.sigma, out, ws, wb, c.stream));
         c.ar.off = mark;
         return 0;
     }
@@ -55,7 +55,8 @@
         void* ws = c.ar.take<char>(wb);
         GEOB_REQUIRE(c.ar.ok(), "native: arena too small (kpconv)");
         TRY(kpconv_group_norm_impl(s_feats, q_pts, s_pts, nbr, m, ns, h, k.kernel_points, 15, k.weights_t, k.bias, k.c_in, k.c_out,
-                                   k.sigma, c.groups, n.gamma, n.beta, 1e-5f, 1, 0.1f, y, out, c.gn_ws, c.gn_ws_bytes, ws, wb, c.stream, seg));
+                                   k.sigma, c.groups, n.gamma, n.beta, 1e-5f, 1, 0.1f, y, out, c.gn_ws, c.gn_ws_bytes, ws, wb, c.stream, seg,
+                                   k.weights_img));
         c.ar.off = mark;
         return 0;
     }
@@ -68,7 +69,7 @@
     float* t = c.fl(rows, l.c_out);
     GEOB_REQUIRE(c.ar.ok(), "native: arena too small (unary)");
     TRY(linear_group_norm_impl(x, l.c_in, l.weight, l.bias, rows, l.c_out, l.c_in, c.groups, n.gamma, n.beta, 1e-5f, residual, leaky,
-                               0.1f, t, out, c.gn_ws, c.gn_ws_bytes, c.stream, seg));
+                               0.1f, t, out, c.gn_ws, c.gn_ws_bytes, c.stream, seg, l.weight_img));
     return 0;
 }
 
@@ -198,7 +199,7 @@
         const geob200_linear_t& l = net->decoders[S - 1 - lvl];
         float* o = out_feats[oi++];
         if (lvl == net->finest_decoder) {
-            TRY(geob200_linear(cat, l.c_in, l.weight, l.bias, o, l.c_out, m, l.c_out, l.c_in, 0, stream));
+            TRY(linear_img(cat, l.c_in, l.weight, l.weight_img, l.bias, o, l.c_out, m, l.c_out, l.c_in, 0, stream));
         } else {
             TRY(run_unary(c, l, net->decoder_norms[S - 1 - lvl], cat, m, nullptr, 1, o, sg[lvl - 1]));
         }
@@ -220,10 +221,10 @@
     float* y1 = c.fl(rows, 2 * ch);
     float* y2 = c.fl(rows, ch);
     GEOB_REQUIRE(c.ar.ok(), "native: arena too small (transformer tail)");
-    TRY(geob200_linear(hidden, ch, L.att_linear.weight, L.att_linear.bias, h, ch, rows, ch, ch, 0, c.stream));
+    TRY(linear_img(hidden, ch, L.att_linear.weight, L.att_linear.weight_img, L.att_linear.bias, h, ch, rows, ch, ch, 0, c.stream));
     TRY(geob200_add_layernorm(h, inp, L.att_norm.gamma, L.att_norm.beta, rows, ch, 1e-5f, x, c.stream));
-    TRY(geob200_linear(x, ch, L.expand.weight, L.expand.bias, y1, 2 * ch, rows, 2 * ch, ch, 1, c.stream));
-    TRY(geob200_linear(y1, 2 * ch, L.squeeze.weight, L.squeeze.bias, y2, ch, rows, ch, 2 * ch, 0, c.stream));
+    TRY(linear_img(x, ch, L.expand.weight, L.expand.weight_img, L.expand.bias, y1, 2 * ch, rows, 2 * ch, ch, 1, c.stream));
+    TRY(linear_img(y1, 2 * ch, L.squeeze.weight, L.squeeze.weight_img, L.squeeze.bias, y2, ch, rows, ch, 2 * ch, 0, c.stream));
     TRY(geob200_add_layernorm(x, y2, L.out_norm.gamma, L.out_norm.beta, rows, ch, 1e-5f, out, c.stream));
     return 0;
 }
@@ -279,7 +280,7 @@
             float* qb = c.fl(n, H);
             float* hidden = c.fl(n, C);
             GEOB_REQUIRE(c.ar.ok(), "native: arena too small (self layer)");
-            TRY(geob200_linear(x, C, L.w_qkv, L.b_qkv, qkv, 3 * C, n, 3 * C, C, 0, stream));
+            TRY(linear_img(x, C, L.w_qkv, L.w_qkv_img, L.b_qkv, qkv, 3 * C, n, 3 * C, C, 0, stream));
             const int64_t d = C / H;
             TRY(geob200_linear_batched(qkv, 3 * C, d, L.wp_t, C, d, nullptr, 0, qp, H * C, C, n, C, d, H, 0, stream));
             TRY(geob200_head_bias(qkv, 3 * C, L.bp, n, C, H, qb, stream));
@@ -299,8 +300,8 @@
             float* kv0 = c.fl(R, 2 * C);
             float* hid1 = c.fl(Sn, C);
             GEOB_REQUIRE(c.ar.ok(), "native: arena too small (cross layer)");
-            TRY(geob200_linear(x, C, L.w_q, L.b_q, q0, C, R, C, C, 0, stream));
-            TRY(geob200_linear(x + R * C, C, L.w_kv, L.b_kv, kv1, 2 * C, Sn, 2 * C, C, 0, stream));
+            TRY(linear_img(x, C, L.w_q, L.w_q_img, L.b_q, q0, C, R, C, C, 0, stream));
+            TRY(linear_img(x + R * C, C, L.w_kv, L.w_kv_img, L.b_kv, kv1, 2 * C, Sn, 2 * C, C, 0, stream));
             for (int64_t p = 0; p < B; ++p) {
                 const int64_t ro = off[p], so = off[B + p] - R;
                 items[p] = geob200_att_item_t{q0 + ro * C, kv1 + so * 2 * C, kv1 + so * 2 * C + C, nullptr, nullptr, nullptr, hid0 + ro * C,
@@ -308,8 +309,8 @@
             }
             TRY(geob200_attention_batched(items, B, C, 2 * C, 2 * C, C, C, H, att_ws, att_ws_bytes, stream));
             TRY(run_tail(c, L, hid0, x, R, C, y));
-            TRY(geob200_linear(x + R * C, C, L.w_q, L.b_q, q1, C, Sn, C, C, 0, stream));
-            TRY(geob200_linear(y, C, L.w_kv, L.b_kv, kv0, 2 * C, R, 2 * C, C, 0, stream));
+            TRY(linear_img(x + R * C, C, L.w_q, L.w_q_img, L.b_q, q1, C, Sn, C, C, 0, stream));
+            TRY(linear_img(y, C, L.w_kv, L.w_kv_img, L.b_kv, kv0, 2 * C, R, 2 * C, C, 0, stream));
             for (int64_t p = 0; p < B; ++p) {
                 const int64_t ro = off[p], so = off[B + p] - R;
                 items[p] = geob200_att_item_t{q1 + so * C, kv0 + ro * 2 * C, kv0 + ro * 2 * C + C, nullptr, nullptr, nullptr, hid1 + so * C,
diff --git a/geotransformer_b200/functional.py b/geotransformer_b200/functional.py
--- a/geotransformer_b200/functional.py
+++ b/geotransformer_b200/functional.py
@@ -96,6 +96,16 @@
         out = torch.empty((m, n), dtype=_f32, device=x.device)
     L.check(L.lib().geob200_linear(x.data_ptr(), x.stride(0), weight.data_ptr(), L.ptr(bias), out.data_ptr(),
                                    out.stride(0), m, n, k, int(relu), L.stream_ptr()), 'linear')
+    return out
+
+
+def split_tf32(weight):
+    weight = _detach(weight)
+    if not weight.is_cuda or weight.dtype != _f32 or weight.dim() != 2 or weight.stride(1) != 1:
+        raise RuntimeError('split_tf32: weight must be a 2-D float32 CUDA tensor with unit inner stride')
+    n, k = weight.shape
+    out = torch.empty((2 * n, k), dtype=_f32, device=weight.device)
+    L.check(L.lib().geob200_split_tf32(weight.data_ptr(), weight.stride(0), n, k, out.data_ptr(), L.stream_ptr()), 'split_tf32')
     return out
 
 
diff --git a/geotransformer_b200/native.py b/geotransformer_b200/native.py
--- a/geotransformer_b200/native.py
+++ b/geotransformer_b200/native.py
@@ -10,7 +10,7 @@
 
 
 class LinearT(ctypes.Structure):
-    _fields_ = [('weight', P), ('bias', P), ('c_in', I64), ('c_out', I64)]
+    _fields_ = [('weight', P), ('bias', P), ('c_in', I64), ('c_out', I64), ('weight_img', P)]
 
 
 class NormT(ctypes.Structure):
@@ -18,7 +18,8 @@
 
 
 class KPConvT(ctypes.Structure):
-    _fields_ = [('weights', P), ('weights_t', P), ('bias', P), ('kernel_points', P), ('c_in', I64), ('c_out', I64), ('sigma', F32)]
+    _fields_ = [('weights', P), ('weights_t', P), ('bias', P), ('kernel_points', P), ('c_in', I64), ('c_out', I64), ('sigma', F32),
+                ('weights_img', P)]
 
 
 class ResBlockT(ctypes.Structure):
@@ -35,7 +36,7 @@
 class TLayerT(ctypes.Structure):
     _fields_ = [('is_self', I32), ('reserved', I32), ('w_qkv', P), ('b_qkv', P), ('w_q', P), ('b_q', P), ('w_kv', P), ('b_kv', P),
                 ('wp_t', P), ('bp', P), ('att_linear', LinearT), ('att_norm', NormT), ('expand', LinearT), ('squeeze', LinearT),
-                ('out_norm', NormT)]
+                ('out_norm', NormT), ('w_qkv_img', P), ('w_q_img', P), ('w_kv_img', P)]
 
 
 def _ptr(t):
@@ -53,8 +54,13 @@
         self.hidden = model.transformer.in_proj.out_features
         self.heads = model.transformer.transformer.layers[0].attention.attention.num_heads
 
+    def _img(self, w):
+        img = GF.split_tf32(w.detach())
+        self._keep.append(img)
+        return _ptr(img)
+
     def _lin(self, mlp):
-        return LinearT(_ptr(mlp.weight), _ptr(mlp.bias), mlp.in_features, mlp.out_features)
+        return LinearT(_ptr(mlp.weight), _ptr(mlp.bias), mlp.in_features, mlp.out_features, self._img(mlp.weight))
 
     def _norm(self, gn):
         return NormT(_ptr(gn.norm.weight), _ptr(gn.norm.bias))
@@ -64,7 +70,8 @@
         wt = w.reshape(-1, w.shape[2]).t().contiguous() if w.shape[1] % 32 == 0 else None
         if wt is not None:
             self._keep.append(wt)
-        return KPConvT(_ptr(w), _ptr(wt), _ptr(kp.bias), _ptr(kp.kernel_points), w.shape[1], w.shape[2], float(kp.sigma))
+        return KPConvT(_ptr(w), _ptr(wt), _ptr(kp.bias), _ptr(kp.kernel_points), w.shape[1], w.shape[2], float(kp.sigma),
+                       None if wt is None else self._img(wt))
 
     def _res(self, blk):
         r = ResBlockT()
@@ -113,15 +120,16 @@
                 wpt = mha.proj_p.weight.detach().t().contiguous()
                 self._keep += [wqkv, bqkv, wpt]
                 t.w_qkv, t.b_qkv, t.wp_t, t.bp = _ptr(wqkv), _ptr(bqkv), _ptr(wpt), _ptr(mha.proj_p.bias)
+                t.w_qkv_img = self._img(wqkv)
             else:
                 wkv, bkv = cat(('proj_k', 'proj_v'), 'weight'), cat(('proj_k', 'proj_v'), 'bias')
                 self._keep += [wkv, bkv]
                 t.w_q, t.b_q, t.w_kv, t.b_kv = _ptr(mha.proj_q.weight), _ptr(mha.proj_q.bias), _ptr(wkv), _ptr(bkv)
+                t.w_q_img, t.w_kv_img = self._img(mha.proj_q.weight), self._img(wkv)
             att, ffn = layer.attention, layer.output
-            t.att_linear = LinearT(_ptr(att.linear.weight), _ptr(att.linear.bias), att.linear.in_features, att.linear.out_features)
+            t.att_linear = self._lin(att.linear)
             t.att_norm = NormT(_ptr(att.norm.weight), _ptr(att.norm.bias))
-            t.expand = LinearT(_ptr(ffn.expand.weight), _ptr(ffn.expand.bias), ffn.expand.in_features, ffn.expand.out_features)
-            t.squeeze = LinearT(_ptr(ffn.squeeze.weight), _ptr(ffn.squeeze.bias), ffn.squeeze.in_features, ffn.squeeze.out_features)
+            t.expand, t.squeeze = self._lin(ffn.expand), self._lin(ffn.squeeze)
             t.out_norm = NormT(_ptr(ffn.norm.weight), _ptr(ffn.norm.bias))
             arr[i] = t
         return arr, len(tr.layers)
diff --git a/include/geob200.h b/include/geob200.h
--- a/include/geob200.h
+++ b/include/geob200.h
@@ -37,6 +37,8 @@
                       int64_t n_support, int64_t n_neighbors, const float* kernel_points, int64_t n_kernel, const float* weights_t,
                       const float* bias, int64_t c_in, int64_t c_out, float sigma, float* out, void* workspace, size_t workspace_bytes,
                       void* stream);
+
+int geob200_split_tf32(const float* w, int64_t ld, int64_t n, int64_t k, float* out, void* stream);
 
 void geob200_set_linear_mode(int mode);
 int geob200_linear(const float* x, int64_t ldx, const float* weight, const float* bias, float* y, int64_t ldy, int64_t m,
@@ -231,10 +233,10 @@
 int64_t geob200_linear_profile_read(int64_t capacity, int64_t* shapes, float* ms);
 
 #define GEOB200_MAX_STAGES 6
-typedef struct { const float* weight; const float* bias; int64_t c_in, c_out; } geob200_linear_t;
+typedef struct { const float* weight; const float* bias; int64_t c_in, c_out; const float* weight_img; } geob200_linear_t;
 typedef struct { const float* gamma; const float* beta; } geob200_norm_t;
 typedef struct { const float* weights; const float* weights_t; const float* bias; const float* kernel_points;
-                 int64_t c_in, c_out; float sigma; } geob200_kpconv_t;
+                 int64_t c_in, c_out; float sigma; const float* weights_img; } geob200_kpconv_t;
 typedef struct {
     int32_t has_unary1, has_shortcut, strided, reserved;
     int64_t c_in;
@@ -271,6 +273,7 @@
     const float* wp_t; const float* bp;
     geob200_linear_t att_linear; geob200_norm_t att_norm;
     geob200_linear_t expand; geob200_linear_t squeeze; geob200_norm_t out_norm;
+    const float* w_qkv_img; const float* w_q_img; const float* w_kv_img;
 } geob200_tlayer_t;
 size_t geob200_transformer_workspace_bytes(int64_t n0, int64_t n1, int64_t channels, int64_t heads, int64_t num_layers);
 int geob200_transformer_forward(const geob200_tlayer_t* layers, int64_t num_layers, int64_t channels, int64_t heads, const float* x,
```

New measurement: 359.1, median of 6. 9.3% higher.
